# gmongaras/Stable-Diffusion-3-From-Scratch

Measured on AMD Instinct MI355X. Metric: train images/sec MMDiT-B 256^2 bf16, higher is better.
Workload: dtype bf16

## Files before the change

### include/mmdit_hip.h

```cpp
#ifndef MMDIT_HIP_H
#define MMDIT_HIP_H

#include <stdint.h>

#ifdef __cplusplus
extern "C" {
#endif

#define MMDIT_F32 0
#define MMDIT_BF16 1
#define MMDIT_FP8 2

#define MMDIT_ERR_ARG (-1)
#define MMDIT_ERR_DTYPE (-2)
#define MMDIT_ERR_SHAPE (-3)

#define MMDIT_ACT_NONE 0
#define MMDIT_ACT_SILU 1
#define MMDIT_ACT_SWIGLU 2

#define MMDIT_ACT_SWIGLU_BWD 3

#define MMDIT_PREC_BF16 0
#define MMDIT_PREC_SPLIT 1

typedef void* mmdit_stream_t;

#define MMDIT_ABI_VERSION 9
int mmdit_abi_version(void);
int mmdit_struct_size(int which);
const char* mmdit_build_arch(void);

typedef struct {
  const void* A; int a_dtype; int a_kmajor; int64_t lda;
  const void* B; int b_dtype; int b_kmajor; int64_t ldb;
  void* C; int c_dtype; int64_t ldc;
  int M, N, K;
  const float* bias;
  int act;
  const float* gate; int64_t ld_gate; int rows_per_batch;
  const float* residual; int64_t ld_res;
  void* aux; int aux_dtype; int64_t ld_aux;
  int accumulate;
  int precision;
  int split_k;
  int stream_k;
  int conv_mode, conv_H, conv_W, conv_C;
  const void* scale_a;
  const void* scale_b;
  int scale_mode;
  void* c_scales;
  float* dbias;
  int cu_budget;
} mmdit_gemm_args;
int mmdit_gemm(const mmdit_gemm_args* args, mmdit_stream_t stream);
int mmdit_gemm_grouped(const mmdit_gemm_args* args, int count, mmdit_stream_t stream);
int mmdit_gemm_zero_mask(const mmdit_gemm_args* args, int count, unsigned* mask);
typedef struct mmdit_qk_epilogue {
  const float* wq; const float* wk;
  const float* rope_cos; const float* rope_sin;
  int tokens, tok0;
} mmdit_qk_epilogue;
int mmdit_gemm_qkv_norm_rope(const mmdit_gemm_args* args, const mmdit_qk_epilogue* qk, int count, int heads, int s_total,
                             void* Q, void* K, void* V, mmdit_stream_t stream);
int mmdit_gemm_set_workspace(void* ptr, long long bytes);
int mmdit_gemm_set_claiming(int on);
int mmdit_gemm_get_claiming(void);
int mmdit_debug_occupy(int wgs, long long cycles, mmdit_stream_t stream);
int mmdit_device_cus(void);
int mmdit_gemm_plan(const mmdit_gemm_args* args, int count);

int mmdit_fp8_amax(const void* x, int x_dtype, int64_t n, float* amax, mmdit_stream_t stream);
int mmdit_fp8_quantize(const void* x, int x_dtype, int64_t n, const float* amax, void* q_fp8, float* scale, mmdit_stream_t stream);
int mmdit_fp8_quantize_delayed(const void* x, int x_dtype, int64_t n, float* state, int phase, float margin, void* q_fp8, mmdit_stream_t stream);
int mmdit_mxfp8_quantize(const void* x, int x_dtype, int rows, int K, int64_t ldx, void* q_fp8, void* scales_e8m0, mmdit_stream_t stream);
int mmdit_ln_modulate_fwd_mx(const float* x, const void* acc, int acc_dtype, const float* gate, int64_t ld_gate, float* x_out,
                             const float* scale, const float* shift, int64_t ld_mod, int rows, int d, int rows_per_batch,
                             void* q_fp8, void* scales_e8m0, float* mean, float* rstd, mmdit_stream_t stream);
int mmdit_swiglu_fwd_mx(const void* gu, int dtype, int rows, int hidden, void* q_fp8, void* scales_e8m0, mmdit_stream_t stream);
int mmdit_attn_fwd_mx(const void* Q, const void* K, const void* V, int batch, int heads, int S, int n_img, float scale,
                      void* Ox_fp8, void* Oc_fp8, void* scales_x, void* scales_c, mmdit_stream_t stream);

int mmdit_cast(const void* src, int src_dtype, void* dst, int dst_dtype, int64_t n, mmdit_stream_t stream);

int mmdit_ln_modulate_fwd(const float* x, const float* scale, const float* shift, int64_t ld_mod,
                          int rows, int d, int rows_per_batch,
                          void* out, int out_dtype, float* mean, float* rstd, mmdit_stream_t stream);
int mmdit_ln_modulate_fwd_res(const float* x, const void* acc, int acc_dtype, const float* gate, int64_t ld_gate, float* x_out,
                              const float* scale, const float* shift, int64_t ld_mod,
                              int rows, int d, int rows_per_batch,
                              void* out, int out_dtype, float* mean, float* rstd, mmdit_stream_t stream);
typedef struct mmdit_ln_fwd_problem {
  const float* x; const void* acc; const float* gate; int64_t ld_gate; float* x_out;
  const float* scale; const float* shift; int64_t ld_mod; int rows, rows_per_batch;
  void* out; float* mean; float* rstd;
} mmdit_ln_fwd_problem;
int mmdit_ln_modulate_fwd_pair(const mmdit_ln_fwd_problem* p0, const mmdit_ln_fwd_problem* p1, int d, int acc_dtype, int out_dtype, mmdit_stream_t stream);
typedef struct mmdit_ln_bwd_problem {
  const void* dout; const float* x; const float* mean; const float* rstd; const float* scale; int64_t ld_mod; const float* dres; int rows, rows_per_batch;
  float* dx; float* dscale; float* dshift; int64_t ld_dmod;
  const void* acc; const float* gate; int64_t ld_gate; void* dacc; float* dgate; int64_t ld_dgate; float* dbias; int64_t ld_dbias;
} mmdit_ln_bwd_problem;
int mmdit_ln_modulate_bwd_pair(const mmdit_ln_bwd_problem* p0, const mmdit_ln_bwd_problem* p1, int d, int dout_dtype, mmdit_stream_t stream);
int mmdit_gate_residual_fwd(const float* x, const void* acc, int acc_dtype, const float* gate, int64_t ld_gate,
                            int rows, int d, int rows_per_batch, float* out, mmdit_stream_t stream);
int mmdit_ln_modulate_bwd(const void* dout, int dout_dtype, const float* x, const float* mean, const float* rstd,
                          const float* scale, int64_t ld_mod, const float* dres,
                          int rows, int d, int rows_per_batch,
                          float* dx, float* dscale, float* dshift, int64_t ld_dmod, mmdit_stream_t stream);
int mmdit_ln_modulate_bwd_gated(const void* dout, int dout_dtype, const float* x, const float* mean, const float* rstd,
                                const float* scale, int64_t ld_mod, const float* dres,
                                int rows, int d, int rows_per_batch,
                                float* dx, float* dscale, float* dshift, int64_t ld_dmod,
                                const void* acc, int acc_dtype, const float* gate, int64_t ld_gate,
                                void* dacc, float* dgate, int64_t ld_dgate, float* dbias, int64_t ld_dbias, mmdit_stream_t stream);

int mmdit_text_rmsnorm_fwd(const void* x, int x_dtype, const float* w1, const float* w2, const float* s1, const float* s2,
                           int batch, int tokens, int split, int d, void* out1, void* out2, int out_dtype, mmdit_stream_t stream);
int mmdit_text_rmsnorm_bwd(const void* dout1, const void* dout2, int dout_dtype, const void* x, int x_dtype,
                           const float* w1, const float* w2, const float* s1, const float* s2,
                           int batch, int tokens, int split, int d,
                           float* dw1, float* dw2, float* ds1, float* ds2, mmdit_stream_t stream);

int mmdit_qk_norm_rope_fwd(const void* qkv, int qkv_dtype, const float* wq, const float* wk,
                           const float* rope_cos, const float* rope_sin,
                           int batch, int tokens, int heads, int s_total, int tok0,
                           void* Q, void* K, void* V, mmdit_stream_t stream);
int mmdit_qk_norm_rope_bwd(const void* dQ, const void* dK, const void* dV, int dq_dtype,
                           const void* qkv, int qkv_dtype, const float* wq, const float* wk,
                           const float* rope_cos, const float* rope_sin,
                           int batch, int tokens, int heads, int s_total, int tok0,
                           void* dqkv, int dqkv_dtype, float* dwq, float* dwk, mmdit_stream_t stream);
typedef struct mmdit_qk_problem {
  const void* qkv; const float* wq; const float* wk; const float* rope_cos; const float* rope_sin; int tokens, tok0;
  void* dqkv; float* dwq; float* dwk;
} mmdit_qk_problem;
int mmdit_qk_norm_rope_fwd_pair(const mmdit_qk_problem* p0, const mmdit_qk_problem* p1, int qkv_dtype, int batch, int heads, int s_total,
                                void* Q, void* K, void* V, mmdit_stream_t stream);
int mmdit_qk_norm_rope_bwd_pair(const mmdit_qk_problem* p0, const mmdit_qk_problem* p1, const void* dQ, const void* dK, const void* dV, int dq_dtype,
                                int qkv_dtype, int dqkv_dtype, int batch, int heads, int s_total, mmdit_stream_t stream);

int mmdit_attn_fwd(const void* Q, const void* K, const void* V, int batch, int heads, int S, int n_img,
                   float scale, int mode, void* Ox, void* Oc, float* lse, mmdit_stream_t stream);
int mmdit_attn_bwd_qk(const void* Q, const void* K, const void* V, const void* Ox, const void* Oc, const void* dOx, const void* dOc,
                      const float* lse, float* delta, int batch, int heads, int S, int n_img, float scale,
                      const void* qkv_x, const void* qkv_c, const float* wq_x, const float* wk_x, const float* wq_c, const float* wk_c,
                      const float* rope_cos, const float* rope_sin, void* dqkv_x, void* dqkv_c, float* dw, mmdit_stream_t stream);
int mmdit_attn_bwd(const void* Q, const void* K, const void* V, const void* Ox, const void* Oc,
                   const void* dOx, const void* dOc, const float* lse, float* delta,
                   int batch, int heads, int S, int n_img, float scale,
                   void* dQ, void* dK, void* dV, int dq_dtype, mmdit_stream_t stream);

int mmdit_swiglu_fwd(const void* gu, void* h, int dtype, int rows, int hidden, mmdit_stream_t stream);
int mmdit_swiglu_bwd(const void* dh, const void* gu, void* dgu, int dtype, int rows, int hidden, float* dbias, mmdit_stream_t stream);
int mmdit_gelu_fwd(const void* u, void* h, int dtype, int rows, int hidden, mmdit_stream_t stream);
int mmdit_gelu_bwd(const void* dh, const void* u, void* du, int dtype, int rows, int hidden, float* dbias, mmdit_stream_t stream);
typedef struct mmdit_mlp_bwd_problem { const void* dh; const void* gu; void* dgu; int rows; float* dbias; } mmdit_mlp_bwd_problem;
int mmdit_mlp_act_bwd_pair(const mmdit_mlp_bwd_problem* p0, const mmdit_mlp_bwd_problem* p1, int dtype, int hidden, int gelu, mmdit_stream_t stream);
int mmdit_silu_bwd(const void* dy, int dy_dtype, const float* pre, void* dpre, int dpre_dtype, int rows, int cols, float* dbias, int rows_per_bias,
                   mmdit_stream_t stream);

int mmdit_gate_residual_bwd(const float* dy, const void* acc, int acc_dtype, const float* gate, int64_t ld_gate,
                            int rows, int d, int rows_per_batch, void* dacc, int dacc_dtype,
                            float* dgate, int64_t ld_dgate, float* dbias, int64_t ld_dbias, mmdit_stream_t stream);

int mmdit_flow_loss(const float* v, const void* x0, const void* eps, int in_dtype, int64_t n, float coef, float* dv, float* partials,
                    float* loss, mmdit_stream_t stream);

int mmdit_colsum(const void* x, int dtype, int rows, int cols, int64_t ld, float* out, mmdit_stream_t stream);

int mmdit_patchify(const void* img, int img_dtype, int batch, int ch, int H, int W, void* tokens, int tok_dtype, mmdit_stream_t stream);
int mmdit_unpatchify(const void* tokens, int tok_dtype, int batch, int ch, int H, int W, void* img, int img_dtype, mmdit_stream_t stream);

int mmdit_time_embed_fwd(const float* t, const float* time_scale, const float* denom, int batch, int dim, void* out, int out_dtype, mmdit_stream_t stream);
int mmdit_time_embed_bwd(const void* dout, int dout_dtype, const float* t, const float* time_scale, const float* denom, int batch, int dim, float* dtime_scale, mmdit_stream_t stream);

int mmdit_vae_nchw_to_nhwc(const void* src, int src_dtype, int batch, int C, int H, int W, int C_padded, float scale, float shift,
                           void* dst_bf16, mmdit_stream_t stream);
int mmdit_vae_nhwc_to_nchw(const float* src, int batch, int C, int H, int W, int ld, float lo, float hi, float* dst, mmdit_stream_t stream);
int mmdit_vae_im2col3x3(const void* src_bf16, int batch, int H, int W, int C, int mode, void* dst_bf16, mmdit_stream_t stream);
int mmdit_vae_groupnorm(const void* x, int x_dtype, const float* gamma, const float* beta, int batch, int H, int W, int C, int groups, float eps, int silu,
                        float* sums_zeroed, void* y_bf16, int pad, mmdit_stream_t stream);
int mmdit_vae_pad_cast(const void* x, int x_dtype, int batch, int H, int W, int C, int upsample, void* y_bf16, mmdit_stream_t stream);
int mmdit_vae_softmax_rows(const float* x, int rows, int cols, int ld, float scale, void* y_bf16, mmdit_stream_t stream);

#define MMDIT_ADAMW_CHUNK 65536
typedef struct mmdit_adamw_tensor {
  float* param;
  const float* grad;
  float* exp_avg;
  float* exp_avg_sq;
  int64_t numel;
  void* shadow_bf16;
} mmdit_adamw_tensor;
int mmdit_grad_sumsq(const mmdit_adamw_tensor* tensors, const int* chunk_tensor, const int64_t* chunk_off, int n_chunks, float* partials, mmdit_stream_t stream);
int mmdit_clip_coef(const float* partials, int n_chunks, const float* loss_scale, float max_norm, float* out3, mmdit_stream_t stream);
int mmdit_adamw_step(const mmdit_adamw_tensor* tensors, const int* chunk_tensor, const int64_t* chunk_off, int n_chunks, const float* coef_found,
                     const float* step_count, double lr, double beta1, double beta2, double eps, double weight_decay, mmdit_stream_t stream);
int mmdit_adamw_step_dlr(const mmdit_adamw_tensor* tensors, const int* chunk_tensor, const int64_t* chunk_off, int n_chunks, const float* coef_found,
                         const float* step_count, const double* lr_dev, double beta1, double beta2, double eps, double weight_decay, mmdit_stream_t stream);

typedef struct mmdit_cast_tensor {
  const float* src;
  void* dst;
  int64_t numel;
} mmdit_cast_tensor;
int mmdit_cast_multi(const mmdit_cast_tensor* tensors, const int* chunk_tensor, const int64_t* chunk_off, int n_chunks, mmdit_stream_t stream);

#ifdef __cplusplus
}
#endif
#endif
```

### stable-diffusion-3-from-scratch_amd/_lib.py

```python
import ctypes
import os
import re

_HERE = os.path.dirname(os.path.abspath(__file__))
def experiment(name: str, default: str) -> str:
    return os.environ.get(name, default) if os.environ.get("MMDIT_EXPERIMENTS") == "1" else default


LIB_PATH = os.environ.get("MMDIT_LIB") or os.path.join(_HERE, "libmmdit_hip.so")
HEADER_PATH = os.path.join(_HERE, "..", "include", "mmdit_hip.h")

F32, BF16 = 0, 1
ACT_NONE, ACT_SILU, ACT_SWIGLU, ACT_SWIGLU_BWD = 0, 1, 2, 3
PREC_BF16, PREC_SPLIT = 0, 1
FP8 = 2

_vp, _i, _i64, _f, _d = ctypes.c_void_p, ctypes.c_int, ctypes.c_int64, ctypes.c_float, ctypes.c_double


class GemmArgs(ctypes.Structure):
    _fields_ = [
        ("A", _vp), ("a_dtype", _i), ("a_kmajor", _i), ("lda", _i64),
        ("B", _vp), ("b_dtype", _i), ("b_kmajor", _i), ("ldb", _i64),
        ("C", _vp), ("c_dtype", _i), ("ldc", _i64),
        ("M", _i), ("N", _i), ("K", _i),
        ("bias", _vp),
        ("act", _i),
        ("gate", _vp), ("ld_gate", _i64), ("rows_per_batch", _i),
        ("residual", _vp), ("ld_res", _i64),
        ("aux", _vp), ("aux_dtype", _i), ("ld_aux", _i64),
        ("accumulate", _i),
        ("precision", _i),
        ("split_k", _i),
        ("stream_k", _i),
        ("conv_mode", _i), ("conv_H", _i), ("conv_W", _i), ("conv_C", _i),
        ("scale_a", _vp), ("scale_b", _vp), ("scale_mode", _i), ("c_scales", _vp),
        ("dbias", _vp),
        ("cu_budget", _i),
    ]


class LnFwdProblem(ctypes.Structure):
    _fields_ = [("x", ctypes.c_void_p), ("acc", ctypes.c_void_p), ("gate", ctypes.c_void_p), ("ld_gate", ctypes.c_int64), ("x_out", ctypes.c_void_p),
                ("scale", ctypes.c_void_p), ("shift", ctypes.c_void_p), ("ld_mod", ctypes.c_int64), ("rows", ctypes.c_int), ("rows_per_batch", ctypes.c_int),
                ("out", ctypes.c_void_p), ("mean", ctypes.c_void_p), ("rstd", ctypes.c_void_p)]


class LnBwdProblem(ctypes.Structure):
    _fields_ = [("dout", ctypes.c_void_p), ("x", ctypes.c_void_p), ("mean", ctypes.c_void_p), ("rstd", ctypes.c_void_p), ("scale", ctypes.c_void_p),
                ("ld_mod", ctypes.c_int64), ("dres", ctypes.c_void_p), ("rows", ctypes.c_int), ("rows_per_batch", ctypes.c_int),
                ("dx", ctypes.c_void_p), ("dscale", ctypes.c_void_p), ("dshift", ctypes.c_void_p), ("ld_dmod", ctypes.c_int64),
                ("acc", ctypes.c_void_p), ("gate", ctypes.c_void_p), ("ld_gate", ctypes.c_int64), ("dacc", ctypes.c_void_p), ("dgate", ctypes.c_void_p),
                ("ld_dgate", ctypes.c_int64), ("dbias", ctypes.c_void_p), ("ld_dbias", ctypes.c_int64)]


class QkProblem(ctypes.Structure):
    _fields_ = [("qkv", ctypes.c_void_p), ("wq", ctypes.c_void_p), ("wk", ctypes.c_void_p), ("rope_cos", ctypes.c_void_p), ("rope_sin", ctypes.c_void_p),
                ("tokens", ctypes.c_int), ("tok0", ctypes.c_int), ("dqkv", ctypes.c_void_p), ("dwq", ctypes.c_void_p), ("dwk", ctypes.c_void_p)]


class MlpBwdProblem(ctypes.Structure):
    _fields_ = [("dh", ctypes.c_void_p), ("gu", ctypes.c_void_p), ("dgu", ctypes.c_void_p), ("rows", ctypes.c_int), ("dbias", ctypes.c_void_p)]


class QkEpilogue(ctypes.Structure):
    _fields_ = [("wq", _vp), ("wk", _vp), ("rope_cos", _vp), ("rope_sin", _vp), ("tokens", _i), ("tok0", _i)]


_SIGNATURES = {
    "mmdit_abi_version": ([], _i),
    "mmdit_struct_size": ([_i], _i),
    "mmdit_build_arch": ([], ctypes.c_char_p),
    "mmdit_gemm": ([ctypes.POINTER(GemmArgs), _vp], _i),
    "mmdit_gemm_grouped": ([ctypes.POINTER(GemmArgs), _i, _vp], _i),
    "mmdit_gemm_plan": ([ctypes.POINTER(GemmArgs), _i], _i),
    "mmdit_gemm_set_workspace": ([_vp, ctypes.c_longlong], _i),
    "mmdit_debug_occupy": ([_i, ctypes.c_longlong, _vp], _i),
    "mmdit_gemm_set_claiming": ([_i], _i),
    "mmdit_gemm_get_claiming": ([], _i),
    "mmdit_device_cus": ([], _i),
    "mmdit_gemm_qkv_norm_rope": ([ctypes.POINTER(GemmArgs), ctypes.POINTER(QkEpilogue), _i, _i, _i, _vp, _vp, _vp, _vp], _i),
    "mmdit_gemm_zero_mask": ([ctypes.POINTER(GemmArgs), _i, ctypes.POINTER(ctypes.c_uint)], _i),
    "mmdit_fp8_amax": ([_vp, _i, _i64, _vp, _vp], _i),
    "mmdit_fp8_quantize": ([_vp, _i, _i64, _vp, _vp, _vp, _vp], _i),
    "mmdit_fp8_quantize_delayed": ([_vp, _i, _i64, _vp, _i, ctypes.c_float, _vp, _vp], _i),
    "mmdit_mxfp8_quantize": ([_vp, _i, _i, _i, _i64, _vp, _vp, _vp], _i),
    "mmdit_ln_modulate_fwd_mx": ([_vp, _vp, _i, _vp, _i64, _vp, _vp, _vp, _i64, _i, _i, _i, _vp, _vp, _vp, _vp, _vp], _i),
    "mmdit_swiglu_fwd_mx": ([_vp, _i, _i, _i, _vp, _vp, _vp], _i),
    "mmdit_attn_fwd_mx": ([_vp, _vp, _vp, _i, _i, _i, _i, ctypes.c_float, _vp, _vp, _vp, _vp, _vp], _i),
    "mmdit_cast": ([_vp, _i, _vp, _i, _i64, _vp], _i),
    "mmdit_ln_modulate_fwd": ([_vp, _vp, _vp, _i64, _i, _i, _i, _vp, _i, _vp, _vp, _vp], _i),
    "mmdit_ln_modulate_fwd_res": ([_vp, _vp, _i, _vp, _i64, _vp, _vp, _vp, _i64, _i, _i, _i, _vp, _i, _vp, _vp, _vp], _i),
    "mmdit_ln_modulate_fwd_pair": ([ctypes.POINTER(LnFwdProblem), ctypes.POINTER(LnFwdProblem), _i, _i, _i, _vp], _i),
    "mmdit_ln_modulate_bwd_pair": ([ctypes.POINTER(LnBwdProblem), ctypes.POINTER(LnBwdProblem), _i, _i, _vp], _i),
    "mmdit_qk_norm_rope_fwd_pair": ([ctypes.POINTER(QkProblem), ctypes.POINTER(QkProblem), _i, _i, _i, _i, _vp, _vp, _vp, _vp], _i),
    "mmdit_qk_norm_rope_bwd_pair": ([ctypes.POINTER(QkProblem), ctypes.POINTER(QkProblem), _vp, _vp, _vp, _i, _i, _i, _i, _i, _i, _vp], _i),
    "mmdit_mlp_act_bwd_pair": ([ctypes.POINTER(MlpBwdProblem), ctypes.POINTER(MlpBwdProblem), _i, _i, _i, _vp], _i),
    "mmdit_gate_residual_fwd": ([_vp, _vp, _i, _vp, _i64, _i, _i, _i, _vp, _vp], _i),
    "mmdit_ln_modulate_bwd": ([_vp, _i, _vp, _vp, _vp, _vp, _i64, _vp, _i, _i, _i, _vp, _vp, _vp, _i64, _vp], _i),
    "mmdit_ln_modulate_bwd_gated": ([_vp, _i, _vp, _vp, _vp, _vp, _i64, _vp, _i, _i, _i, _vp, _vp, _vp, _i64, _vp, _i, _vp, _i64, _vp, _vp, _i64, _vp, _i64, _vp], _i),
    "mmdit_text_rmsnorm_fwd": ([_vp, _i, _vp, _vp, _vp, _vp, _i, _i, _i, _i, _vp, _vp, _i, _vp], _i),
    "mmdit_text_rmsnorm_bwd": ([_vp, _vp, _i, _vp, _i, _vp, _vp, _vp, _vp, _i, _i, _i, _i, _vp, _vp, _vp, _vp, _vp], _i),
    "mmdit_qk_norm_rope_fwd": ([_vp, _i, _vp, _vp, _vp, _vp, _i, _i, _i, _i, _i, _vp, _vp, _vp, _vp], _i),
    "mmdit_qk_norm_rope_bwd": ([_vp, _vp, _vp, _i, _vp, _i, _vp, _vp, _vp, _vp, _i, _i, _i, _i, _i, _vp, _i, _vp, _vp, _vp], _i),
    "mmdit_attn_fwd": ([_vp, _vp, _vp, _i, _i, _i, _i, _f, _i, _vp, _vp, _vp, _vp], _i),
    "mmdit_attn_bwd_qk": ([_vp] * 9 + [_i, _i, _i, _i, _f] + [_vp] * 11 + [_vp], _i),
    "mmdit_attn_bwd": ([_vp, _vp, _vp, _vp, _vp, _vp, _vp, _vp, _vp, _i, _i, _i, _i, _f, _vp, _vp, _vp, _i, _vp], _i),
    "mmdit_swiglu_fwd": ([_vp, _vp, _i, _i, _i, _vp], _i),
    "mmdit_swiglu_bwd": ([_vp, _vp, _vp, _i, _i, _i, _vp, _vp], _i),
    "mmdit_gelu_fwd": ([_vp, _vp, _i, _i, _i, _vp], _i),
    "mmdit_gelu_bwd": ([_vp, _vp, _vp, _i, _i, _i, _vp, _vp], _i),
    "mmdit_silu_bwd": ([_vp, _i, _vp, _vp, _i, _i, _i, _vp, _i, _vp], _i),
    "mmdit_gate_residual_bwd": ([_vp, _vp, _i, _vp, _i64, _i, _i, _i, _vp, _i, _vp, _i64, _vp, _i64, _vp], _i),
    "mmdit_flow_loss": ([_vp, _vp, _vp, _i, _i64, _f, _vp, _vp, _vp, _vp], _i),
    "mmdit_colsum": ([_vp, _i, _i, _i, _i64, _vp, _vp], _i),
    "mmdit_vae_nchw_to_nhwc": ([_vp, _i, _i, _i, _i, _i, _i, ctypes.c_float, ctypes.c_float, _vp, _vp], _i),
    "mmdit_vae_nhwc_to_nchw": ([_vp, _i, _i, _i, _i, _i, ctypes.c_float, ctypes.c_float, _vp, _vp], _i),
    "mmdit_vae_im2col3x3": ([_vp, _i, _i, _i, _i, _i, _vp, _vp], _i),
    "mmdit_vae_groupnorm": ([_vp, _i, _vp, _vp, _i, _i, _i, _i, _i, ctypes.c_float, _i, _vp, _vp, _i, _vp], _i),
    "mmdit_vae_pad_cast": ([_vp, _i, _i, _i, _i, _i, _i, _vp, _vp], _i),
    "mmdit_vae_softmax_rows": ([_vp, _i, _i, _i, ctypes.c_float, _vp, _vp], _i),
    "mmdit_patchify": ([_vp, _i, _i, _i, _i, _i, _vp, _i, _vp], _i),
    "mmdit_unpatchify": ([_vp, _i, _i, _i, _i, _i, _vp, _i, _vp], _i),
    "mmdit_time_embed_fwd": ([_vp, _vp, _vp, _i, _i, _vp, _i, _vp], _i),
    "mmdit_time_embed_bwd": ([_vp, _i, _vp, _vp, _vp, _i, _i, _vp, _vp], _i),
    "mmdit_grad_sumsq": ([_vp, _vp, _vp, _i, _vp, _vp], _i),
    "mmdit_clip_coef": ([_vp, _i, _vp, _f, _vp, _vp], _i),
    "mmdit_adamw_step": ([_vp, _vp, _vp, _i, _vp, _vp, _d, _d, _d, _d, _d, _vp], _i),
    "mmdit_adamw_step_dlr": ([_vp, _vp, _vp, _i, _vp, _vp, _vp, _d, _d, _d, _d, _vp], _i),
    "mmdit_cast_multi": ([_vp, _vp, _vp, _i, _vp], _i),
}
ADAMW_CHUNK = 65536
ABI_VERSION = 9
_STRUCTS = [("mmdit_gemm_args", GemmArgs), ("mmdit_ln_fwd_problem", LnFwdProblem), ("mmdit_ln_bwd_problem", LnBwdProblem),
            ("mmdit_qk_problem", QkProblem), ("mmdit_mlp_bwd_problem", MlpBwdProblem), ("mmdit_adamw_tensor", None), ("mmdit_cast_tensor", None), ("mmdit_qk_epilogue", QkEpilogue)]

_lib = None


def declared_symbols():
    with open(HEADER_PATH) as f:
        txt = f.read()
    return sorted(set(re.findall(r"\b(mmdit_[a-z0-9_]+)\s*\(", txt)) - {"mmdit_stream_t"})


def lib():
    global _lib
    if _lib is None:
        if not os.path.exists(LIB_PATH):
            raise RuntimeError(
                f"{LIB_PATH} is missing: build it with `python __graft_entry__.py build` "
                "(hipcc --offload-arch=gfx950).  There is no PyTorch/CPU fallback for the MMDiT hot path.")
        try:
            import torch
            if torch.cuda.is_available():
                torch.cuda.init()
        except ImportError:
            pass
        L = ctypes.CDLL(LIB_PATH)
        for name, (argtypes, restype) in _SIGNATURES.items():
            fn = getattr(L, name)
            fn.argtypes = argtypes
            fn.restype = restype
        if L.mmdit_abi_version() != ABI_VERSION:
            raise RuntimeError(f"{LIB_PATH}: ABI version {L.mmdit_abi_version()}, this binding is written for {ABI_VERSION}: rebuild (python __graft_entry__.py build)")
        for which, (name, struct) in enumerate(_STRUCTS):
            if struct is not None and L.mmdit_struct_size(which) != ctypes.sizeof(struct):
                raise RuntimeError(f"{LIB_PATH}: sizeof({name}) = {L.mmdit_struct_size(which)}, the binding's ctypes mirror has {ctypes.sizeof(struct)} bytes")
        _lib = L
    return _lib


ERR_ARG, ERR_DTYPE, ERR_SHAPE = -1, -2, -3


def check(status: int, what: str):
    if status != 0:
        kind = {-1: "invalid argument", -2: "dtype combination not built", -3: "unsupported shape"}.get(status, f"hipError {status}")
        raise RuntimeError(f"{what} failed: {kind}")
```

### stable-diffusion-3-from-scratch_amd/csrc/rowops.hip

```cpp
#include "common.h"
#include <float.h>

namespace {

constexpr float LN_EPS = 1e-5f;
constexpr float RMS_EPS = FLT_EPSILON;

__device__ __forceinline__ float bf16_round(float x) { return __builtin_bit_cast(float, pack_bf2(x, 0.f) << 16); }

template <int NITX, typename TO, typename TA, bool RES, bool MX = false>
__device__ __forceinline__ void ln_mod_fwd_body(int block, const float* __restrict__ x, const float* __restrict__ scale, const float* __restrict__ shift,
                                                int64_t ld_mod, int rows, int d, int rpb, TO* __restrict__ out,
                                                float* __restrict__ mean_o, float* __restrict__ rstd_o,
                                                const TA* __restrict__ acc, const float* __restrict__ gate, int64_t ld_gate, float* __restrict__ xo,
                                                unsigned char* __restrict__ mx_scales) {
  constexpr int NIT = NITX < 0 ? -NITX : NITX;
  constexpr bool EXACT = NITX < 0;
  const int lane = threadIdx.x & 63, row = block * 4 + (threadIdx.x >> 6);
  if (row >= rows) return;
  const int nch = d >> 2;
  const int b = row / rpb;
  const float* xr = x + (int64_t)row * d;
  float v[NIT][4];
  float s = 0.f;
#pragma unroll
  for (int it = 0; it < NIT; it++) {
    int ch = lane + 64 * it;
    if (EXACT || ch < nch) {
      ld4(xr + ch * 4, v[it]);
      if constexpr (RES) {
        float av[4], g[4];
        ld4(acc + (int64_t)row * d + ch * 4, av);
        ld4(gate + (int64_t)b * ld_gate + ch * 4, g);
#pragma unroll
        for (int e = 0; e < 4; e++) v[it][e] = v[it][e] + g[e] * av[e];
        __builtin_nontemporal_store(f32x4{v[it][0], v[it][1], v[it][2], v[it][3]}, (f32x4*)(xo + (int64_t)row * d + ch * 4));
      }
      s += v[it][0] + v[it][1] + v[it][2] + v[it][3];
    }
    else { v[it][0] = v[it][1] = v[it][2] = v[it][3] = 0.f; }
  }
  const float mean = wave_sum(s) / d;
  float q = 0.f;
#pragma unroll
  for (int it = 0; it < NIT; it++) {
    int ch = lane + 64 * it;
    if (EXACT || ch < nch) {
#pragma unroll
      for (int e = 0; e < 4; e++) { float c = v[it][e] - mean; q += c * c; }
    }
  }
  const float rstd = rsqrtf(wave_sum(q) / d + LN_EPS);
  if (lane == 0) { mean_o[row] = mean; rstd_o[row] = rstd; }
  const float* sc = scale + (int64_t)b * ld_mod;
  const float* sh = shift + (int64_t)b * ld_mod;
  TO* orow = out + (int64_t)row * d;
#pragma unroll
  for (int it = 0; it < NIT; it++) {
    int ch = lane + 64 * it;
    if (EXACT || ch < nch) {
      float a[4], h[4], o[4];
      ld4(sc + ch * 4, a); ld4(sh + ch * 4, h);
#pragma unroll
      for (int e = 0; e < 4; e++) o[e] = (v[it][e] - mean) * rstd * (1.f + a[e]) + h[e];
      if constexpr (MX) {
#pragma unroll
        for (int e = 0; e < 4; e++) o[e] = bf16_round(o[e]);
        float amax = fmaxf(fmaxf(fabsf(o[0]), fabsf(o[1])), fmaxf(fabsf(o[2]), fabsf(o[3])));
        amax = fmaxf(amax, __shfl_xor(amax, 1, 64));
        amax = fmaxf(amax, __shfl_xor(amax, 2, 64));
        amax = fmaxf(amax, __shfl_xor(amax, 4, 64));
        float inv;
        const int ex = mx_exponent(amax, inv);
        *(unsigned*)((unsigned char*)out + (int64_t)row * d + ch * 4) = mx_pack4(o, inv);
        if ((lane & 7) == 0) mx_scales[mx_scale_index(row, ch >> 3, rows)] = (unsigned char)(ex + 127);
      } else {
        st4(orow + ch * 4, o);
      }
    }
  }
}

template <int NIT, typename TO, typename TA, bool RES, bool MX = false>
__global__ __launch_bounds__(256) void ln_mod_fwd_kernel(const float* __restrict__ x, const float* __restrict__ scale, const float* __restrict__ shift,
                                                         int64_t ld_mod, int rows, int d, int rpb, TO* __restrict__ out,
                                                         float* __restrict__ mean_o, float* __restrict__ rstd_o,
                                                         const TA* __restrict__ acc, const float* __restrict__ gate, int64_t ld_gate, float* __restrict__ xo,
                                                         unsigned char* __restrict__ mx_scales = nullptr) {
  ln_mod_fwd_body<NIT, TO, TA, RES, MX>((int)blockIdx.x, x, scale, shift, ld_mod, rows, d, rpb, out, mean_o, rstd_o, acc, gate, ld_gate, xo, mx_scales);
}

struct LnFwdProb {
  const float* x; const float* scale; const float* shift; int64_t ld_mod; int rows, rpb; void* out; float* mean; float* rstd;
  const void* acc; const float* gate; int64_t ld_gate; float* xo;
};
template <int NIT, typename TO, typename TA, bool RES>
__global__ __launch_bounds__(256) void ln_mod_fwd_pair_kernel(LnFwdProb p0, LnFwdProb p1, int nblk0, int d) {
  const bool first = (int)blockIdx.x < nblk0;
  const LnFwdProb& p = first ? p0 : p1;
  ln_mod_fwd_body<NIT, TO, TA, RES, false>(first ? (int)blockIdx.x : (int)blockIdx.x - nblk0, p.x, p.scale, p.shift, p.ld_mod, p.rows, d, p.rpb, (TO*)p.out, p.mean, p.rstd,
                                           (const TA*)p.acc, p.gate, p.ld_gate, p.xo, nullptr);
}

template <typename TA>
__global__ __launch_bounds__(256) void gate_residual_fwd_kernel(const float* __restrict__ x, const TA* __restrict__ acc, const float* __restrict__ gate, int64_t ld_gate,
                                                                int rows, int d, int rpb, float* __restrict__ out) {
  const int nch = d >> 2;
  for (int64_t i = (int64_t)blockIdx.x * 256 + threadIdx.x; i < (int64_t)rows * nch; i += (int64_t)gridDim.x * 256) {
    const int row = (int)(i / nch), ch = (int)(i - (int64_t)row * nch);
    float xv[4], av[4], g[4];
    ld4(x + (int64_t)row * d + ch * 4, xv);
    ld4(acc + (int64_t)row * d + ch * 4, av);
    ld4(gate + (int64_t)(row / rpb) * ld_gate + ch * 4, g);
#pragma unroll
    for (int e = 0; e < 4; e++) xv[e] = xv[e] + g[e] * av[e];
    st4(out + (int64_t)row * d + ch * 4, xv);
  }
}

#ifndef MMDIT_LN_BWD_RCH
#define MMDIT_LN_BWD_RCH 16
#endif
constexpr int LN_BWD_RCH = MMDIT_LN_BWD_RCH;
template <int NITX, typename TG, typename TA, bool GATED>
__device__ __forceinline__ void ln_mod_bwd_body(int block, const TG* __restrict__ dout, const float* __restrict__ x, const float* __restrict__ mean_i,
                                                const float* __restrict__ rstd_i, const float* __restrict__ scale, int64_t ld_mod,
                                                const float* __restrict__ dres, int d, int rpb, int nchunk,
                                                float* __restrict__ dx, float* __restrict__ dscale, float* __restrict__ dshift, int64_t ld_dmod,
                                                const TA* __restrict__ acc, const float* __restrict__ gate, int64_t ld_gate, TA* __restrict__ dacc,
                                                float* __restrict__ dgate, int64_t ld_dgate, float* __restrict__ dbias, int64_t ld_dbias, int rch = LN_BWD_RCH) {
  constexpr int NIT = NITX < 0 ? -NITX : NITX;
  constexpr bool EXACT = NITX < 0;
  const int lane = threadIdx.x & 63, wave = threadIdx.x >> 6;
  const int b = block / nchunk, chunk = block % nchunk;
  const int nch = d >> 2;
  const float* sc = scale + (int64_t)b * ld_mod;
  __shared__ float s_a1[NIT * 256], s_gt[GATED ? NIT * 256 : 4];
  for (int c = threadIdx.x; c < NIT * 256; c += 256) {
    s_a1[c] = c < d ? sc[c] + 1.f : 0.f;
    if constexpr (GATED) s_gt[c] = c < d ? gate[(int64_t)b * ld_gate + c] : 0.f;
  }
  __syncthreads();
  float ds[NIT][4], dh[NIT][4];
  float sg[GATED ? NIT : 1][4], sb[GATED ? NIT : 1][4];
#pragma unroll
  for (int it = 0; it < NIT; it++) {
#pragma unroll
    for (int e = 0; e < 4; e++) { ds[it][e] = 0.f; dh[it][e] = 0.f; }
    if constexpr (GATED) {
#pragma unroll
      for (int e = 0; e < 4; e++) { sg[it][e] = 0.f; sb[it][e] = 0.f; }
    }
  }
  const int rend = min(rpb, (chunk + 1) * rch);
  for (int rl = chunk * rch + wave; rl < rend; rl += 4) {
    const int64_t row = (int64_t)b * rpb + rl;
    const float mean = mean_i[row], rstd = rstd_i[row];
    float g[NIT][4], xh[NIT][4];
    float c1 = 0.f, c2 = 0.f;
    asm volatile("" ::: "memory");
#pragma unroll
    for (int it = 0; it < NIT; it++) {
      int ch = lane + 64 * it;
      if (EXACT || ch < nch) {
        float dy[4], xv[4], a1[4];
        ld4_nt(dout + row * d + ch * 4, dy);
        ld4_nt(x + row * d + ch * 4, xv);
        ld4(s_a1 + ch * 4, a1);
#pragma unroll
        for (int e = 0; e < 4; e++) {
          xh[it][e] = (xv[e] - mean) * rstd;
          g[it][e] = dy[e] * a1[e];
          c1 += g[it][e]; c2 += g[it][e] * xh[it][e];
          ds[it][e] += dy[e] * xh[it][e]; dh[it][e] += dy[e];
        }
      }
    }
    c1 = wave_sum(c1) / d; c2 = wave_sum(c2) / d;
#pragma unroll
    for (int it = 0; it < NIT; it++) {
      int ch = lane + 64 * it;
      if (EXACT || ch < nch) {
        float o[4];
        if (dres) ld4(dres + row * d + ch * 4, o); else { o[0] = o[1] = o[2] = o[3] = 0.f; }
#pragma unroll
        for (int e = 0; e < 4; e++) o[e] += rstd * (g[it][e] - c1 - xh[it][e] * c2);
        st4(dx + row * d + ch * 4, o);
        if constexpr (GATED) {
          float av[4], da[4], gt[4];
          ld4_nt(acc + row * d + ch * 4, av);
          ld4(s_gt + ch * 4, gt);
#pragma unroll
          for (int e = 0; e < 4; e++) { da[e] = o[e] * gt[e]; sg[it][e] += o[e] * av[e]; sb[it][e] += da[e]; }
          st4(dacc + row * d + ch * 4, da);
        }
      }
    }
  }
  if constexpr (NIT <= 6) {
    __shared__ float red[4][NIT * 256];
    auto flush = [&](const float (&v)[NIT][4], float* dst) {
#pragma unroll
      for (int it = 0; it < NIT; it++)
#pragma unroll
        for (int e = 0; e < 4; e++) red[wave][(it * 64 + lane) * 4 + e] = v[it][e];
      __syncthreads();
      for (int c = threadIdx.x; c < d; c += 256) atomicAdd(dst + c, red[0][c] + red[1][c] + red[2][c] + red[3][c]);
      __syncthreads();
    };
    flush(ds, dscale + (int64_t)b * ld_dmod);
    flush(dh, dshift + (int64_t)b * ld_dmod);
    if constexpr (GATED) {
      flush(sg, dgate + (int64_t)b * ld_dgate);
      if (dbias) flush(sb, dbias + (int64_t)b * ld_dbias);
    }
  } else {
    auto flush = [&](const float (&v)[NIT][4], float* dst) {
#pragma unroll
      for (int it = 0; it < NIT; it++) {
        int ch = lane + 64 * it;
        if (EXACT || ch < nch) {
#pragma unroll
          for (int e = 0; e < 4; e++) atomicAdd(dst + ch * 4 + e, v[it][e]);
        }
      }
    };
    flush(ds, dscale + (int64_t)b * ld_dmod);
    flush(dh, dshift + (int64_t)b * ld_dmod);
    if constexpr (GATED) {
      flush(sg, dgate + (int64_t)b * ld_dgate);
      if (dbias) flush(sb, dbias + (int64_t)b * ld_dbias);
    }
  }
}

template <int NIT, typename TG, typename TA, bool GATED>
__global__ __launch_bounds__(256) void ln_mod_bwd_kernel(const TG* __restrict__ dout, const float* __restrict__ x, const float* __restrict__ mean_i,
                                                         const float* __restrict__ rstd_i, const float* __restrict__ scale, int64_t ld_mod,
                                                         const float* __restrict__ dres, int d, int rpb, int nchunk,
                                                         float* __restrict__ dx, float* __restrict__ dscale, float* __restrict__ dshift, int64_t ld_dmod,
                                                         const TA* __restrict__ acc, const float* __restrict__ gate, int64_t ld_gate, TA* __restrict__ dacc,
                                                         float* __restrict__ dgate, int64_t ld_dgate, float* __restrict__ dbias, int64_t ld_dbias) {
  ln_mod_bwd_body<NIT, TG, TA, GATED>((int)blockIdx.x, dout, x, mean_i, rstd_i, scale, ld_mod, dres, d, rpb, nchunk, dx, dscale, dshift, ld_dmod, acc, gate, ld_gate, dacc,
                                      dgate, ld_dgate, dbias, ld_dbias);
}

struct LnBwdProb {
  const void* dout; const float* x; const float* mean; const float* rstd; const float* scale; int64_t ld_mod; const float* dres; int rpb, nchunk;
  float* dx; float* dscale; float* dshift; int64_t ld_dmod;
  const void* acc; const float* gate; int64_t ld_gate; void* dacc; float* dgate; int64_t ld_dgate; float* dbias; int64_t ld_dbias;
};
template <int NIT, typename TG, typename TA, bool GATED>
__global__ __launch_bounds__(256) void ln_mod_bwd_pair_kernel(LnBwdProb p0, LnBwdProb p1, int nblk0, int d, int rch) {
  const bool first = (int)blockIdx.x < nblk0;
  const LnBwdProb& p = first ? p0 : p1;
  ln_mod_bwd_body<NIT, TG, TA, GATED>(first ? (int)blockIdx.x : (int)blockIdx.x - nblk0, (const TG*)p.dout, p.x, p.mean, p.rstd, p.scale, p.ld_mod, p.dres, d, p.rpb, p.nchunk,
                                      p.dx, p.dscale, p.dshift, p.ld_dmod, (const TA*)p.acc, p.gate, p.ld_gate, (TA*)p.dacc, p.dgate, p.ld_dgate, p.dbias, p.ld_dbias, rch);
}

template <int NITX, typename TI, typename TO>
__global__ __launch_bounds__(256) void text_rms_fwd_kernel(const TI* __restrict__ x, const float* __restrict__ w, const float* __restrict__ sp,
                                                           int rows, int cnt, int tokens, int off, int d, TO* __restrict__ out) {
  constexpr int NIT = NITX < 0 ? -NITX : NITX;
  constexpr bool EXACT = NITX < 0;
  const int lane = threadIdx.x & 63, m = blockIdx.x * 4 + (threadIdx.x >> 6);
  if (m >= rows) return;
  const int nch = d >> 2;
  const TI* xr = x + ((int64_t)(m / cnt) * tokens + off + m % cnt) * d;
  float v[NIT][4];
  float q = 0.f;
#pragma unroll
  for (int it = 0; it < NIT; it++) {
    int ch = lane + 64 * it;
    if (EXACT || ch < nch) { ld4(xr + ch * 4, v[it]); q += v[it][0] * v[it][0] + v[it][1] * v[it][1] + v[it][2] * v[it][2] + v[it][3] * v[it][3]; }
  }
  const float rinv = rsqrtf(wave_sum(q) / d + RMS_EPS);
  const float s = sp[0];
  TO* orow = out + (int64_t)m * d;
#pragma unroll
  for (int it = 0; it < NIT; it++) {
    int ch = lane + 64 * it;
    if (EXACT || ch < nch) {
      float wv[4], o[4];
      ld4(w + ch * 4, wv);
#pragma unroll
      for (int e = 0; e < 4; e++) o[e] = s * (v[it][e] * rinv * wv[e]);
      st4(orow + ch * 4, o);
    }
  }
}

#ifndef TRB_ROWS
#define TRB_ROWS 64
#endif
struct TextRmsBwdHalf { const void* dout; const float* w; const float* sp; int rows, cnt, off; float* dw; float* dsp; };
template <int NITX, typename TI, typename TG>
__global__ __launch_bounds__(512) void text_rms_bwd_kernel(TextRmsBwdHalf h0, TextRmsBwdHalf h1, const TI* __restrict__ x, int tokens, int d) {
  constexpr int NIT = NITX < 0 ? -NITX : NITX;
  constexpr bool EXACT = NITX < 0;
  const TextRmsBwdHalf& hp = blockIdx.y == 0 ? h0 : h1;
  const TG* __restrict__ dout = (const TG*)hp.dout;
  const float* __restrict__ w = hp.w;
  const float* __restrict__ sp = hp.sp;
  const int rows = hp.rows, cnt = hp.cnt, off = hp.off;
  float* __restrict__ dw = hp.dw;
  float* __restrict__ dsp = hp.dsp;
  __shared__ float red[NIT * 256];
  for (int c = threadIdx.x; c < NIT * 256; c += 512) red[c] = 0.f;
  __syncthreads();
  const int lane = threadIdx.x & 63, wave = threadIdx.x >> 6;
  const int nch = d >> 2;
  const float s = sp[0];
  float accw[NIT][4], wv[NIT][4];
  float accs = 0.f;
#pragma unroll
  for (int it = 0; it < NIT; it++) {
    int ch = lane + 64 * it;
    if (EXACT || ch < nch) ld4(w + ch * 4, wv[it]); else { wv[it][0] = wv[it][1] = wv[it][2] = wv[it][3] = 0.f; }
#pragma unroll
    for (int e = 0; e < 4; e++) accw[it][e] = 0.f;
  }
  for (int m = blockIdx.x * TRB_ROWS + wave; m < min(rows, (int)(blockIdx.x + 1) * TRB_ROWS); m += 8) {
    const TI* xr = x + ((int64_t)(m / cnt) * tokens + off + m % cnt) * d;
    float v[NIT][4];
    float q = 0.f;
#pragma unroll
    for (int it = 0; it < NIT; it++) {
      int ch = lane + 64 * it;
      if (EXACT || ch < nch) { ld4(xr + ch * 4, v[it]); q += v[it][0] * v[it][0] + v[it][1] * v[it][1] + v[it][2] * v[it][2] + v[it][3] * v[it][3]; }
    }
    const float rinv = rsqrtf(wave_sum(q) / d + RMS_EPS);
#pragma unroll
    for (int it = 0; it < NIT; it++) {
      int ch = lane + 64 * it;
      if (EXACT || ch < nch) {
        float dy[4];
        ld4(dout + (int64_t)m * d + ch * 4, dy);
#pragma unroll
        for (int e = 0; e < 4; e++) { float xn = v[it][e] * rinv; accw[it][e] += dy[e] * s * xn; accs += dy[e] * xn * wv[it][e]; }
      }
    }
  }
#pragma unroll
  for (int it = 0; it < NIT; it++) {
    const int ch = lane + 64 * it;
    if (EXACT || ch < nch) {
#pragma unroll
      for (int e = 0; e < 4; e++) atomicAdd(&red[ch * 4 + e], accw[it][e]);
    }
  }
  __syncthreads();
#ifndef TRB_NO_GLOBAL
  for (int c = threadIdx.x; c < d; c += 512) atomicAdd(dw + c, red[c]);
#else
  if (red[threadIdx.x] == 123.456f) dw[0] = 1.f;
#endif
  accs = wave_sum(accs);
#ifndef TRB_NO_DSP
  if (lane == 0) atomicAdd(dsp, accs);
#else
  if (accs == 123.456f) dsp[0] = 1.f;
#endif
}

__device__ __forceinline__ float group8_sum(float v) {
  v += __shfl_xor(v, 1, 64); v += __shfl_xor(v, 2, 64); v += __shfl_xor(v, 4, 64);
  return v;
}

template <typename TI>
__device__ __forceinline__ void qk_norm_rope_fwd_body(int bid, int rstride, const TI* __restrict__ qkv, const float* __restrict__ wq, const float* __restrict__ wk,
                                                      const float* __restrict__ rcos, const float* __restrict__ rsin,
                                                      int rows, int tokens, int heads, int s_total, int tok0,
                                                      bf16_t* __restrict__ Q, bf16_t* __restrict__ K, bf16_t* __restrict__ V) {
  const int hc = threadIdx.x % (8 * heads), part = threadIdx.x / (8 * heads), head = hc >> 3, chunk = hc & 7;
  bf16_t* obase = part == 0 ? Q : part == 1 ? K : V;
  float w[8];
#pragma unroll
  for (int e = 0; e < 8; e++) w[e] = 0.f;
  if (part < 2) ld8((part == 0 ? wq : wk) + chunk * 8, w);
  const bool same_token = rcos && rstride % tokens == 0;
  float cs[2][8], sn[2][8];
  if (same_token && part < 2) {
    const int n = bid % tokens;
    ld8(rcos + (int64_t)n * 64 + chunk * 8, cs[0]);
    ld8(rsin + (int64_t)n * 64 + chunk * 8, sn[0]);
#pragma unroll
    for (int e = 0; e < 8; e++) { cs[1][e] = cs[0][e]; sn[1][e] = sn[0][e]; }
  }
  for (int row0 = bid; row0 < rows; row0 += 2 * rstride) {
    float x[2][8];
#pragma unroll
    for (int k = 0; k < 2; k++) {
      const int row = min(row0 + k * rstride, rows - 1);
      ld8(qkv + (((int64_t)row * 3 + part) * heads + head) * 64 + chunk * 8, x[k]);
    }
    if (part < 2 && rcos && !same_token) {
#pragma unroll
      for (int k = 0; k < 2; k++) {
        const int n = min(row0 + k * rstride, rows - 1) % tokens;
        ld8(rcos + (int64_t)n * 64 + chunk * 8, cs[k]);
        ld8(rsin + (int64_t)n * 64 + chunk * 8, sn[k]);
      }
    }
#pragma unroll
    for (int k = 0; k < 2; k++) {
      const int row = row0 + k * rstride;
      if (row >= rows) break;
      const int n = row % tokens, b = row / tokens;
      if (part < 2) {
// ... 185 lines not shown
        if ((tx & 3) == 0) mx_scales[mx_scale_index(r, c >> 5, rows)] = (unsigned char)(ex + 127);
      } else {
        st8(h + (int64_t)r * hidden + c, o);
      }
    }
  }
}

__device__ __forceinline__ void colsum_flush(float (&acc)[8], float* sbuf , float* dst, int c, int ncols) {
  const int tx = threadIdx.x & 127, ty = threadIdx.x >> 7;
  if (ty == 1) {
#pragma unroll
    for (int e = 0; e < 8; e++) sbuf[tx * 8 + e] = acc[e];
  }
  __syncthreads();
  if (ty == 0 && c < ncols) {
#pragma unroll
    for (int e = 0; e < 8; e++) atomicAdd(dst + c + e, acc[e] + sbuf[tx * 8 + e]);
  }
  __syncthreads();
}

constexpr int MB_RCH = 128;
template <typename T, bool GELU>
__device__ __forceinline__ void mlp_act_bwd_body(int by, const T* __restrict__ dh, const T* __restrict__ gu, T* __restrict__ dgu,
                                                 int rows, int hidden, float* __restrict__ dbias) {
  __shared__ float sbuf[8 * 256];
  const int tx = threadIdx.x & 31, ty = threadIdx.x >> 5;
  const int c = blockIdx.x * 256 + tx * 8;
  const bool act = c < hidden;
  const int64_t ldi = GELU ? hidden : 2 * (int64_t)hidden;
  float sg[8], su[8];
#pragma unroll
  for (int e = 0; e < 8; e++) { sg[e] = 0.f; su[e] = 0.f; }
  const int rend = min(rows, (by + 1) * MB_RCH);
  if (act) {
    for (int r0 = by * MB_RCH + ty; r0 < rend; r0 += 16) {
      float d[2][8], g[2][8], u[2][8];
#pragma unroll
      for (int k = 0; k < 2; k++) {
        const int r = r0 + 8 * k;
        if (r < rend) {
          ld8_nt(dh + (int64_t)r * hidden + c, d[k]);
          ld8_nt(gu + r * ldi + c, g[k]);
          if constexpr (!GELU) ld8_nt(gu + r * ldi + hidden + c, u[k]);
        }
      }
#pragma unroll
      for (int k = 0; k < 2; k++) {
        const int r = r0 + 8 * k;
        if (r >= rend) break;
        float og[8], ou[8];
        if constexpr (GELU) {
#pragma unroll
          for (int e = 0; e < 8; e++) { og[e] = d[k][e] * gelu_grad_f(g[k][e]); sg[e] += og[e]; }
          st8(dgu + r * ldi + c, og);
        } else {
#pragma unroll
          for (int e = 0; e < 8; e++) {
            swiglu_bwd_f(d[k][e], g[k][e], u[k][e], og[e], ou[e]);
            sg[e] += og[e]; su[e] += ou[e];
          }
          st8(dgu + r * ldi + c, og);
          st8(dgu + r * ldi + hidden + c, ou);
        }
      }
    }
  }
  if (dbias) {
    const int col = blockIdx.x * 256 + threadIdx.x;
#pragma unroll
    for (int which = 0; which < (GELU ? 1 : 2); which++) {
#pragma unroll
      for (int e = 0; e < 8; e++) sbuf[ty * 256 + tx * 8 + e] = which == 0 ? sg[e] : su[e];
      __syncthreads();
      if (col < hidden) {
        float s = 0.f;
#pragma unroll
        for (int r = 0; r < 8; r++) s += sbuf[r * 256 + threadIdx.x];
        atomicAdd(dbias + which * hidden + col, s);
      }
      __syncthreads();
    }
  }
}
template <typename T, bool GELU>
__global__ __launch_bounds__(256) void mlp_act_bwd_kernel(const T* __restrict__ dh, const T* __restrict__ gu, T* __restrict__ dgu,
                                                          int rows, int hidden, float* __restrict__ dbias) {
  mlp_act_bwd_body<T, GELU>((int)blockIdx.y, dh, gu, dgu, rows, hidden, dbias);
}
struct MlpBwdProb { const void* dh; const void* gu; void* dgu; int rows; float* dbias; };
template <typename T, bool GELU>
__global__ __launch_bounds__(256) void mlp_act_bwd_pair_kernel(MlpBwdProb p0, MlpBwdProb p1, int nby0, int hidden) {
  const bool first = (int)blockIdx.y < nby0;
  const MlpBwdProb& p = first ? p0 : p1;
  mlp_act_bwd_body<T, GELU>(first ? (int)blockIdx.y : (int)blockIdx.y - nby0, (const T*)p.dh, (const T*)p.gu, (T*)p.dgu, p.rows, hidden, p.dbias);
}

constexpr int GR_RCH = 64;
template <typename TA, typename TO>
__global__ __launch_bounds__(256) void gate_res_bwd_kernel(const float* __restrict__ dy, const TA* __restrict__ acc, const float* __restrict__ gate, int64_t ld_gate,
                                                           int d, int rpb, int nchunk, TO* __restrict__ dacc,
                                                           float* __restrict__ dgate, int64_t ld_dgate, float* __restrict__ dbias, int64_t ld_dbias) {
  __shared__ float sbuf[8 * 256];
  const int tx = threadIdx.x & 31, ty = threadIdx.x >> 5;
  const int c = blockIdx.x * 256 + tx * 8;
  const bool act = c < d;
  const int b = blockIdx.y / nchunk, chunk = blockIdx.y % nchunk;
  float g[8], sgate[8], sb[8];
#pragma unroll
  for (int e = 0; e < 8; e++) { g[e] = 0.f; sgate[e] = 0.f; sb[e] = 0.f; }
  if (act) {
    ld8(gate + (int64_t)b * ld_gate + c, g);
    const int rend = min(rpb, (chunk + 1) * GR_RCH);
    for (int rl = chunk * GR_RCH + ty; rl < rend; rl += 16) {
      const int64_t row0 = (int64_t)b * rpb + rl, row1 = row0 + 8;
      const bool two = rl + 8 < rend;
      float dv0[8], av0[8], dv1[8], av1[8], o[8];
      ld8(dy + row0 * d + c, dv0);
      ld8(acc + row0 * d + c, av0);
      if (two) {
        ld8(dy + row1 * d + c, dv1);
        ld8(acc + row1 * d + c, av1);
      }
#pragma unroll
      for (int e = 0; e < 8; e++) { o[e] = dv0[e] * g[e]; sgate[e] += dv0[e] * av0[e]; sb[e] += o[e]; }
      st8(dacc + row0 * d + c, o);
      if (two) {
#pragma unroll
        for (int e = 0; e < 8; e++) { o[e] = dv1[e] * g[e]; sgate[e] += dv1[e] * av1[e]; sb[e] += o[e]; }
        st8(dacc + row1 * d + c, o);
      }
    }
  }
  const int col = blockIdx.x * 256 + threadIdx.x;
#pragma unroll
  for (int which = 0; which < 2; which++) {
    float* dst = which == 0 ? dgate + (int64_t)b * ld_dgate : (dbias ? dbias + (int64_t)b * ld_dbias : nullptr);
    if (!dst) break;
#pragma unroll
    for (int e = 0; e < 8; e++) sbuf[ty * 256 + tx * 8 + e] = which == 0 ? sgate[e] : sb[e];
    __syncthreads();
    if (col < d) {
      float s = 0.f;
#pragma unroll
      for (int r = 0; r < 8; r++) s += sbuf[r * 256 + threadIdx.x];
      atomicAdd(dst + col, s);
    }
    __syncthreads();
  }
}

template <typename T>
__global__ __launch_bounds__(256) void colsum_kernel(const T* __restrict__ x, int rows, int cols, int64_t ld, float* __restrict__ out, int rch) {
  __shared__ float sbuf[1024];
  const int tx = threadIdx.x & 127, ty = threadIdx.x >> 7;
  const int c = blockIdx.x * 1024 + tx * 8;
  float s[8];
#pragma unroll
  for (int e = 0; e < 8; e++) s[e] = 0.f;
  if (c < cols) {
    const int rend = min(rows, (int)(blockIdx.y + 1) * rch);
#pragma unroll 4
    for (int r = blockIdx.y * rch + ty; r < rend; r += 2) {
      float v[8];
      ld8(x + r * ld + c, v);
#pragma unroll
      for (int e = 0; e < 8; e++) s[e] += v[e];
    }
  }
  colsum_flush(s, sbuf, out, c, cols);
}

template <typename TG, typename TO>
__global__ __launch_bounds__(256) void silu_bwd_kernel(const TG* __restrict__ dy, const float* __restrict__ pre, TO* __restrict__ dpre, int rpg, int cols, float* __restrict__ dbias) {
  __shared__ float sb[4][64];
  const int cl = threadIdx.x & 63, rl = threadIdx.x >> 6;
  const int c = blockIdx.x * 64 + cl;
  const int r0 = blockIdx.y * rpg;
  float s = 0.f;
  if (c < cols) {
#pragma unroll 4
    for (int r = r0 + rl; r < r0 + rpg; r += 4) {
      const int64_t i = (int64_t)r * cols + c;
      const float p = pre[i], sig = sigmoid_f(p);
      const float g = io<TG>::ld(dy + i) * sig * (1.f + p * (1.f - sig));
      io<TO>::st(dpre + i, g);
      s += g;
    }
  }
  sb[rl][cl] = s;
  __syncthreads();
  if (rl == 0 && c < cols && dbias) dbias[(int64_t)blockIdx.y * cols + c] += sb[0][cl] + sb[1][cl] + sb[2][cl] + sb[3][cl];
}

template <typename TI, typename TO>
__global__ void cast_kernel(const TI* __restrict__ src, TO* __restrict__ dst, int64_t n) {
  const int64_t n8 = n >> 3;
  for (int64_t i = (int64_t)blockIdx.x * blockDim.x + threadIdx.x; i < n8; i += (int64_t)gridDim.x * blockDim.x) {
    float v[8];
    ld8(src + i * 8, v);
    st8(dst + i * 8, v);
  }
  if (blockIdx.x == 0 && threadIdx.x < (n & 7)) io<TO>::st(dst + n8 * 8 + threadIdx.x, io<TI>::ld(src + n8 * 8 + threadIdx.x));
}

template <typename TI, typename TO, bool TO_TOKENS>
__global__ void patch_kernel(const TI* __restrict__ src, TO* __restrict__ dst, int batch, int ch, int H, int W) {
  const int W2 = W >> 1, H2 = H >> 1;
  const int64_t total = (int64_t)batch * ch * H * W2;
  for (int64_t g = (int64_t)blockIdx.x * blockDim.x + threadIdx.x; g < total; g += (int64_t)gridDim.x * blockDim.x) {
    const int j = (int)(g % W2); int64_t r = g / W2;
    const int y = (int)(r % H); r /= H;
    const int c = (int)(r % ch); const int64_t b = r / ch;
    const int64_t img_off = ((b * ch + c) * H + y) * W + 2 * j;
    const int64_t tok_off = ((b * H2 + (y >> 1)) * W2 + j) * (int64_t)(ch * 4) + c * 4 + (y & 1) * 2;
    if (TO_TOKENS) { io<TO>::st(dst + tok_off, io<TI>::ld(src + img_off)); io<TO>::st(dst + tok_off + 1, io<TI>::ld(src + img_off + 1)); }
    else { io<TO>::st(dst + img_off, io<TI>::ld(src + tok_off)); io<TO>::st(dst + img_off + 1, io<TI>::ld(src + tok_off + 1)); }
  }
}

template <typename TO>
__global__ void time_embed_fwd_kernel(const float* __restrict__ t, const float* __restrict__ ts, const float* __restrict__ denom, int batch, int dim, TO* __restrict__ out) {
  const int i = blockIdx.x * blockDim.x + threadIdx.x, b = blockIdx.y;
  if (i >= dim) return;
  const float tau = t[b] * ts[0];
  const int half = dim >> 1;
  const float v = i < half ? sinf(tau / denom[2 * i]) : cosf(tau / denom[2 * (i - half) + 1]);
  io<TO>::st(out + (int64_t)b * dim + i, v);
}

template <typename TG>
__global__ __launch_bounds__(256) void time_embed_bwd_kernel(const TG* __restrict__ dout, const float* __restrict__ t, const float* __restrict__ ts,
                                                             const float* __restrict__ denom, int batch, int dim, float* __restrict__ dts) {
  __shared__ float red[4];
  const int b = blockIdx.x;
  const float tau = t[b] * ts[0];
  const int half = dim >> 1;
  float s = 0.f;
  for (int i = threadIdx.x; i < dim; i += 256) {
    const float g = io<TG>::ld(dout + (int64_t)b * dim + i);
    if (i < half) { const float dn = denom[2 * i]; s += g * cosf(tau / dn) / dn; }
    else { const float dn = denom[2 * (i - half) + 1]; s -= g * sinf(tau / dn) / dn; }
  }
  s = wave_sum(s);
  if ((threadIdx.x & 63) == 0) red[threadIdx.x >> 6] = s;
  __syncthreads();
  if (threadIdx.x == 0) atomicAdd(dts, (red[0] + red[1] + red[2] + red[3]) * t[b]);
}

inline int nit_for(int d) { return (d / 4 + 63) / 64; }
inline int grid_cap(int64_t n, int bs) { int64_t g = (n + bs - 1) / bs; return (int)(g < 1 ? 1 : g > 4096 ? 4096 : g); }

}

#define NIT_CASE(n, ...)                                                        \
  { if (d == (n) * 256) { constexpr int NIT = -(n); __VA_ARGS__; } else { constexpr int NIT = (n); __VA_ARGS__; } }
#define NIT_SWITCH(nit, ...)                                    \
  do {                                                          \
    if (nit <= 1) NIT_CASE(1, __VA_ARGS__)                      \
    else if (nit <= 2) NIT_CASE(2, __VA_ARGS__)                 \
    else if (nit <= 3) NIT_CASE(3, __VA_ARGS__)                 \
    else if (nit <= 4) NIT_CASE(4, __VA_ARGS__)                 \
    else if (nit <= 6) NIT_CASE(6, __VA_ARGS__)                 \
    else if (nit <= 9) NIT_CASE(9, __VA_ARGS__)                 \
    else if (nit <= 12) NIT_CASE(12, __VA_ARGS__)               \
    else NIT_CASE(16, __VA_ARGS__)                              \
  } while (0)

#define LN_FWD_NIT (NIT < 0 ? -NIT : NIT)

extern "C" int mmdit_abi_version(void) { return MMDIT_ABI_VERSION; }
extern "C" int mmdit_struct_size(int which) {
  switch (which) {
    case 0: return (int)sizeof(mmdit_gemm_args);
    case 1: return (int)sizeof(mmdit_ln_fwd_problem);
    case 2: return (int)sizeof(mmdit_ln_bwd_problem);
    case 3: return (int)sizeof(mmdit_qk_problem);
    case 4: return (int)sizeof(mmdit_mlp_bwd_problem);
    case 5: return (int)sizeof(mmdit_adamw_tensor);
    case 6: return (int)sizeof(mmdit_cast_tensor);
    case 7: return (int)sizeof(mmdit_qk_epilogue);
    default: return -1;
  }
}
extern "C" const char* mmdit_build_arch(void) { return "gfx950"; }

extern "C" int mmdit_ln_modulate_fwd(const float* x, const float* scale, const float* shift, int64_t ld_mod, int rows, int d, int rpb,
                                     void* out, int out_dtype, float* mean, float* rstd, mmdit_stream_t stream) {
  MMDIT_CHECK_ARG(x && scale && shift && out && mean && rstd && rows > 0 && d > 0 && d % 4 == 0 && d <= 4096 && rpb > 0 && ld_mod % 4 == 0);
  hipStream_t s = (hipStream_t)stream;
  const int nit = nit_for(d);
  dim3 grid((rows + 3) / 4);
  if (out_dtype == MMDIT_BF16) { NIT_SWITCH(nit, hipLaunchKernelGGL((ln_mod_fwd_kernel<LN_FWD_NIT, bf16_t, bf16_t, false>), grid, dim3(256), 0, s, x, scale, shift, ld_mod, rows, d, rpb, (bf16_t*)out, mean, rstd, nullptr, nullptr, 0, nullptr)); }
  else if (out_dtype == MMDIT_F32) { NIT_SWITCH(nit, hipLaunchKernelGGL((ln_mod_fwd_kernel<LN_FWD_NIT, float, float, false>), grid, dim3(256), 0, s, x, scale, shift, ld_mod, rows, d, rpb, (float*)out, mean, rstd, nullptr, nullptr, 0, nullptr)); }
  else return MMDIT_ERR_DTYPE;
  return mmdit_launch_status();
}

extern "C" int mmdit_ln_modulate_fwd_res(const float* x, const void* acc, int acc_dtype, const float* gate, int64_t ld_gate, float* x_out,
                                         const float* scale, const float* shift, int64_t ld_mod, int rows, int d, int rpb,
                                         void* out, int out_dtype, float* mean, float* rstd, mmdit_stream_t stream) {
  MMDIT_CHECK_ARG(x && acc && gate && x_out && scale && shift && out && mean && rstd && rows > 0 && d > 0 && d % 4 == 0 && d <= 4096 && rpb > 0 && ld_mod % 4 == 0 && ld_gate % 4 == 0);
  MMDIT_CHECK_ARG(acc_dtype == out_dtype);
  hipStream_t s = (hipStream_t)stream;
  const int nit = nit_for(d);
  dim3 grid((rows + 3) / 4);
  if (out_dtype == MMDIT_BF16) { NIT_SWITCH(nit, hipLaunchKernelGGL((ln_mod_fwd_kernel<LN_FWD_NIT, bf16_t, bf16_t, true>), grid, dim3(256), 0, s, x, scale, shift, ld_mod, rows, d, rpb, (bf16_t*)out, mean, rstd, (const bf16_t*)acc, gate, ld_gate, x_out)); }
  else if (out_dtype == MMDIT_F32) { NIT_SWITCH(nit, hipLaunchKernelGGL((ln_mod_fwd_kernel<LN_FWD_NIT, float, float, true>), grid, dim3(256), 0, s, x, scale, shift, ld_mod, rows, d, rpb, (float*)out, mean, rstd, (const float*)acc, gate, ld_gate, x_out)); }
  else return MMDIT_ERR_DTYPE;
  return mmdit_launch_status();
}

extern "C" int mmdit_ln_modulate_fwd_mx(const float* x, const void* acc, int acc_dtype, const float* gate, int64_t ld_gate, float* x_out,
                                        const float* scale, const float* shift, int64_t ld_mod, int rows, int d, int rpb,
                                        void* q_fp8, void* scales_e8m0, float* mean, float* rstd, mmdit_stream_t stream) {
  MMDIT_CHECK_ARG(x && scale && shift && q_fp8 && scales_e8m0 && mean && rstd && rows > 0 && d > 0 && d % 64 == 0 && d <= 4096 && rpb > 0 && ld_mod % 4 == 0);
  MMDIT_CHECK_ARG(!acc || (gate && x_out && acc_dtype == MMDIT_BF16 && ld_gate % 4 == 0));
  hipStream_t s = (hipStream_t)stream;
  const int nit = nit_for(d);
  dim3 grid((rows + 3) / 4);
  unsigned char* q = (unsigned char*)q_fp8;
  unsigned char* sc = (unsigned char*)scales_e8m0;
  if (acc) { NIT_SWITCH(nit, hipLaunchKernelGGL((ln_mod_fwd_kernel<LN_FWD_NIT, unsigned char, bf16_t, true, true>), grid, dim3(256), 0, s, x, scale, shift, ld_mod, rows, d, rpb, q, mean, rstd, (const bf16_t*)acc, gate, ld_gate, x_out, sc)); }
  else { NIT_SWITCH(nit, hipLaunchKernelGGL((ln_mod_fwd_kernel<LN_FWD_NIT, unsigned char, bf16_t, false, true>), grid, dim3(256), 0, s, x, scale, shift, ld_mod, rows, d, rpb, q, mean, rstd, nullptr, nullptr, 0, nullptr, sc)); }
  return mmdit_launch_status();
}

extern "C" int mmdit_gate_residual_fwd(const float* x, const void* acc, int acc_dtype, const float* gate, int64_t ld_gate, int rows, int d, int rpb,
                                       float* out, mmdit_stream_t stream) {
  MMDIT_CHECK_ARG(x && acc && gate && out && rows > 0 && d > 0 && d % 4 == 0 && rpb > 0 && ld_gate % 4 == 0);
  hipStream_t s = (hipStream_t)stream;
  dim3 grid(grid_cap((int64_t)rows * (d / 4), 256));
  if (acc_dtype == MMDIT_BF16) hipLaunchKernelGGL((gate_residual_fwd_kernel<bf16_t>), grid, dim3(256), 0, s, x, (const bf16_t*)acc, gate, ld_gate, rows, d, rpb, out);
  else if (acc_dtype == MMDIT_F32) hipLaunchKernelGGL((gate_residual_fwd_kernel<float>), grid, dim3(256), 0, s, x, (const float*)acc, gate, ld_gate, rows, d, rpb, out);
  else return MMDIT_ERR_DTYPE;
  return mmdit_launch_status();
}

template <typename TG, typename TA, bool GATED>
static int ln_mod_bwd_launch(const void* dout, const float* x, const float* mean, const float* rstd, const float* scale, int64_t ld_mod, const float* dres,
                             int rows, int d, int rpb, float* dx, float* dscale, float* dshift, int64_t ld_dmod, const void* acc, const float* gate,
                             int64_t ld_gate, void* dacc, float* dgate, int64_t ld_dgate, float* dbias, int64_t ld_dbias, hipStream_t s) {
  const int nit = nit_for(d), nchunk = (rpb + LN_BWD_RCH - 1) / LN_BWD_RCH;
  dim3 grid((rows / rpb) * nchunk);
  NIT_SWITCH(nit, hipLaunchKernelGGL((ln_mod_bwd_kernel<(NIT < 0 ? -NIT : NIT), TG, TA, GATED>), grid, dim3(256), 0, s, (const TG*)dout, x, mean, rstd, scale, ld_mod, dres, d, rpb, nchunk,
                                     dx, dscale, dshift, ld_dmod, (const TA*)acc, gate, ld_gate, (TA*)dacc, dgate, ld_dgate, dbias, ld_dbias));
  return mmdit_launch_status();
}

extern "C" int mmdit_ln_modulate_bwd(const void* dout, int dout_dtype, const float* x, const float* mean, const float* rstd, const float* scale, int64_t ld_mod,
                                     const float* dres, int rows, int d, int rpb, float* dx, float* dscale, float* dshift, int64_t ld_dmod, mmdit_stream_t stream) {
  MMDIT_CHECK_ARG(dout && x && mean && rstd && scale && dx && dscale && dshift && rows > 0 && d % 4 == 0 && d <= 4096 && rpb > 0 && rows % rpb == 0 && ld_mod % 4 == 0);
  hipStream_t s = (hipStream_t)stream;
  if (dout_dtype == MMDIT_BF16) return ln_mod_bwd_launch<bf16_t, bf16_t, false>(dout, x, mean, rstd, scale, ld_mod, dres, rows, d, rpb, dx, dscale, dshift, ld_dmod, nullptr, nullptr, 0, nullptr, nullptr, 0, nullptr, 0, s);
  if (dout_dtype == MMDIT_F32) return ln_mod_bwd_launch<float, float, false>(dout, x, mean, rstd, scale, ld_mod, dres, rows, d, rpb, dx, dscale, dshift, ld_dmod, nullptr, nullptr, 0, nullptr, nullptr, 0, nullptr, 0, s);
  return MMDIT_ERR_DTYPE;
}

extern "C" int mmdit_ln_modulate_bwd_gated(const void* dout, int dout_dtype, const float* x, const float* mean, const float* rstd, const float* scale, int64_t ld_mod,
                                           const float* dres, int rows, int d, int rpb, float* dx, float* dscale, float* dshift, int64_t ld_dmod,
                                           const void* acc, int acc_dtype, const float* gate, int64_t ld_gate, void* dacc, float* dgate, int64_t ld_dgate,
                                           float* dbias, int64_t ld_dbias, mmdit_stream_t stream) {
  MMDIT_CHECK_ARG(dout && x && mean && rstd && scale && dx && dscale && dshift && rows > 0 && d % 4 == 0 && d <= 4096 && rpb > 0 && rows % rpb == 0 && ld_mod % 4 == 0);
  MMDIT_CHECK_ARG(acc && gate && dacc && dgate && ld_gate % 4 == 0 && acc_dtype == dout_dtype);
  hipStream_t s = (hipStream_t)stream;
  if (dout_dtype == MMDIT_BF16) return ln_mod_bwd_launch<bf16_t, bf16_t, true>(dout, x, mean, rstd, scale, ld_mod, dres, rows, d, rpb, dx, dscale, dshift, ld_dmod, acc, gate, ld_gate, dacc, dgate, ld_dgate, dbias, ld_dbias, s);
  if (dout_dtype == MMDIT_F32) return ln_mod_bwd_launch<float, float, true>(dout, x, mean, rstd, scale, ld_mod, dres, rows, d, rpb, dx, dscale, dshift, ld_dmod, acc, gate, ld_gate, dacc, dgate, ld_dgate, dbias, ld_dbias, s);
  return MMDIT_ERR_DTYPE;
}

extern "C" int mmdit_ln_modulate_fwd_pair(const mmdit_ln_fwd_problem* a, const mmdit_ln_fwd_problem* b, int d, int acc_dtype, int out_dtype, mmdit_stream_t stream) {
  MMDIT_CHECK_ARG(a && b && d > 0 && d % 4 == 0 && d <= 4096);
  const bool res = a->acc != nullptr;
  MMDIT_CHECK_ARG((b->acc != nullptr) == res && (!res || acc_dtype == out_dtype));
  LnFwdProb q[2];
  const mmdit_ln_fwd_problem* src[2] = {a, b};
  for (int i = 0; i < 2; i++) {
    const mmdit_ln_fwd_problem* p = src[i];
    MMDIT_CHECK_ARG(p->x && p->scale && p->shift && p->out && p->mean && p->rstd && p->rows > 0 && p->rows_per_batch > 0 && p->ld_mod % 4 == 0);
    if (res) MMDIT_CHECK_ARG(p->gate && p->x_out && p->ld_gate % 4 == 0);
    q[i] = LnFwdProb{p->x, p->scale, p->shift, p->ld_mod, p->rows, p->rows_per_batch, p->out, p->mean, p->rstd, p->acc, p->gate, p->ld_gate, p->x_out};
  }
  hipStream_t s = (hipStream_t)stream;
  const int nit = nit_for(d), nb0 = (a->rows + 3) / 4, nb1 = (b->rows + 3) / 4;
  dim3 grid(nb0 + nb1);
#define LNP(TO, RES) NIT_SWITCH(nit, hipLaunchKernelGGL((ln_mod_fwd_pair_kernel<LN_FWD_NIT, TO, TO, RES>), grid, dim3(256), 0, s, q[0], q[1], nb0, d))
  if (out_dtype == MMDIT_BF16) { if (res) { LNP(bf16_t, true); } else { LNP(bf16_t, false); } }
  else if (out_dtype == MMDIT_F32) { if (res) { LNP(float, true); } else { LNP(float, false); } }
  else return MMDIT_ERR_DTYPE;
#undef LNP
  return mmdit_launch_status();
}

extern "C" int mmdit_ln_modulate_bwd_pair(const mmdit_ln_bwd_problem* a, const mmdit_ln_bwd_problem* b, int d, int dout_dtype, mmdit_stream_t stream) {
  MMDIT_CHECK_ARG(a && b && d > 0 && d % 4 == 0 && d <= 4096 && a->rows_per_batch > 0 && b->rows_per_batch > 0);
  const bool gated = a->acc != nullptr;
  MMDIT_CHECK_ARG((b->acc != nullptr) == gated);
  LnBwdProb q[2];
  const mmdit_ln_bwd_problem* src[2] = {a, b};
  int nb[2];
  auto wgs = [&](int r) { return (long)(a->rows / a->rows_per_batch) * ((a->rows_per_batch + r - 1) / r) + (long)(b->rows / b->rows_per_batch) * ((b->rows_per_batch + r - 1) / r); };
  const int nit_ = nit_for(d), nit_abs = nit_ < 0 ? -nit_ : nit_;
  int per_cu = nit_abs <= 3 ? 4 : nit_abs == 4 ? 3 : 2, cus = 256;
  {
    static int occ[64][17][2][2], cu_count[64];
    const int dev = mmdit_current_device(), ti = dout_dtype == MMDIT_BF16 ? 0 : 1, gi = gated ? 1 : 0, ni = nit_abs > 16 ? 16 : nit_abs;
    if (!cu_count[dev]) {
      int n = 0;
      cu_count[dev] = (hipDeviceGetAttribute(&n, hipDeviceAttributeMultiprocessorCount, dev) == hipSuccess && n > 0) ? n : 256;
    }
    cus = cu_count[dev];
    if (!occ[dev][ni][ti][gi]) {
      int nbq = 0;
      hipError_t e = hipErrorUnknown;
#define LNQ(T, G) NIT_SWITCH(nit_, e = hipOccupancyMaxActiveBlocksPerMultiprocessor(&nbq, (const void*)ln_mod_bwd_pair_kernel<(NIT < 0 ? -NIT : NIT), T, T, G>, 256, 0))
      if (dout_dtype == MMDIT_BF16) { if (gated) { LNQ(bf16_t, true); } else { LNQ(bf16_t, false); } }
      else if (dout_dtype == MMDIT_F32) { if (gated) { LNQ(float, true); } else { LNQ(float, false); } }
#undef LNQ
      occ[dev][ni][ti][gi] = (e == hipSuccess && nbq > 0) ? nbq : 8;
    }
    per_cu = per_cu < occ[dev][ni][ti][gi] ? per_cu : occ[dev][ni][ti][gi];
  }
  const long slots = (long)cus * per_cu;
  int rch = LN_BWD_RCH;
  if (wgs(LN_BWD_RCH) > slots && wgs(LN_BWD_RCH) <= 2 * slots)
    for (int r = LN_BWD_RCH + 4; r <= 64; r += 4)
      if (wgs(r) <= slots) { rch = r; break; }
  for (int i = 0; i < 2; i++) {
    const mmdit_ln_bwd_problem* p = src[i];
    MMDIT_CHECK_ARG(p->dout && p->x && p->mean && p->rstd && p->scale && p->dx && p->dscale && p->dshift && p->rows > 0 && p->rows_per_batch > 0 &&
                    p->rows % p->rows_per_batch == 0 && p->ld_mod % 4 == 0);
    if (gated) MMDIT_CHECK_ARG(p->gate && p->dacc && p->dgate && p->ld_gate % 4 == 0);
    const int nchunk = (p->rows_per_batch + rch - 1) / rch;
    nb[i] = (p->rows / p->rows_per_batch) * nchunk;
    q[i] = LnBwdProb{p->dout, p->x, p->mean, p->rstd, p->scale, p->ld_mod, p->dres, p->rows_per_batch, nchunk, p->dx, p->dscale, p->dshift, p->ld_dmod,
                     p->acc, p->gate, p->ld_gate, p->dacc, p->dgate, p->ld_dgate, p->dbias, p->ld_dbias};
  }
  hipStream_t s = (hipStream_t)stream;
  const int nit = nit_for(d);
  dim3 grid(nb[0] + nb[1]);
#define LNP(T, G) NIT_SWITCH(nit, hipLaunchKernelGGL((ln_mod_bwd_pair_kernel<(NIT < 0 ? -NIT : NIT), T, T, G>), grid, dim3(256), 0, s, q[0], q[1], nb[0], d, rch))
  if (dout_dtype == MMDIT_BF16) { if (gated) { LNP(bf16_t, true); } else { LNP(bf16_t, false); } }
  else if (dout_dtype == MMDIT_F32) { if (gated) { LNP(float, true); } else { LNP(float, false); } }
  else return MMDIT_ERR_DTYPE;
#undef LNP
  return mmdit_launch_status();
}

extern "C" int mmdit_text_rmsnorm_fwd(const void* x, int x_dtype, const float* w1, const float* w2, const float* s1, const float* s2,
                                      int batch, int tokens, int split, int d, void* out1, void* out2, int out_dtype, mmdit_stream_t stream) {
  MMDIT_CHECK_ARG(x && w1 && w2 && s1 && s2 && out1 && out2 && batch > 0 && split > 0 && split < tokens && d % 4 == 0 && d <= 4096);
  hipStream_t s = (hipStream_t)stream;
  const int nit = nit_for(d);
  for (int half = 0; half < 2; half++) {
    const int cnt = half ? tokens - split : split, off = half ? split : 0, rows = batch * cnt;
    const float* w = half ? w2 : w1; const float* sp = half ? s2 : s1; void* out = half ? out2 : out1;
    dim3 grid((rows + 3) / 4);
#define TRF(TI, TO) NIT_SWITCH(nit, hipLaunchKernelGGL((text_rms_fwd_kernel<LN_FWD_NIT, TI, TO>), grid, dim3(256), 0, s, (const TI*)x, w, sp, rows, cnt, tokens, off, d, (TO*)out))
    if (x_dtype == MMDIT_F32 && out_dtype == MMDIT_F32) { TRF(float, float); }
    else if (x_dtype == MMDIT_F32 && out_dtype == MMDIT_BF16) { TRF(float, bf16_t); }
    else if (x_dtype == MMDIT_BF16 && out_dtype == MMDIT_BF16) { TRF(bf16_t, bf16_t); }
    else if (x_dtype == MMDIT_BF16 && out_dtype == MMDIT_F32) { TRF(bf16_t, float); }
    else return MMDIT_ERR_DTYPE;
#undef TRF
  }
  return mmdit_launch_status();
}

extern "C" int mmdit_text_rmsnorm_bwd(const void* dout1, const void* dout2, int dout_dtype, const void* x, int x_dtype,
                                      const float* w1, const float* w2, const float* s1, const float* s2, int batch, int tokens, int split, int d,
                                      float* dw1, float* dw2, float* ds1, float* ds2, mmdit_stream_t stream) {
  MMDIT_CHECK_ARG(dout1 && dout2 && x && w1 && w2 && s1 && s2 && dw1 && dw2 && ds1 && ds2 && batch > 0 && split > 0 && split < tokens && d % 4 == 0 && d <= 4096);
  hipStream_t s = (hipStream_t)stream;
  const int nit = nit_for(d);
  TextRmsBwdHalf h[2];
  int maxrows = 0;
  for (int half = 0; half < 2; half++) {
    const int cnt = half ? tokens - split : split, rows = batch * cnt;
    h[half] = TextRmsBwdHalf{half ? dout2 : dout1, half ? w2 : w1, half ? s2 : s1, rows, cnt, half ? split : 0, half ? dw2 : dw1, half ? ds2 : ds1};
    maxrows = rows > maxrows ? rows : maxrows;
  }
  dim3 grid((maxrows + TRB_ROWS - 1) / TRB_ROWS, 2);
#define TRB(TI, TG) NIT_SWITCH(nit, hipLaunchKernelGGL((text_rms_bwd_kernel<NIT, TI, TG>), grid, dim3(512), 0, s, h[0], h[1], (const TI*)x, tokens, d))
  if (x_dtype == MMDIT_F32 && dout_dtype == MMDIT_F32) { TRB(float, float); }
  else if (x_dtype == MMDIT_F32 && dout_dtype == MMDIT_BF16) { TRB(float, bf16_t); }
  else if (x_dtype == MMDIT_BF16 && dout_dtype == MMDIT_BF16) { TRB(bf16_t, bf16_t); }
  else if (x_dtype == MMDIT_BF16 && dout_dtype == MMDIT_F32) { TRB(bf16_t, float); }
  else return MMDIT_ERR_DTYPE;
#undef TRB
  return mmdit_launch_status();
}

extern "C" int mmdit_qk_norm_rope_fwd(const void* qkv, int qkv_dtype, const float* wq, const float* wk, const float* rope_cos, const float* rope_sin,
                                      int batch, int tokens, int heads, int s_total, int tok0, void* Q, void* K, void* V, mmdit_stream_t stream) {
  MMDIT_CHECK_ARG(qkv && wq && wk && Q && K && V && batch > 0 && tokens > 0 && heads > 0 && tok0 >= 0 && tok0 + tokens <= s_total);
  MMDIT_CHECK_ARG((rope_cos == nullptr) == (rope_sin == nullptr));
  hipStream_t s = (hipStream_t)stream;
  MMDIT_CHECK_ARG(24 * heads <= 1024);
  const int rows = batch * tokens;
  int g = rows < 1024 ? rows : 1024;
  if (rope_cos && tokens <= 1024 && rows >= tokens) g = (g / tokens > 0 ? g / tokens : 1) * tokens;
  dim3 grid(g);
  if (qkv_dtype == MMDIT_BF16) hipLaunchKernelGGL((qk_norm_rope_fwd_kernel<bf16_t>), grid, dim3(24 * heads), 0, s, (const bf16_t*)qkv, wq, wk, rope_cos, rope_sin, rows, tokens, heads, s_total, tok0, (bf16_t*)Q, (bf16_t*)K, (bf16_t*)V);
  else if (qkv_dtype == MMDIT_F32) hipLaunchKernelGGL((qk_norm_rope_fwd_kernel<float>), grid, dim3(24 * heads), 0, s, (const float*)qkv, wq, wk, rope_cos, rope_sin, rows, tokens, heads, s_total, tok0, (bf16_t*)Q, (bf16_t*)K, (bf16_t*)V);
  else return MMDIT_ERR_DTYPE;
  return mmdit_launch_status();
}

static int qk_bwd_rl(int heads, int min_rows) {
  static const int env = [] { const char* e = mmdit_exp_env("MMDIT_QK_RL"); return e ? atoi(e) : 0; }();
  int rl = 1024 / (24 * heads);
  if (env > 0 && env < rl) rl = env;
  if (rl < 1 || min_rows < 2048) rl = 1;
  return rl;
}
static int qk_bwd_grid(int rows, int tokens, bool rope, int& rl) {
  static const int lanes_max = [] { const char* e = mmdit_exp_env("MMDIT_QK_LANES"); return e ? atoi(e) : 768; }();
  if (rl == 1) {
    int g = rows < 512 ? rows : 512;
    if (rope && tokens <= 1024 && rows >= tokens) g = (g / tokens > 0 ? g / tokens : 1) * tokens;
    return g;
  }
  if (!rope) return lanes_max / rl;
  if (tokens > lanes_max) return tokens <= 2048 && tokens % rl == 0 ? tokens / rl : lanes_max / rl;
  int k = lanes_max / tokens;
  while (k > 1 && (k * tokens) % rl) k--;
  if ((k * tokens) % rl) return lanes_max / rl;
  return k * tokens / rl;
}

extern "C" int mmdit_qk_norm_rope_bwd(const void* dQ, const void* dK, const void* dV, int dq_dtype, const void* qkv, int qkv_dtype,
                                      const float* wq, const float* wk, const float* rope_cos, const float* rope_sin,
                                      int batch, int tokens, int heads, int s_total, int tok0, void* dqkv, int dqkv_dtype, float* dwq, float* dwk, mmdit_stream_t stream) {
  MMDIT_CHECK_ARG(dQ && dK && dV && qkv && wq && wk && dqkv && dwq && dwk && batch > 0 && tokens > 0 && heads > 0 && tok0 >= 0 && tok0 + tokens <= s_total);
  MMDIT_CHECK_ARG((rope_cos == nullptr) == (rope_sin == nullptr));
  hipStream_t s = (hipStream_t)stream;
  MMDIT_CHECK_ARG(heads >= 1 && 24 * heads <= 1024);
  const int rows = batch * tokens;
  int rl = qk_bwd_rl(heads, rows);
  dim3 grid(qk_bwd_grid(rows, tokens, rope_cos != nullptr, rl));
  const bool fast = !rope_cos || ((int)grid.x * rl) % tokens == 0;
#define QKB(TG, TI, TO) do { if (fast) hipLaunchKernelGGL((qk_norm_rope_bwd_kernel<true, TG, TI, TO>), grid, dim3(24 * heads * rl), 0, s, (const TG*)dQ, (const TG*)dK, (const TG*)dV, (const TI*)qkv, wq, wk, rope_cos, rope_sin, rows, tokens, heads, s_total, tok0, (TO*)dqkv, dwq, dwk); \
  else hipLaunchKernelGGL((qk_norm_rope_bwd_kernel<false, TG, TI, TO>), grid, dim3(24 * heads * rl), 0, s, (const TG*)dQ, (const TG*)dK, (const TG*)dV, (const TI*)qkv, wq, wk, rope_cos, rope_sin, rows, tokens, heads, s_total, tok0, (TO*)dqkv, dwq, dwk); } while (0)
  if (dq_dtype == MMDIT_BF16 && qkv_dtype == MMDIT_BF16 && dqkv_dtype == MMDIT_BF16) QKB(bf16_t, bf16_t, bf16_t);
  else if (dq_dtype == MMDIT_F32 && qkv_dtype == MMDIT_F32 && dqkv_dtype == MMDIT_F32) QKB(float, float, float);
  else if (dq_dtype == MMDIT_BF16 && qkv_dtype == MMDIT_F32 && dqkv_dtype == MMDIT_F32) QKB(bf16_t, float, float);
  else return MMDIT_ERR_DTYPE;
#undef QKB
  return mmdit_launch_status();
}

extern "C" int mmdit_qk_norm_rope_fwd_pair(const mmdit_qk_problem* a, const mmdit_qk_problem* b, int qkv_dtype, int batch, int heads, int s_total,
                                           void* Q, void* K, void* V, mmdit_stream_t stream) {
  MMDIT_CHECK_ARG(a && b && Q && K && V && batch > 0 && heads > 0 && 24 * heads <= 1024);
  const mmdit_qk_problem* src[2] = {a, b};
  QkProb q[2];
  int g[2];
  for (int i = 0; i < 2; i++) {
    const mmdit_qk_problem* p = src[i];
    MMDIT_CHECK_ARG(p->qkv && p->wq && p->wk && p->tokens > 0 && p->tok0 >= 0 && p->tok0 + p->tokens <= s_total && (p->rope_cos == nullptr) == (p->rope_sin == nullptr));
    const int rows = batch * p->tokens;
    g[i] = rows < 1024 ? rows : 1024;
    if (p->rope_cos && p->tokens <= 1024) g[i] = (g[i] / p->tokens > 0 ? g[i] / p->tokens : 1) * p->tokens;
    q[i] = QkProb{p->qkv, p->wq, p->wk, p->rope_cos, p->rope_sin, rows, p->tokens, p->tok0, nullptr, nullptr, nullptr, nullptr, nullptr, nullptr};
  }
  hipStream_t s = (hipStream_t)stream;
  dim3 grid(g[0] + g[1]);
  if (qkv_dtype == MMDIT_BF16) hipLaunchKernelGGL((qk_norm_rope_fwd_pair_kernel<bf16_t>), grid, dim3(24 * heads), 0, s, q[0], q[1], g[0], heads, s_total, (bf16_t*)Q, (bf16_t*)K, (bf16_t*)V);
  else if (qkv_dtype == MMDIT_F32) hipLaunchKernelGGL((qk_norm_rope_fwd_pair_kernel<float>), grid, dim3(24 * heads), 0, s, q[0], q[1], g[0], heads, s_total, (bf16_t*)Q, (bf16_t*)K, (bf16_t*)V);
  else return MMDIT_ERR_DTYPE;
  return mmdit_launch_status();
}

extern "C" int mmdit_qk_norm_rope_bwd_pair(const mmdit_qk_problem* a, const mmdit_qk_problem* b, const void* dQ, const void* dK, const void* dV, int dq_dtype,
                                           int qkv_dtype, int dqkv_dtype, int batch, int heads, int s_total, mmdit_stream_t stream) {
  MMDIT_CHECK_ARG(a && b && dQ && dK && dV && batch > 0 && heads > 0 && 24 * heads <= 1024);
  const mmdit_qk_problem* src[2] = {a, b};
  QkProb q[2];
  int g[2];
  for (int i = 0; i < 2; i++) {
    const mmdit_qk_problem* p = src[i];
    MMDIT_CHECK_ARG(p->qkv && p->wq && p->wk && p->dqkv && p->dwq && p->dwk && p->tokens > 0 && p->tok0 >= 0 && p->tok0 + p->tokens <= s_total &&
                    (p->rope_cos == nullptr) == (p->rope_sin == nullptr));
    q[i] = QkProb{p->qkv, p->wq, p->wk, p->rope_cos, p->rope_sin, batch * p->tokens, p->tokens, p->tok0, dQ, dK, dV, p->dqkv, p->dwq, p->dwk};
  }
  int rl = qk_bwd_rl(heads, q[0].rows < q[1].rows ? q[0].rows : q[1].rows);
  for (int i = 0; i < 2; i++) g[i] = qk_bwd_grid(q[i].rows, q[i].tokens, q[i].rcos != nullptr, rl);
  hipStream_t s = (hipStream_t)stream;
  dim3 grid(g[0] + g[1]);
  bool fast = true;
  for (int i = 0; i < 2; i++) fast = fast && (!q[i].rcos || (g[i] * rl) % q[i].tokens == 0);
#define QKP(TG, TI, TO) do { if (fast) hipLaunchKernelGGL((qk_norm_rope_bwd_pair_kernel<true, TG, TI, TO>), grid, dim3(24 * heads * rl), 0, s, q[0], q[1], g[0], heads, s_total); \
  else hipLaunchKernelGGL((qk_norm_rope_bwd_pair_kernel<false, TG, TI, TO>), grid, dim3(24 * heads * rl), 0, s, q[0], q[1], g[0], heads, s_total); } while (0)
  if (dq_dtype == MMDIT_BF16 && qkv_dtype == MMDIT_BF16 && dqkv_dtype == MMDIT_BF16) QKP(bf16_t, bf16_t, bf16_t);
  else if (dq_dtype == MMDIT_F32 && qkv_dtype == MMDIT_F32 && dqkv_dtype == MMDIT_F32) QKP(float, float, float);
  else if (dq_dtype == MMDIT_BF16 && qkv_dtype == MMDIT_F32 && dqkv_dtype == MMDIT_F32) QKP(bf16_t, float, float);
  else return MMDIT_ERR_DTYPE;
#undef QKP
  return mmdit_launch_status();
}

extern "C" int mmdit_mlp_act_bwd_pair(const mmdit_mlp_bwd_problem* a, const mmdit_mlp_bwd_problem* b, int dtype, int hidden, int gelu, mmdit_stream_t stream) {
  MMDIT_CHECK_ARG(a && b && hidden > 0 && hidden % 8 == 0);
  const mmdit_mlp_bwd_problem* src[2] = {a, b};
  MlpBwdProb q[2];
  int nby[2];
  for (int i = 0; i < 2; i++) {
    MMDIT_CHECK_ARG(src[i]->dh && src[i]->gu && src[i]->dgu && src[i]->rows > 0);
    q[i] = MlpBwdProb{src[i]->dh, src[i]->gu, src[i]->dgu, src[i]->rows, src[i]->dbias};
    nby[i] = (src[i]->rows + MB_RCH - 1) / MB_RCH;
  }
  dim3 grid((hidden + 255) / 256, nby[0] + nby[1]);
  hipStream_t s = (hipStream_t)stream;
#define MBP(T, G) hipLaunchKernelGGL((mlp_act_bwd_pair_kernel<T, G>), grid, dim3(256), 0, s, q[0], q[1], nby[0], hidden)
  if (dtype == MMDIT_BF16) { if (gelu) MBP(bf16_t, true); else MBP(bf16_t, false); }
  else if (dtype == MMDIT_F32) { if (gelu) MBP(float, true); else MBP(float, false); }
  else return MMDIT_ERR_DTYPE;
#undef MBP
  return mmdit_launch_status();
}

template <bool GELU>
static int mlp_act_fwd(const void* gu, void* h, int dtype, int rows, int hidden, mmdit_stream_t stream) {
  MMDIT_CHECK_ARG(gu && h && rows > 0 && hidden > 0 && hidden % 8 == 0);
  dim3 grid((hidden + 255) / 256, (rows + CO_RCH - 1) / CO_RCH);
  hipStream_t s = (hipStream_t)stream;
  if (dtype == MMDIT_BF16) hipLaunchKernelGGL((mlp_act_fwd_kernel<bf16_t, GELU>), grid, dim3(256), 0, s, (const bf16_t*)gu, (bf16_t*)h, rows, hidden);
  else if (dtype == MMDIT_F32) hipLaunchKernelGGL((mlp_act_fwd_kernel<float, GELU>), grid, dim3(256), 0, s, (const float*)gu, (float*)h, rows, hidden);
  else return MMDIT_ERR_DTYPE;
  return mmdit_launch_status();
}
template <bool GELU>
static int mlp_act_bwd(const void* dh, const void* gu, void* dgu, int dtype, int rows, int hidden, float* dbias, mmdit_stream_t stream) {
  MMDIT_CHECK_ARG(dh && gu && dgu && rows > 0 && hidden > 0 && hidden % 8 == 0);
  dim3 grid((hidden + 255) / 256, (rows + MB_RCH - 1) / MB_RCH);
  hipStream_t s = (hipStream_t)stream;
  if (dtype == MMDIT_BF16) hipLaunchKernelGGL((mlp_act_bwd_kernel<bf16_t, GELU>), grid, dim3(256), 0, s, (const bf16_t*)dh, (const bf16_t*)gu, (bf16_t*)dgu, rows, hidden, dbias);
  else if (dtype == MMDIT_F32) hipLaunchKernelGGL((mlp_act_bwd_kernel<float, GELU>), grid, dim3(256), 0, s, (const float*)dh, (const float*)gu, (float*)dgu, rows, hidden, dbias);
  else return MMDIT_ERR_DTYPE;
  return mmdit_launch_status();
}
extern "C" int mmdit_swiglu_fwd_mx(const void* gu, int dtype, int rows, int hidden, void* q_fp8, void* scales_e8m0, mmdit_stream_t stream) {
  MMDIT_CHECK_ARG(gu && q_fp8 && scales_e8m0 && rows > 0 && hidden > 0 && hidden % 64 == 0);
  dim3 grid((hidden + 255) / 256, (rows + CO_RCH - 1) / CO_RCH);
  hipStream_t s = (hipStream_t)stream;
  if (dtype == MMDIT_BF16) hipLaunchKernelGGL((mlp_act_fwd_kernel<bf16_t, false, true>), grid, dim3(256), 0, s, (const bf16_t*)gu, (bf16_t*)q_fp8, rows, hidden, (unsigned char*)scales_e8m0);
  else return MMDIT_ERR_DTYPE;
  return mmdit_launch_status();
}
extern "C" int mmdit_swiglu_fwd(const void* gu, void* h, int dtype, int rows, int hidden, mmdit_stream_t st) { return mlp_act_fwd<false>(gu, h, dtype, rows, hidden, st); }
extern "C" int mmdit_swiglu_bwd(const void* dh, const void* gu, void* dgu, int dtype, int rows, int hidden, float* dbias, mmdit_stream_t st) { return mlp_act_bwd<false>(dh, gu, dgu, dtype, rows, hidden, dbias, st); }
extern "C" int mmdit_gelu_fwd(const void* u, void* h, int dtype, int rows, int hidden, mmdit_stream_t st) { return mlp_act_fwd<true>(u, h, dtype, rows, hidden, st); }
extern "C" int mmdit_gelu_bwd(const void* dh, const void* u, void* du, int dtype, int rows, int hidden, float* dbias, mmdit_stream_t st) { return mlp_act_bwd<true>(dh, u, du, dtype, rows, hidden, dbias, st); }

extern "C" int mmdit_silu_bwd(const void* dy, int dy_dtype, const float* pre, void* dpre, int dpre_dtype, int rows, int cols, float* dbias, int rows_per_bias,
                              mmdit_stream_t stream) {
  MMDIT_CHECK_ARG(dy && pre && dpre && rows > 0 && cols > 0);
  const int rpg = rows_per_bias > 0 ? rows_per_bias : rows;
  MMDIT_CHECK_ARG(rows % rpg == 0);
  hipStream_t s = (hipStream_t)stream;
  dim3 grid((cols + 63) / 64, rows / rpg);
  if (dy_dtype == MMDIT_BF16 && dpre_dtype == MMDIT_BF16) hipLaunchKernelGGL((silu_bwd_kernel<bf16_t, bf16_t>), grid, dim3(256), 0, s, (const bf16_t*)dy, pre, (bf16_t*)dpre, rpg, cols, dbias);
  else if (dy_dtype == MMDIT_F32 && dpre_dtype == MMDIT_F32) hipLaunchKernelGGL((silu_bwd_kernel<float, float>), grid, dim3(256), 0, s, (const float*)dy, pre, (float*)dpre, rpg, cols, dbias);
  else if (dy_dtype == MMDIT_F32 && dpre_dtype == MMDIT_BF16) hipLaunchKernelGGL((silu_bwd_kernel<float, bf16_t>), grid, dim3(256), 0, s, (const float*)dy, pre, (bf16_t*)dpre, rpg, cols, dbias);
  else return MMDIT_ERR_DTYPE;
  return mmdit_launch_status();
}

extern "C" int mmdit_gate_residual_bwd(const float* dy, const void* acc, int acc_dtype, const float* gate, int64_t ld_gate, int rows, int d, int rpb,
                                       void* dacc, int dacc_dtype, float* dgate, int64_t ld_dgate, float* dbias, int64_t ld_dbias, mmdit_stream_t stream) {
  MMDIT_CHECK_ARG(dy && acc && gate && dacc && dgate && rows > 0 && d % 8 == 0 && rpb > 0 && rows % rpb == 0 && ld_gate % 4 == 0);
  hipStream_t s = (hipStream_t)stream;
  const int nchunk = (rpb + GR_RCH - 1) / GR_RCH;
  dim3 grid((d + 255) / 256, (rows / rpb) * nchunk);
  if (acc_dtype == MMDIT_BF16 && dacc_dtype == MMDIT_BF16) hipLaunchKernelGGL((gate_res_bwd_kernel<bf16_t, bf16_t>), grid, dim3(256), 0, s, dy, (const bf16_t*)acc, gate, ld_gate, d, rpb, nchunk, (bf16_t*)dacc, dgate, ld_dgate, dbias, ld_dbias);
  else if (acc_dtype == MMDIT_F32 && dacc_dtype == MMDIT_F32) hipLaunchKernelGGL((gate_res_bwd_kernel<float, float>), grid, dim3(256), 0, s, dy, (const float*)acc, gate, ld_gate, d, rpb, nchunk, (float*)dacc, dgate, ld_dgate, dbias, ld_dbias);
  else return MMDIT_ERR_DTYPE;
  return mmdit_launch_status();
}

namespace {
template <typename T>
__global__ __launch_bounds__(256) void flow_loss_partial_kernel(const float* __restrict__ v, const T* __restrict__ x0, const T* __restrict__ eps, int64_t n8, float coef2,
                                                                float* __restrict__ dv, float* __restrict__ partials) {
  float s = 0.f;
  for (int64_t i = (int64_t)blockIdx.x * 256 + threadIdx.x; i < n8; i += (int64_t)gridDim.x * 256) {
    float a[8], b[8], c[8], g[8];
    ld8(v + i * 8, a);
    ld8(x0 + i * 8, b);
    ld8(eps + i * 8, c);
#pragma unroll
    for (int e = 0; e < 8; e++) {
      float lab = c[e] - b[e];
      if (sizeof(T) == 2) lab = bf2f(f2bf(lab));
      const float d = a[e] - lab;
      s += d * d;
      g[e] = coef2 * d;
    }
    if (dv) st8(dv + i * 8, g);
  }
  __shared__ float sm[4];
  s = wave_sum(s);
  if ((threadIdx.x & 63) == 0) sm[threadIdx.x >> 6] = s;
  __syncthreads();
  if (threadIdx.x == 0) partials[blockIdx.x] = ((sm[0] + sm[1]) + sm[2]) + sm[3];
}
__global__ __launch_bounds__(64) void flow_loss_final_kernel(const float* __restrict__ partials, int count, float coef, float* __restrict__ loss) {
  float s = 0.f;
  for (int i = threadIdx.x; i < count; i += 64) s += partials[i];
  s = wave_sum(s);
  if (threadIdx.x == 0) loss[0] = s * coef;
}
}

extern "C" int mmdit_flow_loss(const float* v, const void* x0, const void* eps, int in_dtype, int64_t n, float coef, float* dv, float* partials,
                               float* loss, mmdit_stream_t stream) {
  MMDIT_CHECK_ARG(v && x0 && eps && partials && loss && n > 0 && n % 8 == 0);
  const int64_t n8 = n / 8;
  const int grid = (int)((n8 + 255) / 256 < 256 ? (n8 + 255) / 256 : 256);
  hipStream_t s = (hipStream_t)stream;
  if (in_dtype == MMDIT_BF16)
    hipLaunchKernelGGL((flow_loss_partial_kernel<bf16_t>), dim3(grid), dim3(256), 0, s, v, (const bf16_t*)x0, (const bf16_t*)eps, n8, 2.f * coef, dv, partials);
  else if (in_dtype == MMDIT_F32)
    hipLaunchKernelGGL((flow_loss_partial_kernel<float>), dim3(grid), dim3(256), 0, s, v, (const float*)x0, (const float*)eps, n8, 2.f * coef, dv, partials);
  else
    return MMDIT_ERR_DTYPE;
  hipLaunchKernelGGL(flow_loss_final_kernel, dim3(1), dim3(64), 0, s, (const float*)partials, grid, coef, loss);
  return mmdit_launch_status();
}

extern "C" int mmdit_colsum(const void* x, int dtype, int rows, int cols, int64_t ld, float* out, mmdit_stream_t stream) {
  MMDIT_CHECK_ARG(x && out && rows > 0 && cols > 0 && cols % 8 == 0 && ld % 8 == 0);
  hipStream_t s = (hipStream_t)stream;
  const int rch = rows <= 256 ? 8 : CO_RCH;
  dim3 grid((cols + 1023) / 1024, (rows + rch - 1) / rch);
  if (dtype == MMDIT_BF16) hipLaunchKernelGGL((colsum_kernel<bf16_t>), grid, dim3(256), 0, s, (const bf16_t*)x, rows, cols, ld, out, rch);
  else if (dtype == MMDIT_F32) hipLaunchKernelGGL((colsum_kernel<float>), grid, dim3(256), 0, s, (const float*)x, rows, cols, ld, out, rch);
  else return MMDIT_ERR_DTYPE;
  return mmdit_launch_status();
}

namespace {
template <typename TI>
__global__ __launch_bounds__(256) void fp8_amax_kernel(const TI* __restrict__ x, int64_t n8, float* __restrict__ amax) {
  float m = 0.f;
  for (int64_t i = (int64_t)blockIdx.x * 256 + threadIdx.x; i < n8; i += (int64_t)gridDim.x * 256) {
    float v[8];
    ld8(x + i * 8, v);
#pragma unroll
    for (int e = 0; e < 8; e++) m = fmaxf(m, fabsf(v[e]));
  }
  __shared__ float sm[4];
  m = wave_max(m);
  if ((threadIdx.x & 63) == 0) sm[threadIdx.x >> 6] = m;
  __syncthreads();
  if (threadIdx.x == 0) atomicMax((unsigned int*)amax, __float_as_uint(fmaxf(fmaxf(sm[0], sm[1]), fmaxf(sm[2], sm[3]))));
}
template <typename TI>
__global__ __launch_bounds__(256) void fp8_quant_kernel(const TI* __restrict__ x, int64_t n8, const float* __restrict__ amax, uint2* __restrict__ q, float* __restrict__ scale) {
  const float a = fmaxf(amax[0], 1e-12f), s = 448.f / a;
  if (blockIdx.x == 0 && threadIdx.x == 0) scale[0] = a / 448.f;
  for (int64_t i = (int64_t)blockIdx.x * 256 + threadIdx.x; i < n8; i += (int64_t)gridDim.x * 256) {
    float v[8];
    ld8(x + i * 8, v);
#pragma unroll
    for (int e = 0; e < 8; e++) v[e] = fminf(fmaxf(v[e] * s, -448.f), 448.f);
    int lo = 0, hi = 0;
    lo = __builtin_amdgcn_cvt_pk_fp8_f32(v[0], v[1], lo, false);
    lo = __builtin_amdgcn_cvt_pk_fp8_f32(v[2], v[3], lo, true);
    hi = __builtin_amdgcn_cvt_pk_fp8_f32(v[4], v[5], hi, false);
    hi = __builtin_amdgcn_cvt_pk_fp8_f32(v[6], v[7], hi, true);
    q[i] = make_uint2((unsigned)lo, (unsigned)hi);
  }
}
template <typename TI>
__global__ __launch_bounds__(256) void fp8_quant_delayed_kernel(const TI* __restrict__ x, int64_t n8, float* __restrict__ state, int phase, float margin,
                                                                uint2* __restrict__ q) {
  __shared__ float sm[4];
  const float a = fmaxf(state[phase % 3] * margin, 1e-12f), s = 448.f / a;
  if (blockIdx.x == 0 && threadIdx.x == 0) { state[3] = a / 448.f; state[(phase + 2) % 3] = 0.f; }
  float m = 0.f;
  for (int64_t i = (int64_t)blockIdx.x * 256 + threadIdx.x; i < n8; i += (int64_t)gridDim.x * 256) {
    float v[8];
    ld8(x + i * 8, v);
#pragma unroll
    for (int e = 0; e < 8; e++) { m = fmaxf(m, fabsf(v[e])); v[e] = fminf(fmaxf(v[e] * s, -448.f), 448.f); }
    int lo = 0, hi = 0;
    lo = __builtin_amdgcn_cvt_pk_fp8_f32(v[0], v[1], lo, false);
    lo = __builtin_amdgcn_cvt_pk_fp8_f32(v[2], v[3], lo, true);
    hi = __builtin_amdgcn_cvt_pk_fp8_f32(v[4], v[5], hi, false);
    hi = __builtin_amdgcn_cvt_pk_fp8_f32(v[6], v[7], hi, true);
    q[i] = make_uint2((unsigned)lo, (unsigned)hi);
  }
  m = wave_max(m);
  if ((threadIdx.x & 63) == 0) sm[threadIdx.x >> 6] = m;
  __syncthreads();
  if (threadIdx.x == 0) atomicMax((unsigned int*)(state + (phase + 1) % 3), __float_as_uint(fmaxf(fmaxf(sm[0], sm[1]), fmaxf(sm[2], sm[3]))));
}
}

namespace {
template <typename TI>
__global__ __launch_bounds__(256) void mxfp8_quant_kernel(const TI* __restrict__ x, int rows, int K, int64_t ldx, uint4* __restrict__ q, unsigned char* __restrict__ sc) {
  const int bpr = K >> 5;
  const int64_t t = (int64_t)blockIdx.x * 256 + threadIdx.x;
  if (t >= (int64_t)rows * bpr) return;
  const int row = (int)(t / bpr), blk = (int)(t - (int64_t)row * bpr);
  const TI* src = x + (int64_t)row * ldx + blk * 32;
  float v[32];
#pragma unroll
  for (int c = 0; c < 4; c++) ld8(src + c * 8, *(float(*)[8])(v + c * 8));
  float amax = 0.f;
#pragma unroll
  for (int e = 0; e < 32; e++) amax = fmaxf(amax, fabsf(v[e]));
  float inv;
  const int ex = mx_exponent(amax, inv);
  unsigned w[8];
#pragma unroll
  for (int c = 0; c < 8; c++) w[c] = mx_pack4(v + 4 * c, inv);
  uint4* dst = q + ((int64_t)row * K + blk * 32) / 16;
  dst[0] = make_uint4(w[0], w[1], w[2], w[3]);
  dst[1] = make_uint4(w[4], w[5], w[6], w[7]);
  sc[mx_scale_index(row, blk, rows)] = (unsigned char)(ex + 127);
}
}

extern "C" int mmdit_mxfp8_quantize(const void* x, int x_dtype, int rows, int K, int64_t ldx, void* q_fp8, void* scales, mmdit_stream_t stream) {
  MMDIT_CHECK_ARG(x && q_fp8 && scales && rows > 0 && K > 0 && K % 64 == 0 && ldx >= K && ldx % 8 == 0);
  hipStream_t s = (hipStream_t)stream;
  const int64_t nblk = (int64_t)rows * (K / 32);
  const dim3 grid((unsigned)((nblk + 255) / 256));
  if (x_dtype == MMDIT_F32) hipLaunchKernelGGL((mxfp8_quant_kernel<float>), grid, dim3(256), 0, s, (const float*)x, rows, K, ldx, (uint4*)q_fp8, (unsigned char*)scales);
  else if (x_dtype == MMDIT_BF16) hipLaunchKernelGGL((mxfp8_quant_kernel<bf16_t>), grid, dim3(256), 0, s, (const bf16_t*)x, rows, K, ldx, (uint4*)q_fp8, (unsigned char*)scales);
  else return MMDIT_ERR_DTYPE;
  return mmdit_launch_status();
}

extern "C" int mmdit_fp8_quantize_delayed(const void* x, int x_dtype, int64_t n, float* state, int phase, float margin, void* q_fp8, mmdit_stream_t stream) {
  MMDIT_CHECK_ARG(x && state && q_fp8 && n > 0 && n % 8 == 0 && phase >= 0 && margin >= 1.f);
  hipStream_t s = (hipStream_t)stream;
  const int g0 = grid_cap(n / 8, 256);
  dim3 grid(g0 > 1024 ? 1024 : g0);
  if (x_dtype == MMDIT_F32) hipLaunchKernelGGL((fp8_quant_delayed_kernel<float>), grid, dim3(256), 0, s, (const float*)x, n / 8, state, phase, margin, (uint2*)q_fp8);
  else if (x_dtype == MMDIT_BF16) hipLaunchKernelGGL((fp8_quant_delayed_kernel<bf16_t>), grid, dim3(256), 0, s, (const bf16_t*)x, n / 8, state, phase, margin, (uint2*)q_fp8);
  else return MMDIT_ERR_DTYPE;
  return mmdit_launch_status();
}

extern "C" int mmdit_fp8_amax(const void* x, int x_dtype, int64_t n, float* amax, mmdit_stream_t stream) {
  MMDIT_CHECK_ARG(x && amax && n > 0 && n % 8 == 0);
  hipStream_t s = (hipStream_t)stream;
  const int g0 = grid_cap(n / 8, 256);
  dim3 grid(g0 > 1024 ? 1024 : g0);
  if (x_dtype == MMDIT_F32) hipLaunchKernelGGL((fp8_amax_kernel<float>), grid, dim3(256), 0, s, (const float*)x, n / 8, amax);
  else if (x_dtype == MMDIT_BF16) hipLaunchKernelGGL((fp8_amax_kernel<bf16_t>), grid, dim3(256), 0, s, (const bf16_t*)x, n / 8, amax);
  else return MMDIT_ERR_DTYPE;
  return mmdit_launch_status();
}
extern "C" int mmdit_fp8_quantize(const void* x, int x_dtype, int64_t n, const float* amax, void* q_fp8, float* scale, mmdit_stream_t stream) {
  MMDIT_CHECK_ARG(x && amax && q_fp8 && scale && n > 0 && n % 8 == 0);
  hipStream_t s = (hipStream_t)stream;
  dim3 grid(grid_cap(n / 8, 256));
  if (x_dtype == MMDIT_F32) hipLaunchKernelGGL((fp8_quant_kernel<float>), grid, dim3(256), 0, s, (const float*)x, n / 8, amax, (uint2*)q_fp8, scale);
  else if (x_dtype == MMDIT_BF16) hipLaunchKernelGGL((fp8_quant_kernel<bf16_t>), grid, dim3(256), 0, s, (const bf16_t*)x, n / 8, amax, (uint2*)q_fp8, scale);
  else return MMDIT_ERR_DTYPE;
  return mmdit_launch_status();
}

extern "C" int mmdit_cast(const void* src, int src_dtype, void* dst, int dst_dtype, int64_t n, mmdit_stream_t stream) {
  MMDIT_CHECK_ARG(src && dst && n > 0);
  hipStream_t s = (hipStream_t)stream;
  dim3 grid(grid_cap(n / 8 + 1, 256));
  if (src_dtype == MMDIT_F32 && dst_dtype == MMDIT_BF16) hipLaunchKernelGGL((cast_kernel<float, bf16_t>), grid, dim3(256), 0, s, (const float*)src, (bf16_t*)dst, n);
  else if (src_dtype == MMDIT_BF16 && dst_dtype == MMDIT_F32) hipLaunchKernelGGL((cast_kernel<bf16_t, float>), grid, dim3(256), 0, s, (const bf16_t*)src, (float*)dst, n);
  else return MMDIT_ERR_DTYPE;
  return mmdit_launch_status();
}

template <bool TO_TOKENS>
static int patch_dispatch(const void* src, int sdt, void* dst, int ddt, int batch, int ch, int H, int W, mmdit_stream_t stream) {
  MMDIT_CHECK_ARG(src && dst && batch > 0 && ch > 0 && H > 0 && W > 0 && H % 2 == 0 && W % 2 == 0);
  hipStream_t s = (hipStream_t)stream;
  dim3 grid(grid_cap((int64_t)batch * ch * H * (W / 2), 256));
#define PK(TI, TO) hipLaunchKernelGGL((patch_kernel<TI, TO, TO_TOKENS>), grid, dim3(256), 0, s, (const TI*)src, (TO*)dst, batch, ch, H, W)
  if (sdt == MMDIT_F32 && ddt == MMDIT_F32) PK(float, float);
  else if (sdt == MMDIT_F32 && ddt == MMDIT_BF16) PK(float, bf16_t);
  else if (sdt == MMDIT_BF16 && ddt == MMDIT_BF16) PK(bf16_t, bf16_t);
  else if (sdt == MMDIT_BF16 && ddt == MMDIT_F32) PK(bf16_t, float);
  else return MMDIT_ERR_DTYPE;
#undef PK
  return mmdit_launch_status();
}
extern "C" int mmdit_patchify(const void* img, int img_dtype, int batch, int ch, int H, int W, void* tokens, int tok_dtype, mmdit_stream_t st) {
  return patch_dispatch<true>(img, img_dtype, tokens, tok_dtype, batch, ch, H, W, st);
}
extern "C" int mmdit_unpatchify(const void* tokens, int tok_dtype, int batch, int ch, int H, int W, void* img, int img_dtype, mmdit_stream_t st) {
  return patch_dispatch<false>(tokens, tok_dtype, img, img_dtype, batch, ch, H, W, st);
}

extern "C" int mmdit_time_embed_fwd(const float* t, const float* time_scale, const float* denom, int batch, int dim, void* out, int out_dtype, mmdit_stream_t stream) {
  MMDIT_CHECK_ARG(t && time_scale && denom && out && batch > 0 && dim > 0 && dim % 2 == 0);
  hipStream_t s = (hipStream_t)stream;
  dim3 grid((dim + 255) / 256, batch);
  if (out_dtype == MMDIT_BF16) hipLaunchKernelGGL((time_embed_fwd_kernel<bf16_t>), grid, dim3(256), 0, s, t, time_scale, denom, batch, dim, (bf16_t*)out);
  else if (out_dtype == MMDIT_F32) hipLaunchKernelGGL((time_embed_fwd_kernel<float>), grid, dim3(256), 0, s, t, time_scale, denom, batch, dim, (float*)out);
  else return MMDIT_ERR_DTYPE;
  return mmdit_launch_status();
}
extern "C" int mmdit_time_embed_bwd(const void* dout, int dout_dtype, const float* t, const float* time_scale, const float* denom, int batch, int dim, float* dtime_scale, mmdit_stream_t stream) {
  MMDIT_CHECK_ARG(dout && t && time_scale && denom && dtime_scale && batch > 0 && dim > 0 && dim % 2 == 0);
  hipStream_t s = (hipStream_t)stream;
  if (dout_dtype == MMDIT_BF16) hipLaunchKernelGGL((time_embed_bwd_kernel<bf16_t>), dim3(batch), dim3(256), 0, s, (const bf16_t*)dout, t, time_scale, denom, batch, dim, dtime_scale);
  else if (dout_dtype == MMDIT_F32) hipLaunchKernelGGL((time_embed_bwd_kernel<float>), dim3(batch), dim3(256), 0, s, (const float*)dout, t, time_scale, denom, batch, dim, dtime_scale);
  else return MMDIT_ERR_DTYPE;
  return mmdit_launch_status();
}
```

### stable-diffusion-3-from-scratch_amd/engine.py

```python
from types import SimpleNamespace as NS

import torch

from . import _lib, ops
from ._lib import ACT_SILU, PREC_BF16, PREC_SPLIT

F32 = torch.float32
BF16 = torch.bfloat16


class Mode:
    def __init__(self, fast: bool = True, fp8: bool = False, mx: bool = False):
        self.fast = fast
        self.fp8 = fp8
        self.mx = mx
        self.T = BF16 if fast else F32
        self.prec = PREC_BF16 if fast else PREC_SPLIT
        self.attn_mode = 0 if fast else 1
        self._q = {}

    def act(self, t):
        return t if t.dtype == self.T else ops.cast(t, self.T)


# ... 183 lines not shown
    return [(pres[i], yps[i], mods[i]) for i in range(nb)], pre_all


class Pending:
    __slots__ = ("x", "acc", "gate", "rpb")

    def __init__(self, x, acc=None, gate=None, rpb=0):
        self.x, self.acc, self.gate, self.rpb = x, acc, gate, rpb

    def value(self):
        return self.x if self.acc is None else ops.gate_residual_fwd(self.x, self.acc, self.gate, self.rpb)


def _norm(m, P, scale, shift, rpb, mx=False):
    pend = isinstance(P, Pending) and P.acc is not None
    if mx:
        return ops.ln_modulate_fwd_mx(P.x if isinstance(P, Pending) else P, scale, shift, rpb, acc=P.acc if pend else None, gate=P.gate if pend else None)
    if pend:
        return ops.ln_modulate_fwd_res(P.x, P.acc, P.gate, scale, shift, rpb, m.T)
    x = P.x if isinstance(P, Pending) else P
    return (x,) + ops.ln_modulate_fwd(x, scale, shift, rpb, m.T)


def _norm_pair(m, a, b, mx=False):
    pend = [isinstance(P, Pending) and P.acc is not None for P, *_ in (a, b)]
    dev = (a[0].x if isinstance(a[0], Pending) else a[0]).device
    if mx or pend[0] != pend[1] or dev.type != "cuda" or not _LN_PAIR:
        return _norm(m, *a, mx=mx), _norm(m, *b, mx=mx)
    args = []
    for (P, scale, shift, rpb), pe in zip((a, b), pend):
        d = dict(x=P.x if isinstance(P, Pending) else P, scale=scale, shift=shift, rpb=rpb)
        if pe:
            d.update(acc=P.acc, gate=P.gate)
        args.append(d)
    ra, rb = ops.ln_modulate_fwd_pair(args[0], args[1], m.T)
    return ra, rb


def _ln_bwd_pair(a, b):
    ga, gb = a.get("gated") is not None, b.get("gated") is not None
    if ga != gb or not a["x"].is_cuda or not _LN_PAIR:
        return [ops.ln_modulate_bwd(p["dout"], p["x"], p["mean"], p["rstd"], p["scale"], p["dres"], p["rpb"], p["dscale"], p["dshift"], gated=p.get("gated")) for p in (a, b)]
    return ops.ln_modulate_bwd_pair(a, b)


def block_fwd(m, w, X, C, y, dims, rope, cond=None, keep=True, lazy=False):
    B, N, Mt, H, d = dims
    S, dev = N + Mt, (X.x if isinstance(X, Pending) else X).device
    both = not w.last
    sv = NS(y=y)
    if cond is not None:
        sv.pre, sv.yp, sv.mod = cond
    else:
        sv.pre = torch.empty((B, d), dtype=F32, device=dev)
        sv.yp = _gemm(m, y, w.Wy, bias=w.by, act=ACT_SILU, aux=sv.pre, out_dtype=m.T)
        sv.mod = _gemm(m, sv.yp, w.Wmod, out_dtype=F32)
    ms = _mod_views(sv.mod, d, w.last)
    mxf = (m.mx and not keep and dev.type == "cuda" and d % 128 == 0 and not w.mlp_x.gelu
           and w.mlp_x.hidden % 128 == 0 and (w.last or (not w.mlp_c.gelu and w.mlp_c.hidden % 128 == 0)) and _MX_FUSE)

    (sv.X, sv.ln1x, sv.mu1x, sv.rs1x), (sv.C, sv.ln1c, sv.mu1c, sv.rs1c) = _norm_pair(m, (X, ms.scale1x, ms.shift1x, N), (C, ms.scale1c, ms.shift1c, Mt), mx=mxf)
    sv.Q = torch.empty((B, H, S, 64), dtype=BF16, device=dev)
    sv.K, sv.V = torch.empty_like(sv.Q), torch.empty_like(sv.Q)
    fused = None
    if _QKV_FUSE and m.fast and dev.type == "cuda" and m.T == BF16 and (not m.fp8 or mxf) and d == H * 64:
        qp = [dict(A=sv.ln1x, B=w.Wqkv_x, out_dtype=m.T, precision=m.prec), dict(A=sv.ln1c, B=w.Wqkv_c, out_dtype=m.T, precision=m.prec)]
        if mxf:
            qq = [_to_fp8(m, p) for p in qp]
            qp = qq if all(x is not p for x, p in zip(qq, qp)) else None
        if qp is not None:
            fused = ops.gemm_qkv_norm_rope(qp, [(w.wq_x, w.wk_x, rope[0], rope[1], N, 0), (w.wq_c, w.wk_c, None, None, Mt, N)], H, S, sv.Q, sv.K, sv.V, raw=_QKV_RAW or not mxf)
    if fused is not None:
        sv.qkv_x, sv.qkv_c = fused
    else:
        sv.qkv_x, sv.qkv_c = _group(m, [dict(A=sv.ln1x, B=w.Wqkv_x, out_dtype=m.T), dict(A=sv.ln1c, B=w.Wqkv_c, out_dtype=m.T)], fp8=True)
    if fused is not None:
        pass
    elif _LN_PAIR and dev.type == "cuda":
        ops.qk_norm_rope_fwd_pair((sv.qkv_x, w.wq_x, w.wk_x, rope[0], rope[1], N, 0), (sv.qkv_c, w.wq_c, w.wk_c, None, None, Mt, N), B, H, S, sv.Q, sv.K, sv.V)
    else:
        ops.qk_norm_rope_fwd(sv.qkv_x, w.wq_x, w.wk_x, rope[0], rope[1], B, N, H, S, 0, sv.Q, sv.K, sv.V)
        ops.qk_norm_rope_fwd(sv.qkv_c, w.wq_c, w.wk_c, None, None, B, Mt, H, S, N, sv.Q, sv.K, sv.V)
    if mxf:
        sv.Oxa, sv.Oca = ops.attn_fwd_mx(sv.Q, sv.K, sv.V, N, 64 ** -0.5)
    else:
        sv.Ox, sv.Oc, sv.lse = ops.attn_fwd(sv.Q, sv.K, sv.V, N, 64 ** -0.5, m.attn_mode)
        sv.Oxa = m.act(sv.Ox.view(B * N, d))
        if both:
            sv.Oca = m.act(sv.Oc.view(B * Mt, d))

    probs = [dict(A=sv.Oxa, B=w.Wo_x, out_dtype=m.T)]
    if both:
        probs.append(dict(A=sv.Oca, B=w.Wo_c, out_dtype=m.T))
    outs = _group(m, probs, fp8=True)
    sv.acc_ox = outs[0]
    if both:
        sv.acc_oc = outs[1]
        (sv.X1, sv.ln2x, sv.mu2x, sv.rs2x), (sv.C1, sv.ln2c, sv.mu2c, sv.rs2c) = _norm_pair(
            m, (Pending(sv.X, sv.acc_ox, ms.gate1x, N), ms.scale2x, ms.shift2x, N), (Pending(sv.C, sv.acc_oc, ms.gate1c, Mt), ms.scale2c, ms.shift2c, Mt), mx=mxf)
    else:
        sv.C1 = sv.C
        sv.X1, sv.ln2x, sv.mu2x, sv.rs2x = _norm(m, Pending(sv.X, sv.acc_ox, ms.gate1x, N), ms.scale2x, ms.shift2x, N, mx=mxf)
    fuse = _FUSE_SWIGLU and m.fast and dev.type == "cuda" and not w.mlp_x.gelu and w.mlp_x.hidden % 128 == 0 and d % (128 if m.fp8 else 64) == 0

    def up(xn, mw, rows):
        if fuse and mxf:
            q, sc = ops._mx_buffers(rows, mw.hidden, dev)
            return dict(A=xn, B=mw.Wup, bias=mw.bup, act=ops.ACT_SWIGLU, out=q, out_scales=sc)
        if fuse:
            return dict(A=xn, B=mw.Wup, bias=mw.bup, act=ops.ACT_SWIGLU, aux=torch.empty((rows, 2 * mw.hidden), dtype=m.T, device=dev) if keep else None)
        return dict(A=xn, B=mw.Wup, bias=mw.bup, out_dtype=m.T)

    probs = [up(sv.ln2x, w.mlp_x, B * N)]
    if both:
        probs.append(up(sv.ln2c, w.mlp_c, B * Mt))
    outs = _group(m, probs, fp8=True)
    pre = [p.get("aux") for p in probs]
    if fuse and mxf:
        outs = [ops.MxAct(p["out"], p["out_scales"]) for p in probs]
    if fuse:
        sv.gu_x, sv.h_x = pre[0], outs[0]
    else:
        sv.gu_x = outs[0]
        sv.h_x = ops.swiglu_fwd_mx(sv.gu_x, w.mlp_x.hidden) if mxf else ops.mlp_act_fwd(sv.gu_x, w.mlp_x.hidden, w.mlp_x.gelu)
    probs = [dict(A=sv.h_x, B=w.mlp_x.Wdown, bias=w.mlp_x.bdown, out_dtype=m.T)]
    if both:
        if fuse:
            sv.gu_c, sv.h_c = pre[1], outs[1]
        else:
            sv.gu_c = outs[1]
            sv.h_c = ops.swiglu_fwd_mx(sv.gu_c, w.mlp_c.hidden) if mxf else ops.mlp_act_fwd(sv.gu_c, w.mlp_c.hidden, w.mlp_c.gelu)
        probs.append(dict(A=sv.h_c, B=w.mlp_c.Wdown, bias=w.mlp_c.bdown, out_dtype=m.T))
    outs = _group(m, probs, fp8=True)
    sv.acc_mx = outs[0]
    X2 = Pending(sv.X1, sv.acc_mx, ms.gate2x, N)
    if both:
        sv.acc_mc = outs[1]
        C2 = Pending(sv.C1, sv.acc_mc, ms.gate2c, Mt)
    else:
        C2 = Pending(sv.C1)
    if not lazy:
        X2, C2 = X2.value(), C2.value()
    return X2, C2, sv


_LN_PAIR = _lib.experiment("MMDIT_LN_PAIR", "1") != "0"
_MX_FUSE = _lib.experiment("MMDIT_MX_FUSE", "1") != "0"
_BATCH_WMOD = _lib.experiment("MMDIT_BATCH_WMOD", "1") != "0"
_QKV_FUSE = _lib.experiment("MMDIT_QKV_FUSE", "1") != "0"
_QKV_RAW = _lib.experiment("MMDIT_QKV_RAW", "0") == "1"
_QK_FUSE = _lib.experiment("MMDIT_ATTN_QK_FUSE", "1") != "0"
_FUSE_SWIGLU_BWD = _lib.experiment("MMDIT_FUSE_SWIGLU_BWD", "1") != "0"
_FUSE_GATE = _lib.experiment("MMDIT_FUSE_GATE", "1") != "0"


def _qk_bwd_two_pass(m, w, sv, g, dOx, dOc, dims, rope, dev):
    B, N, Mt, H, d = dims
    S = N + Mt
    dQ, dK, dV = ops.attn_bwd(sv.Q, sv.K, sv.V, sv.Ox, sv.Oc, dOx, dOc, sv.lse, N, 64 ** -0.5, m.T)
    if _LN_PAIR and dev.type == "cuda":
        return ops.qk_norm_rope_bwd_pair(dQ, dK, dV, (sv.qkv_x, w.wq_x, w.wk_x, rope[0], rope[1], N, 0, g.wq_x, g.wk_x),
                                         (sv.qkv_c, w.wq_c, w.wk_c, None, None, Mt, N, g.wq_c, g.wk_c), B, H, S, m.T)
    dqkv_x = ops.qk_norm_rope_bwd(dQ, dK, dV, sv.qkv_x, w.wq_x, w.wk_x, rope[0], rope[1], B, N, H, S, 0, g.wq_x, g.wk_x, m.T)
    dqkv_c = ops.qk_norm_rope_bwd(dQ, dK, dV, sv.qkv_c, w.wq_c, w.wk_c, None, None, B, Mt, H, S, N, g.wq_c, g.wk_c, m.T)
    return dqkv_x, dqkv_c


def block_bwd_begin(m, w, sv, dims, dev, defer_cond=False):
    B, N, Mt, H, d = dims
    both = not w.last
    ms = _mod_views(sv.mod, d, w.last)
    g = NS(mlp_x=NS(), mlp_c=NS() if both else None)
    hx = sv.gu_x.shape[1]
    nb = 2 if both else 1
    shapes = [(nb * d,), (hx,), (64,), (64,), (64,), (64,)] + ([(sv.gu_c.shape[1],)] if both else []) + ([] if defer_cond else [(d,)])
    npar = len(shapes)
    shapes += [tuple(sv.mod.shape), (B, nb * d)]
    zs, small_arena = _zeros_views(shapes, dev, prefix=npar)
    st = NS(g=g, ms=ms, zs=zs, npar=npar, small_arena=small_arena, both=both)
    st.bdown, g.mlp_x.bup, g.wq_x, g.wk_x, g.wq_c, g.wk_c = zs[:6]
    if not defer_cond:
        g.by = zs[npar - 1]
    st.dmod, st.bpart = zs[npar], zs[npar + 1]
    g.mlp_x.bdown = st.bdown[:d]
    if both:
        g.mlp_c.bdown, g.mlp_c.bup = st.bdown[d:], zs[6]
    st.dms = _mod_views(st.dmod, d, w.last)
    st.req_x = (sv.acc_mx, ms.gate2x, st.dms.gate2x, st.bpart[:, :d])
    st.req_c = (sv.acc_mc, ms.gate2c, st.dms.gate2c, st.bpart[:, d:]) if both else None
    return st


def block_bwd(m, w, sv, dX2, dC2, dy_acc, dims, rope, defer_cond=False, st=None, dacc=None, nxt=None, defer_wmod=False):
    B, N, Mt, H, d = dims
    S, dev = N + Mt, dX2.device
    both = not w.last
    if st is None:
        st = block_bwd_begin(m, w, sv, dims, dev, defer_cond)
    g, ms, dms, bpart, bdown, dmod = st.g, st.ms, st.dms, st.bpart, st.bdown, st.dmod
    pending = []
    fuse = _FUSE_GATE

    def defer(ns, name, dY, Xa):
        pending.append((lambda o, ns=ns, name=name: setattr(ns, name, o), _wg(dY, Xa)))

    dacc_x = dacc[0] if dacc is not None else ops.gate_residual_bwd(dX2, sv.acc_mx, ms.gate2x, N, dms.gate2x, bpart[:, :d], m.T)
    probs = [dict(A=dacc_x, B=w.mlp_x.Wdown, b_kmajor=True, out_dtype=m.T)]
    if both:
        dacc_c = dacc[1] if dacc is not None else ops.gate_residual_bwd(dC2, sv.acc_mc, ms.gate2c, Mt, dms.gate2c, bpart[:, d:], m.T)
        probs.append(dict(A=dacc_c, B=w.mlp_c.Wdown, b_kmajor=True, out_dtype=m.T))
    ops.colsum(bpart, bdown)
    dgu = None
    if (_FUSE_SWIGLU_BWD and m.fast and dev.type == "cuda" and m.prec == PREC_BF16 and dacc_x.dtype == BF16 and sv.gu_x.dtype == BF16
            and not w.mlp_x.gelu and (not both or not w.mlp_c.gelu)):
        fp = [dict(A=dacc_x, B=w.mlp_x.Wdown, aux=sv.gu_x, dbias=g.mlp_x.bup, precision=m.prec)]
        if both:
            fp.append(dict(A=dacc_c, B=w.mlp_c.Wdown, aux=sv.gu_c, dbias=g.mlp_c.bup, precision=m.prec))
        dgu = ops.gemm_swiglu_bwd(fp)
    if dgu is None:
        dh = _group(m, probs)
    defer(g.mlp_x, "Wdown", dacc_x, sv.h_x)
    pair = both and _LN_PAIR and dev.type == "cuda" and w.mlp_x.hidden == w.mlp_c.hidden and w.mlp_x.gelu == w.mlp_c.gelu
    if dgu is not None:
        dgu_x, dgu_c = dgu[0], (dgu[1] if both else None)
    elif pair:
        dgu_x, dgu_c = ops.mlp_act_bwd_pair((dh[0], sv.gu_x, g.mlp_x.bup), (dh[1], sv.gu_c, g.mlp_c.bup), w.mlp_x.hidden, w.mlp_x.gelu)
    else:
        dgu_x = ops.mlp_act_bwd(dh[0], sv.gu_x, w.mlp_x.hidden, g.mlp_x.bup, w.mlp_x.gelu)
    probs = [dict(A=dgu_x, B=w.mlp_x.Wup, b_kmajor=True, out_dtype=m.T)]
    defer(g.mlp_x, "Wup", dgu_x, sv.ln2x)
    if both:
        defer(g.mlp_c, "Wdown", dacc_c, sv.h_c)
        if not pair and dgu is None:
            dgu_c = ops.mlp_act_bwd(dh[1], sv.gu_c, w.mlp_c.hidden, g.mlp_c.bup, w.mlp_c.gelu)
        probs.append(dict(A=dgu_c, B=w.mlp_c.Wup, b_kmajor=True, out_dtype=m.T))
        defer(g.mlp_c, "Wup", dgu_c, sv.ln2c)
    dln2 = _group(m, probs)

    ax = dict(dout=dln2[0], x=sv.X1, mean=sv.mu2x, rstd=sv.rs2x, scale=ms.scale2x, dres=dX2, rpb=N, dscale=dms.scale2x, dshift=dms.shift2x)
    if fuse:
        ax["gated"] = (sv.acc_ox, ms.gate1x, dms.gate1x, None)
    dC1 = dC2
    if both:
        ac = dict(dout=dln2[1], x=sv.C1, mean=sv.mu2c, rstd=sv.rs2c, scale=ms.scale2c, dres=dC2, rpb=Mt, dscale=dms.scale2c, dshift=dms.shift2c)
        if fuse:
            ac["gated"] = (sv.acc_oc, ms.gate1c, dms.gate1c, None)
        rx, rc = _ln_bwd_pair(ax, ac)
    else:
        rx = ops.ln_modulate_bwd(ax["dout"], ax["x"], ax["mean"], ax["rstd"], ax["scale"], ax["dres"], N, ax["dscale"], ax["dshift"], gated=ax.get("gated"))
    if fuse:
        dX1, dacc_x = rx
    else:
        dX1 = rx
        dacc_x = ops.gate_residual_bwd(dX1, sv.acc_ox, ms.gate1x, N, dms.gate1x, None, m.T)
    probs = [dict(A=dacc_x, B=w.Wo_x, b_kmajor=True, out_dtype=BF16)]
    defer(g, "Wo_x", dacc_x, sv.Oxa)
    if both:
        if fuse:
            dC1, dacc_c = rc
        else:
            dC1 = rc
            dacc_c = ops.gate_residual_bwd(dC1, sv.acc_oc, ms.gate1c, Mt, dms.gate1c, None, m.T)
        probs.append(dict(A=dacc_c, B=w.Wo_c, b_kmajor=True, out_dtype=BF16))
        defer(g, "Wo_c", dacc_c, sv.Oca)
    dO = _group(m, probs)
    dOx, dOc = dO[0], (dO[1] if both else None)

    if _QK_FUSE and m.fast and dev.type == "cuda" and ops.attn_bwd_qk_ok(sv.Q, N, sv.qkv_x) and g.wq_x.data_ptr() + 768 == g.wk_c.data_ptr():
        dqkv_x, dqkv_c = ops.attn_bwd_qk(sv.Q, sv.K, sv.V, sv.Ox, sv.Oc, dOx, dOc, sv.lse, N, 64 ** -0.5, sv.qkv_x, sv.qkv_c, w.wq_x, w.wk_x, w.wq_c, w.wk_c,
                                         rope[0], rope[1], torch.as_strided(g.wq_x, (256,), (1,)))
    else:
        dqkv_x, dqkv_c = _qk_bwd_two_pass(m, w, sv, g, dOx, dOc, dims, rope, dev)
    dln1 = _group(m, [dict(A=dqkv_x, B=w.Wqkv_x, b_kmajor=True, out_dtype=m.T), dict(A=dqkv_c, B=w.Wqkv_c, b_kmajor=True, out_dtype=m.T)])
    defer(g, "Wqkv_x", dqkv_x, sv.ln1x)
    defer(g, "Wqkv_c", dqkv_c, sv.ln1c)
    nacc = None
    ax = dict(dout=dln1[0], x=sv.X, mean=sv.mu1x, rstd=sv.rs1x, scale=ms.scale1x, dres=dX1, rpb=N, dscale=dms.scale1x, dshift=dms.shift1x)
    ac = dict(dout=dln1[1], x=sv.C, mean=sv.mu1c, rstd=sv.rs1c, scale=ms.scale1c, dres=dC1, rpb=Mt, dscale=dms.scale1c, dshift=dms.shift1c)
    if nxt is not None and fuse:
        ax["gated"], ac["gated"] = nxt.req_x, nxt.req_c
        (dX, nax), (dC, nac) = _ln_bwd_pair(ax, ac)
        nacc = (nax, nac)
    else:
        dX, dC = _ln_bwd_pair(ax, ac)

    dmod_a = m.act(dmod)
    if defer_cond:
        if not defer_wmod:
            defer(g, "Wmod", dmod_a, sv.yp)
        dy_acc = dmod_a
    else:
        defer(g, "Wmod", dmod_a, sv.yp)
        dyp = _dgrad(m, dmod_a, w.Wmod, F32, **({"split_k": 16} if m.fast else {}))
        dpre = ops.silu_bwd(dyp, sv.pre, m.T, g.by)
        dy_acc = _dgrad(m, dpre, w.Wy, F32, residual=dy_acc)
        defer(g, "Wy", dpre, sv.y)

    wg_arena = _wgrad_flush(m, pending)
    g.arenas = [wg_arena, st.small_arena] if wg_arena is not None else None
    if nxt is not None:
        return dX, dC, dy_acc, g, nacc
    return dX, dC, dy_acc, g


def text_fwd(m, W, c):
    B, Mt = c.shape[0], c.shape[1]
    d = W.dim
    cn1, cn2 = ops.text_rmsnorm_fwd(c, W.wn1, W.wn2, W.s1, W.s2, W.split, m.T)
    c1, c2 = _group(m, [dict(A=cn1, B=W.Wc1, out_dtype=F32), dict(A=cn2, B=W.Wc2, out_dtype=F32)])
    C = torch.cat([c1.view(B, W.split, d), c2.view(B, Mt - W.split, d)], dim=1).view(B * Mt, d)
    return C, cn1, cn2


def model_fwd(m, W, x_t, t, c, c_pooled, rope, keep=True, C=None):
    B, Cin, Hh, Ww = x_t.shape
    d, H = W.dim, W.heads
    N, Mt = (Hh // 2) * (Ww // 2), c.shape[1]
    dims = (B, N, Mt, H, d)
    sv = NS(dims=dims, img=(B, Cin, Hh, Ww), c=c, t=t)
    sv.pe = ops.time_embed_fwd(t, W.time_scale, W.denom, m.T)
    temb = _gemm(m, sv.pe, W.Wt, out_dtype=F32)
    sv.cp = m.act(c_pooled)
    sv.y = _gemm(m, sv.cp, W.Wcond, residual=temb, out_dtype=m.T)

    if C is None:
        C, sv.cn1, sv.cn2 = text_fwd(m, W, c)

    sv.patches = ops.patchify(x_t, m.T)
    sv.X0 = _gemm(m, sv.patches, W.Wpatch, out_dtype=m.T)
    X = _gemm(m, sv.X0, W.Wpe, bias=W.bpe, out_dtype=F32)

    sv.blocks = []
    conds, sv.pre_all = cond_fwd_all(m, W.blocks, sv.y)
    for wb, cond in zip(W.blocks, conds):
        X, C, bs = block_fwd(m, wb, X, C, sv.y, dims, rope, cond, keep, lazy=True)
        sv.blocks.append(bs)

    sv.modo = _gemm(m, sv.y, W.Wmod_out, out_dtype=F32)
    sv.Xf, sv.lnf, sv.muf, sv.rsf = _norm(m, X, sv.modo[:, d:], sv.modo[:, :d], N)
    Z = _gemm(m, sv.lnf, W.Wout, bias=W.bout, out_dtype=F32)
    v = ops.unpatchify(Z, B, Cin, Hh, Ww, F32)
    return v, sv


def _grad_tensors(g):
    out = []
    for v in vars(g).values():
        if isinstance(v, NS):
            out += _grad_tensors(v)
        elif torch.is_tensor(v):
            out.append(v)
    return out


def _set_grad_tensors(g, new, pos=0):
    for k, v in list(vars(g).items()):
        if isinstance(v, NS):
            pos = _set_grad_tensors(v, new, pos)
        elif torch.is_tensor(v):
            setattr(g, k, new[pos])
            pos += 1
    return pos


def model_bwd(m, W, sv, dv, rope, on_grads=None):
    B, N, Mt, H, d = sv.dims
    _, Cin, Hh, Ww = sv.img
    dev = dv.device
    if dev.type == "cuda":
        ops.zero_pool_begin(dev)
    g = NS()
    pending = []

    def defer(name, dY, Xa):
        pending.append((lambda o, name=name: setattr(g, name, o), _wg(dY, Xa)))

    dZ = ops.patchify(dv.contiguous(), m.T)
    g.bout = ops.zeros(W.Wout.shape[0], dev)
    ops.colsum(dZ, g.bout)
    dlnf = _dgrad(m, dZ, W.Wout, m.T)
    defer("Wout", dZ, sv.lnf)
    dmodo = ops.zeros(sv.modo.shape, dev) if sv.modo.dtype == F32 else torch.zeros_like(sv.modo)
    nblk = len(W.blocks)
    sts = [None] * nblk
    sts[nblk - 1] = block_bwd_begin(m, W.blocks[-1], sv.blocks[-1], sv.dims, dev, defer_cond=True)
    dacc = None
    if _FUSE_GATE:
        dX, dax = ops.ln_modulate_bwd(dlnf, sv.Xf, sv.muf, sv.rsf, sv.modo[:, d:], None, N, dmodo[:, d:], dmodo[:, :d], gated=sts[-1].req_x)
        dacc = (dax, None)
    else:
        dX = ops.ln_modulate_bwd(dlnf, sv.Xf, sv.muf, sv.rsf, sv.modo[:, d:], None, N, dmodo[:, d:], dmodo[:, :d])
    dmodo_a = m.act(dmodo)
    dy_acc = _dgrad(m, dmodo_a, W.Wmod_out, F32, **({"split_k": 4} if m.fast else {}))
    defer("Wmod_out", dmodo_a, sv.y)

    dC = None
    g.blocks = [None] * nblk
    dmods = [None] * nblk
    yps = [None] * nblk
    batch_wmod = on_grads is None and _BATCH_WMOD
    for i in range(nblk - 1, -1, -1):
        if i > 0:
            sts[i - 1] = block_bwd_begin(m, W.blocks[i - 1], sv.blocks[i - 1], sv.dims, dev, defer_cond=True)
            dX, dC, dmods[i], g.blocks[i], dacc = block_bwd(m, W.blocks[i], sv.blocks[i], dX, dC, None, sv.dims, rope, defer_cond=True,
                                                            st=sts[i], dacc=dacc, nxt=sts[i - 1], defer_wmod=batch_wmod)
        else:
            dX, dC, dmods[i], g.blocks[i] = block_bwd(m, W.blocks[i], sv.blocks[i], dX, dC, None, sv.dims, rope, defer_cond=True, st=sts[i], dacc=dacc,
                                                      defer_wmod=batch_wmod)
        sts[i] = None
        yps[i] = sv.blocks[i].yp
        sv.blocks[i] = None
        if on_grads is not None:
            repl = on_grads(_grad_tensors(g.blocks[i]), _wg_streams.get(dev), g.blocks[i].arenas)
            if repl is not None:
                _set_grad_tensors(g.blocks[i], repl)

    dyp_all = ops.zeros((nblk * B, d), dev)
    by_all = ops.zeros((nblk, d), dev)
    for i0 in range(0, nblk, 12):
        _group(m, [dict(A=dmods[i], B=W.blocks[i].Wmod, b_kmajor=True, out=dyp_all[i * B:(i + 1) * B], **({"split_k": 4} if m.fast else {}))
                   for i in range(i0, min(nblk, i0 + 12))])
    dpre_all = ops.silu_bwd(dyp_all, sv.pre_all, m.T, by_all, rows_per_bias=B)
    dyc = torch.empty((nblk + 1, B, d), dtype=F32, device=dev)
    dyc[nblk].copy_(dy_acc)
    for i0 in range(0, nblk, 12):
        _group(m, [dict(A=dpre_all[i * B:(i + 1) * B], B=W.blocks[i].Wy, b_kmajor=True, out=dyc[i]) for i in range(i0, min(nblk, i0 + 12))])
    dy_acc = dyc.sum(0)
    late = []
    for i in range(nblk):
        g.blocks[i].by = by_all[i]
        pending.append((lambda o, i=i: setattr(g.blocks[i], "Wy", o), _wg(dpre_all[i * B:(i + 1) * B], sv.y)))
        late += [(i, "by"), (i, "Wy")]
        if batch_wmod:
            pending.append((lambda o, i=i: setattr(g.blocks[i], "Wmod", o), _wg(dmods[i], yps[i])))

    g.bpe = ops.zeros(d, dev)
    ops.colsum(dX, g.bpe)
    dX_a = m.act(dX)
    dX0 = _dgrad(m, dX_a, W.Wpe, m.T)
    defer("Wpe", dX_a, sv.X0)
    defer("Wpatch", dX0, sv.patches)

    dCv = dC.view(B, Mt, d)
    dc1 = m.act(dCv[:, :W.split].reshape(B * W.split, d))
    dc2 = m.act(dCv[:, W.split:].reshape(B * (Mt - W.split), d))
    dcn1, dcn2 = _group(m, [dict(A=dc1, B=W.Wc1, b_kmajor=True, out_dtype=m.T), dict(A=dc2, B=W.Wc2, b_kmajor=True, out_dtype=m.T)])
    defer("Wc1", dc1, sv.cn1)
    defer("Wc2", dc2, sv.cn2)
    g.wn1, g.wn2, g.s1, g.s2 = ops.text_rmsnorm_bwd(dcn1, dcn2, sv.c, W.wn1, W.wn2, W.s1, W.s2, W.split)

    dy_a = m.act(dy_acc)
    defer("Wcond", dy_a, sv.cp)
    dpe = _dgrad(m, dy_a, W.Wt, m.T)
    defer("Wt", dy_a, sv.pe)
    g.time_scale = ops.time_embed_bwd(dpe, sv.t, W.time_scale, W.denom)
    _wgrad_flush(m, pending)
    if on_grads is not None:
        keys = [k for k, v in vars(g).items() if torch.is_tensor(v)]
        repl = on_grads([getattr(g, k) for k in keys] + [getattr(g.blocks[i], n) for i, n in late], _wg_streams.get(dev))
        if repl is not None:
            for k, t in zip(keys, repl):
                setattr(g, k, t)
            for (i, n), t in zip(late, repl[len(keys):]):
                setattr(g.blocks[i], n, t)
    wgrad_join(dev)
    return g
```

### stable-diffusion-3-from-scratch_amd/ops.py

```python
import ctypes
import os

import torch

from . import _lib
from ._lib import ACT_NONE, ACT_SILU, ACT_SWIGLU, ACT_SWIGLU_BWD, BF16, F32, FP8, PREC_BF16, PREC_SPLIT, GemmArgs, check

_DT = {torch.float32: F32, torch.bfloat16: BF16, torch.float8_e4m3fn: FP8}

PROFILE = None
_ZERO_ALL = _lib.experiment("MMDIT_ZERO_ALL", "0") == "1"


class _ZeroPool:

    def __init__(self):
        self.buf, self.off, self.cap, self.need = None, 0, 0, 0

    def begin(self, device):
        self.cap = max(self.cap, self.need)
        self.need, self.off = 0, 0
        self.buf = torch.zeros(self.cap, dtype=torch.float32, device=device) if self.cap else None

    def take(self, numel, device):
# ... 208 lines not shown
        aux, out = q["aux"], q.get("out")
        if aux.data_ptr() % 16 or aux.stride(0) % 8 or aux.shape[-1] % 16 or (out is not None and (out.data_ptr() % 16 or out.stride(0) % 8)):
            return None
    _ensure_gemm_workspace(problems[0]["A"].device)
    arr = (GemmArgs * n)()
    outs = [_fill_gemm(arr[i], **dict(problems[i], b_kmajor=True, act=ACT_SWIGLU_BWD)) for i in range(n)]
    if PROFILE is not None:
        e0, e1 = torch.cuda.Event(enable_timing=True), torch.cuda.Event(enable_timing=True)
        e0.record()
    rc = _lib.lib().mmdit_gemm_grouped(arr, n, _s())
    if rc == _lib.ERR_SHAPE:
        return None
    check(rc, "mmdit_gemm_grouped(swiglu_bwd)")
    if PROFILE is not None:
        e1.record()
        PROFILE.append((_variant(arr, n, outs), sum(2.0 * arr[i].M * arr[i].N * arr[i].K for i in range(n)), e0, e1))
    return outs


def gemm_qkv_norm_rope(problems, streams, heads, s_total, Q, K, V, raw=True):
    n = len(problems)
    _ensure_gemm_workspace(problems[0]["A"].device)
    arr = (GemmArgs * n)()
    if raw:
        outs = [_fill_gemm(arr[i], **problems[i]) for i in range(n)]
    else:
        for i in range(n):
            N_ = problems[i]["B"].shape[0]
            _fill_gemm(arr[i], **dict(problems[i], out=torch.empty((1, N_), dtype=problems[i].get("out_dtype") or torch.bfloat16, device=problems[i]["A"].device)))
            arr[i].C = None
        outs = [None] * n
    qk = (_lib.QkEpilogue * n)()
    for i, (wq, wk, rc, rs, tokens, tok0) in enumerate(streams):
        qk[i].wq, qk[i].wk, qk[i].rope_cos, qk[i].rope_sin, qk[i].tokens, qk[i].tok0 = _p(wq), _p(wk), _p(rc), _p(rs), int(tokens), int(tok0)
    L = _lib.lib()
    if PROFILE is not None:
        e0, e1 = torch.cuda.Event(enable_timing=True), torch.cuda.Event(enable_timing=True)
        e0.record()
    rc = L.mmdit_gemm_qkv_norm_rope(arr, qk, n, int(heads), int(s_total), _p(Q), _p(K), _p(V), _s())
    if rc == _lib.ERR_SHAPE:
        return None
    check(rc, "mmdit_gemm_qkv_norm_rope")
    if PROFILE is not None:
        e1.record()
        on8 = arr[0].a_dtype == _lib.FP8 or bool(L.mmdit_gemm_get_claiming())
        PROFILE.append((("gemm8_kernel<256,0,0,bf16>+qk" if on8 else "gemm_wide_kernel<2,4,5,2,0>+qk"), sum(2.0 * arr[i].M * arr[i].N * arr[i].K for i in range(n)), e0, e1))
    return outs


def gemm(A, B, **kw):
    return gemm_grouped([dict(A=A, B=B, **kw)])[0]


def quant_fp8(x):
    n = x.numel()
    buf = torch.zeros(2, dtype=torch.float32, device=x.device)
    q = torch.empty(x.shape, dtype=torch.float8_e4m3fn, device=x.device)
    L = _lib.lib()
    check(L.mmdit_fp8_amax(_p(_c(x)), _dt(x), n, _p(buf), _s()), "mmdit_fp8_amax")
    check(L.mmdit_fp8_quantize(_p(x), _dt(x), n, _p(buf), _p(q), _p(buf[1:]), _s()), "mmdit_fp8_quantize")
    return q, buf[1:]


class MxAct:
    __slots__ = ("q", "sc")

    def __init__(self, q, sc):
        self.q, self.sc = q, sc

    @property
    def shape(self):
        return self.q.shape

    def dequant(self):
        rows, K = self.q.shape
        e = mx_scales_to_rows(self.sc, rows, K).to(torch.int32) - 127
        return (self.q.float().view(rows, K // 32, 32) * torch.ldexp(torch.ones((), device=self.q.device), e).unsqueeze(-1)).view(rows, K)


def mx_scale_bytes(rows, K):
    return (K // 64) * ((rows + 127) // 128 * 128) * 2 + 512


def mx_scales_to_rows(sc, rows, K):
    rp = (rows + 127) // 128 * 128
    v = sc[:(K // 64) * rp * 2].view(K // 64, rp // 128, 32, 2, 4)
    return v.permute(1, 4, 2, 0, 3).reshape(rp, K // 32)[:rows]


def _mx_buffers(rows, K, device):
    return (torch.empty((rows, K), dtype=torch.float8_e4m3fn, device=device), torch.empty(mx_scale_bytes(rows, K), dtype=torch.uint8, device=device))


def ln_modulate_fwd_mx(x, scale, shift, rows_per_batch, acc=None, gate=None):
    rows, d = x.shape
    q, sc = _mx_buffers(rows, d, x.device)
    mean = torch.empty((rows,), dtype=torch.float32, device=x.device)
    rstd = torch.empty((rows,), dtype=torch.float32, device=x.device)
    x1 = torch.empty((rows, d), dtype=torch.float32, device=x.device) if acc is not None else x
    check(_lib.lib().mmdit_ln_modulate_fwd_mx(_p(_c(x)), _p(acc), _dt(acc) if acc is not None else BF16, _p(gate), gate.stride(0) if gate is not None else 0,
                                              _p(x1) if acc is not None else None, _p(scale), _p(shift), scale.stride(0), rows, d, rows_per_batch,
                                              _p(q), _p(sc), _p(mean), _p(rstd), _s()), "mmdit_ln_modulate_fwd_mx")
    return x1, MxAct(q, sc), mean, rstd


def swiglu_fwd_mx(gu, hidden):
    rows = gu.shape[0]
    q, sc = _mx_buffers(rows, hidden, gu.device)
    check(_lib.lib().mmdit_swiglu_fwd_mx(_p(_c(gu)), _dt(gu), rows, hidden, _p(q), _p(sc), _s()), "mmdit_swiglu_fwd_mx")
    return MxAct(q, sc)


def attn_fwd_mx(Q, K, V, n_img, scale):
    B, H, S, hd = Q.shape
    n_txt = S - n_img
    qx, sx = _mx_buffers(B * n_img, H * hd, Q.device)
    qc, scc = _mx_buffers(B * n_txt, H * hd, Q.device) if n_txt else (None, None)
    check(_lib.lib().mmdit_attn_fwd_mx(_p(Q), _p(K), _p(V), B, H, S, n_img, float(scale), _p(qx), _p(qc), _p(sx), _p(scc), _s()), "mmdit_attn_fwd_mx")
    return MxAct(qx, sx), (MxAct(qc, scc) if n_txt else None)


def quant_mxfp8(x):
    rows, K = x.shape
    q = torch.empty((rows, K), dtype=torch.float8_e4m3fn, device=x.device)
    sc = torch.empty(mx_scale_bytes(rows, K), dtype=torch.uint8, device=x.device)
    check(_lib.lib().mmdit_mxfp8_quantize(_p(x), _dt(x), rows, K, x.stride(0), _p(q), _p(sc), _s()), "mmdit_mxfp8_quantize")
    return q, sc


class Fp8Site:

    def __init__(self, margin=1.5):
        self.state, self.phase, self.margin = None, 0, margin

    def quantise(self, x):
        L = _lib.lib()
        q = torch.empty(x.shape, dtype=torch.float8_e4m3fn, device=x.device)
        if self.state is None:
            self.state = torch.zeros(4, dtype=torch.float32, device=x.device)
            check(L.mmdit_fp8_amax(_p(_c(x)), _dt(x), x.numel(), _p(self.state), _s()), "mmdit_fp8_amax")
        check(L.mmdit_fp8_quantize_delayed(_p(_c(x)), _dt(x), x.numel(), _p(self.state), self.phase, float(self.margin if self.phase else 1.0),
                                           _p(q), _s()), "mmdit_fp8_quantize_delayed")
        self.phase += 1
        return q, self.state[3:]


def cast(src, dtype, out=None):
    if out is None:
        out = torch.empty(src.shape, dtype=dtype, device=src.device)
    check(_lib.lib().mmdit_cast(_p(_c(src)), _dt(src), _p(_c(out)), _dt(out), src.numel(), _s()), "mmdit_cast")
    return out


_CAST_TABLES = {}


def cast_multi(pairs):
    import numpy as np
    dev = pairs[0][0].device
    key = tuple((s.data_ptr(), d.data_ptr(), s.numel()) for s, d in pairs)
    t = _CAST_TABLES.get(key)
    if t is None:
        for s, d in pairs:
            if s.dtype != torch.float32 or d.dtype != torch.bfloat16 or not s.is_contiguous() or not d.is_contiguous() or s.numel() != d.numel() or d.device != dev:
                raise RuntimeError("cast_multi: contiguous fp32 sources and bf16 destinations of equal size on one device")
        rec = np.array(key, dtype=np.int64).reshape(-1)
        ct = np.concatenate([np.full((n + _lib.ADAMW_CHUNK - 1) // _lib.ADAMW_CHUNK, i, dtype=np.int32) for i, (_, _, n) in enumerate(key)])
        co = np.concatenate([np.arange(0, n, _lib.ADAMW_CHUNK, dtype=np.int64) for _, _, n in key])
        host = [torch.from_numpy(a).pin_memory() for a in (rec, ct, co)]
        if len(_CAST_TABLES) >= 8:
            _CAST_TABLES.pop(next(iter(_CAST_TABLES)))
        t = _CAST_TABLES[key] = dict(host=host, dev=[h.to(dev, non_blocking=True) for h in host], n=len(ct))
    check(_lib.lib().mmdit_cast_multi(_p(t["dev"][0]), _p(t["dev"][1]), _p(t["dev"][2]), t["n"], _s()), "mmdit_cast_multi")


def ln_modulate_fwd(x, scale, shift, rows_per_batch, out_dtype):
    rows, d = x.shape
    out = torch.empty((rows, d), dtype=out_dtype, device=x.device)
    mean = torch.empty((rows,), dtype=torch.float32, device=x.device)
    rstd = torch.empty((rows,), dtype=torch.float32, device=x.device)
    check(_lib.lib().mmdit_ln_modulate_fwd(_p(_c(x)), _p(scale), _p(shift), scale.stride(0), rows, d, rows_per_batch,
                                           _p(out), _dt(out), _p(mean), _p(rstd), _s()), "mmdit_ln_modulate_fwd")
    return out, mean, rstd


def ln_modulate_fwd_res(x, acc, gate, scale, shift, rows_per_batch, out_dtype):
    rows, d = x.shape
    x1 = torch.empty((rows, d), dtype=torch.float32, device=x.device)
    out = torch.empty((rows, d), dtype=out_dtype, device=x.device)
    mean = torch.empty((rows,), dtype=torch.float32, device=x.device)
    rstd = torch.empty((rows,), dtype=torch.float32, device=x.device)
    check(_lib.lib().mmdit_ln_modulate_fwd_res(_p(_c(x)), _p(_c(acc)), _dt(acc), _p(gate), gate.stride(0), _p(x1), _p(scale), _p(shift), scale.stride(0),
                                               rows, d, rows_per_batch, _p(out), _dt(out), _p(mean), _p(rstd), _s()), "mmdit_ln_modulate_fwd_res")
    return x1, out, mean, rstd


def ln_modulate_fwd_pair(pa, pb, out_dtype):
    res = pa.get("acc") is not None
    assert (pb.get("acc") is not None) == res
    d = pa["x"].shape[1]
    probs, outs = (_lib.LnFwdProblem * 2)(), []
    for q, p in zip(probs, (pa, pb)):
        x = _c(p["x"])
        rows = x.shape[0]
        dev = x.device
        x1 = torch.empty((rows, d), dtype=torch.float32, device=dev) if res else x
        out = torch.empty((rows, d), dtype=out_dtype, device=dev)
        mean = torch.empty((rows,), dtype=torch.float32, device=dev)
        rstd = torch.empty((rows,), dtype=torch.float32, device=dev)
        q.x, q.scale, q.shift, q.ld_mod, q.rows, q.rows_per_batch = _p(x), _p(p["scale"]), _p(p["shift"]), p["scale"].stride(0), rows, p["rpb"]
        q.out, q.mean, q.rstd = _p(out), _p(mean), _p(rstd)
        if res:
            acc = _c(p["acc"])
            q.acc, q.gate, q.ld_gate, q.x_out = _p(acc), _p(p["gate"]), p["gate"].stride(0), _p(x1)
            p["_keep"] = (x, acc)
        else:
            p["_keep"] = (x,)
        outs.append((x1, out, mean, rstd))
    acc_dt = _dt(pa["acc"]) if res else _DT[out_dtype]
    check(_lib.lib().mmdit_ln_modulate_fwd_pair(ctypes.byref(probs[0]), ctypes.byref(probs[1]), d, acc_dt, _DT[out_dtype], _s()), "mmdit_ln_modulate_fwd_pair")
    return outs


def ln_modulate_bwd_pair(pa, pb):
    gated = pa.get("gated") is not None
    assert (pb.get("gated") is not None) == gated
    d = pa["x"].shape[1]
    probs, outs, keep = (_lib.LnBwdProblem * 2)(), [], []
    for q, p in zip(probs, (pa, pb)):
        dout, x = _c(p["dout"]), p["x"]
        rows, dev = x.shape[0], x.device
        dx = torch.empty((rows, d), dtype=torch.float32, device=dev)
        q.dout, q.x, q.mean, q.rstd, q.scale, q.ld_mod = _p(dout), _p(x), _p(p["mean"]), _p(p["rstd"]), _p(p["scale"]), p["scale"].stride(0)
        q.dres, q.rows, q.rows_per_batch = _p(p.get("dres")), rows, p["rpb"]
        q.dx, q.dscale, q.dshift, q.ld_dmod = _p(dx), _p(p["dscale"]), _p(p["dshift"]), p["dscale"].stride(0)
        keep.append(dout)
        if gated:
            acc, gate, dgate, dbias = p["gated"]
            acc = _c(acc)
            dacc = torch.empty((rows, d), dtype=acc.dtype, device=dev)
            q.acc, q.gate, q.ld_gate, q.dacc, q.dgate, q.ld_dgate = _p(acc), _p(gate), gate.stride(0), _p(dacc), _p(dgate), dgate.stride(0)
            q.dbias, q.ld_dbias = _p(dbias), (dbias.stride(0) if dbias is not None else 0)
            keep.append(acc)
            outs.append((dx, dacc))
        else:
            outs.append(dx)
    check(_lib.lib().mmdit_ln_modulate_bwd_pair(ctypes.byref(probs[0]), ctypes.byref(probs[1]), d, _dt(pa["dout"]), _s()), "mmdit_ln_modulate_bwd_pair")
    return outs


def gate_residual_fwd(x, acc, gate, rows_per_batch):
    rows, d = x.shape
    out = torch.empty((rows, d), dtype=torch.float32, device=x.device)
    check(_lib.lib().mmdit_gate_residual_fwd(_p(_c(x)), _p(_c(acc)), _dt(acc), _p(gate), gate.stride(0), rows, d, rows_per_batch, _p(out), _s()), "mmdit_gate_residual_fwd")
    return out


def ln_modulate_bwd(dout, x, mean, rstd, scale, dres, rows_per_batch, dscale, dshift, gated=None):
    rows, d = x.shape
    dx = torch.empty((rows, d), dtype=torch.float32, device=x.device)
    if gated is None:
        check(_lib.lib().mmdit_ln_modulate_bwd(_p(_c(dout)), _dt(dout), _p(x), _p(mean), _p(rstd), _p(scale), scale.stride(0), _p(dres),
                                               rows, d, rows_per_batch, _p(dx), _p(dscale), _p(dshift), dscale.stride(0), _s()), "mmdit_ln_modulate_bwd")
        return dx
    acc, gate, dgate, dbias = gated
    dacc = torch.empty((rows, d), dtype=acc.dtype, device=x.device)
    check(_lib.lib().mmdit_ln_modulate_bwd_gated(_p(_c(dout)), _dt(dout), _p(x), _p(mean), _p(rstd), _p(scale), scale.stride(0), _p(dres),
                                                 rows, d, rows_per_batch, _p(dx), _p(dscale), _p(dshift), dscale.stride(0),
                                                 _p(_c(acc)), _dt(acc), _p(gate), gate.stride(0), _p(dacc), _p(dgate), dgate.stride(0),
                                                 _p(dbias), dbias.stride(0) if dbias is not None else 0, _s()), "mmdit_ln_modulate_bwd_gated")
    return dx, dacc


def text_rmsnorm_fwd(x, w1, w2, s1, s2, split, out_dtype):
    batch, tokens, d = x.shape
    out1 = torch.empty((batch * split, d), dtype=out_dtype, device=x.device)
    out2 = torch.empty((batch * (tokens - split), d), dtype=out_dtype, device=x.device)
    check(_lib.lib().mmdit_text_rmsnorm_fwd(_p(_c(x)), _dt(x), _p(w1), _p(w2), _p(s1), _p(s2), batch, tokens, split, d,
                                            _p(out1), _p(out2), _dt(out1), _s()), "mmdit_text_rmsnorm_fwd")
    return out1, out2


def text_rmsnorm_bwd(dout1, dout2, x, w1, w2, s1, s2, split):
    batch, tokens, d = x.shape
    dw1, dw2 = zeros(w1.shape, w1.device), zeros(w2.shape, w2.device)
    ds1, ds2 = zeros(s1.shape, s1.device), zeros(s2.shape, s2.device)
    check(_lib.lib().mmdit_text_rmsnorm_bwd(_p(_c(dout1)), _p(_c(dout2)), _dt(dout1), _p(x), _dt(x), _p(w1), _p(w2), _p(s1), _p(s2),
                                            batch, tokens, split, d, _p(dw1), _p(dw2), _p(ds1), _p(ds2), _s()), "mmdit_text_rmsnorm_bwd")
    return dw1, dw2, ds1, ds2


def qk_norm_rope_fwd(qkv, wq, wk, rope_cos, rope_sin, batch, tokens, heads, s_total, tok0, Q, K, V):
    check(_lib.lib().mmdit_qk_norm_rope_fwd(_p(_c(qkv)), _dt(qkv), _p(wq), _p(wk), _p(rope_cos), _p(rope_sin), batch, tokens, heads, s_total, tok0,
                                            _p(Q), _p(K), _p(V), _s()), "mmdit_qk_norm_rope_fwd")


def qk_norm_rope_bwd(dQ, dK, dV, qkv, wq, wk, rope_cos, rope_sin, batch, tokens, heads, s_total, tok0, dwq, dwk, out_dtype):
    dqkv = torch.empty(qkv.shape, dtype=out_dtype, device=qkv.device)
    check(_lib.lib().mmdit_qk_norm_rope_bwd(_p(dQ), _p(dK), _p(dV), _dt(dQ), _p(qkv), _dt(qkv), _p(wq), _p(wk), _p(rope_cos), _p(rope_sin),
                                            batch, tokens, heads, s_total, tok0, _p(dqkv), _dt(dqkv), _p(dwq), _p(dwk), _s()), "mmdit_qk_norm_rope_bwd")
    return dqkv


def qk_norm_rope_fwd_pair(img, txt, batch, heads, s_total, Q, K, V):
    probs, keep = (_lib.QkProblem * 2)(), []
    for q, (qkv, wq, wk, rc, rs, tokens, tok0) in zip(probs, (img, txt)):
        qkv = _c(qkv)
        keep.append(qkv)
        q.qkv, q.wq, q.wk, q.rope_cos, q.rope_sin, q.tokens, q.tok0 = _p(qkv), _p(wq), _p(wk), _p(rc), _p(rs), tokens, tok0
    check(_lib.lib().mmdit_qk_norm_rope_fwd_pair(ctypes.byref(probs[0]), ctypes.byref(probs[1]), _dt(img[0]), batch, heads, s_total, _p(Q), _p(K), _p(V), _s()),
          "mmdit_qk_norm_rope_fwd_pair")


def qk_norm_rope_bwd_pair(dQ, dK, dV, img, txt, batch, heads, s_total, out_dtype):
    probs, outs = (_lib.QkProblem * 2)(), []
    for q, (qkv, wq, wk, rc, rs, tokens, tok0, dwq, dwk) in zip(probs, (img, txt)):
        dqkv = torch.empty(qkv.shape, dtype=out_dtype, device=qkv.device)
        q.qkv, q.wq, q.wk, q.rope_cos, q.rope_sin, q.tokens, q.tok0 = _p(qkv), _p(wq), _p(wk), _p(rc), _p(rs), tokens, tok0
        q.dqkv, q.dwq, q.dwk = _p(dqkv), _p(dwq), _p(dwk)
        outs.append(dqkv)
    check(_lib.lib().mmdit_qk_norm_rope_bwd_pair(ctypes.byref(probs[0]), ctypes.byref(probs[1]), _p(dQ), _p(dK), _p(dV), _dt(dQ), _dt(img[0]), _DT[out_dtype],
                                                 batch, heads, s_total, _s()), "mmdit_qk_norm_rope_bwd_pair")
    return outs


def attn_fwd(Q, K, V, n_img, scale, mode):
    batch, heads, S, hd = Q.shape
    if hd != 64:
        raise RuntimeError("attention kernels are built for head_dim 64 (the reference's dim = 64*num_heads convention)")
    D = heads * hd
    Ox = torch.empty((batch, n_img, D), dtype=torch.bfloat16, device=Q.device)
    Oc = torch.empty((batch, S - n_img, D), dtype=torch.bfloat16, device=Q.device) if S > n_img else None
    lse = torch.empty((batch, heads, S), dtype=torch.float32, device=Q.device)
    check(_lib.lib().mmdit_attn_fwd(_p(Q), _p(K), _p(V), batch, heads, S, n_img, float(scale), mode, _p(Ox), _p(Oc), _p(lse), _s()), "mmdit_attn_fwd")
    return Ox, Oc, lse


def attn_bwd(Q, K, V, Ox, Oc, dOx, dOc, lse, n_img, scale, out_dtype):
    batch, heads, S, hd = Q.shape
    delta = torch.empty((batch, heads, S), dtype=torch.float32, device=Q.device)
    dQ = torch.empty(Q.shape, dtype=out_dtype, device=Q.device)
    dK = torch.empty(Q.shape, dtype=out_dtype, device=Q.device)
    dV = torch.empty(Q.shape, dtype=out_dtype, device=Q.device)
    check(_lib.lib().mmdit_attn_bwd(_p(Q), _p(K), _p(V), _p(Ox), _p(Oc), _p(_c(dOx)), _p(_c(dOc)), _p(lse), _p(delta), batch, heads, S, n_img,
                                    float(scale), _p(dQ), _p(dK), _p(dV), _dt(dQ), _s()), "mmdit_attn_bwd")
    return dQ, dK, dV


def attn_bwd_qk(Q, K, V, Ox, Oc, dOx, dOc, lse, n_img, scale, qkv_x, qkv_c, wq_x, wk_x, wq_c, wk_c, rope_cos, rope_sin, dw4):
    batch, heads, S, hd = Q.shape
    delta = torch.empty((batch, heads, S), dtype=torch.float32, device=Q.device)
    dqkv_x = torch.empty(qkv_x.shape, dtype=torch.bfloat16, device=Q.device)
    dqkv_c = torch.empty(qkv_c.shape, dtype=torch.bfloat16, device=Q.device)
    if dw4.dtype != torch.float32 or dw4.numel() != 256 or not dw4.is_contiguous():
        raise RuntimeError("attn_bwd_qk: dw4 is the contiguous fp32 [wq_x | wk_x | wq_c | wk_c] accumulator (256)")
    check(_lib.lib().mmdit_attn_bwd_qk(_p(Q), _p(K), _p(V), _p(Ox), _p(Oc), _p(_c(dOx)), _p(_c(dOc)), _p(lse), _p(delta), batch, heads, S, n_img, float(scale),
                                       _p(_c(qkv_x)), _p(_c(qkv_c)), _p(wq_x), _p(wk_x), _p(wq_c), _p(wk_c), _p(rope_cos), _p(rope_sin),
                                       _p(dqkv_x), _p(dqkv_c), _p(dw4), _s()), "mmdit_attn_bwd_qk")
    return dqkv_x, dqkv_c


def attn_bwd_qk_ok(Q, n_img, qkv_x):
    return Q.is_cuda and Q.shape[-1] == 64 and n_img % 32 == 0 and n_img < Q.shape[2] and qkv_x.dtype == torch.bfloat16


def mlp_act_fwd(gu, hidden, gelu=False):
    rows = gu.shape[0]
    h = torch.empty((rows, hidden), dtype=gu.dtype, device=gu.device)
    fn = _lib.lib().mmdit_gelu_fwd if gelu else _lib.lib().mmdit_swiglu_fwd
    check(fn(_p(_c(gu)), _p(h), _dt(gu), rows, hidden, _s()), "mmdit_mlp_act_fwd")
    return h


def mlp_act_bwd(dh, gu, hidden, dbias, gelu=False):
    rows = gu.shape[0]
    dgu = torch.empty_like(gu)
    fn = _lib.lib().mmdit_gelu_bwd if gelu else _lib.lib().mmdit_swiglu_bwd
    check(fn(_p(_c(dh)), _p(gu), _p(dgu), _dt(gu), rows, hidden, _p(dbias), _s()), "mmdit_mlp_act_bwd")
    return dgu


def mlp_act_bwd_pair(a, b, hidden, gelu=False):
    probs, outs, keep = (_lib.MlpBwdProblem * 2)(), [], []
    for q, (dh, gu, dbias) in zip(probs, (a, b)):
        dh = _c(dh)
        dgu = torch.empty_like(gu)
        q.dh, q.gu, q.dgu, q.rows, q.dbias = _p(dh), _p(gu), _p(dgu), gu.shape[0], _p(dbias)
        keep.append(dh)
        outs.append(dgu)
    check(_lib.lib().mmdit_mlp_act_bwd_pair(ctypes.byref(probs[0]), ctypes.byref(probs[1]), _dt(a[1]), hidden, int(gelu), _s()), "mmdit_mlp_act_bwd_pair")
    return outs


def silu_bwd(dy, pre, out_dtype, dbias, rows_per_bias=0):
    rows, cols = pre.shape
    dpre = torch.empty((rows, cols), dtype=out_dtype, device=pre.device)
    check(_lib.lib().mmdit_silu_bwd(_p(_c(dy)), _dt(dy), _p(pre), _p(dpre), _dt(dpre), rows, cols, _p(dbias), int(rows_per_bias), _s()), "mmdit_silu_bwd")
    return dpre


def gate_residual_bwd(dy, acc, gate, rows_per_batch, dgate, dbias, out_dtype):
    rows, d = dy.shape
    dacc = torch.empty((rows, d), dtype=out_dtype, device=dy.device)
    ld_dbias = dbias.stride(0) if (dbias is not None and dbias.dim() == 2) else 0
    check(_lib.lib().mmdit_gate_residual_bwd(_p(_c(dy)), _p(acc), _dt(acc), _p(gate), gate.stride(0), rows, d, rows_per_batch,
                                             _p(dacc), _dt(dacc), _p(dgate), dgate.stride(0), _p(dbias), ld_dbias, _s()), "mmdit_gate_residual_bwd")
    return dacc


def flow_loss(v, x0, eps, accumulation_steps=1, need_grad=True):
    n = v.numel()
    if v.dtype != torch.float32 or x0.dtype != eps.dtype or x0.numel() != n or eps.numel() != n or n % 8:
        raise RuntimeError("flow_loss: v fp32, x0 and eps of one dtype and v's size, numel % 8 == 0")
    loss = torch.empty((), dtype=torch.float32, device=v.device)
    part = torch.empty(256, dtype=torch.float32, device=v.device)
    dv = torch.empty(v.shape, dtype=torch.float32, device=v.device) if need_grad else None
    check(_lib.lib().mmdit_flow_loss(_p(_c(v)), _p(_c(x0)), _p(_c(eps)), _dt(x0), n, 1.0 / (n * accumulation_steps), _p(dv), _p(part), _p(loss), _s()), "mmdit_flow_loss")
    return loss, dv


def colsum(x, out):
    rows, cols = x.shape
    check(_lib.lib().mmdit_colsum(_p(x), _dt(x), rows, cols, x.stride(0), _p(out), _s()), "mmdit_colsum")
    return out


def patchify(img, out_dtype):
    batch, ch, H, W = img.shape
    tokens = torch.empty((batch * (H // 2) * (W // 2), ch * 4), dtype=out_dtype, device=img.device)
    check(_lib.lib().mmdit_patchify(_p(_c(img)), _dt(img), batch, ch, H, W, _p(tokens), _dt(tokens), _s()), "mmdit_patchify")
    return tokens


def unpatchify(tokens, batch, ch, H, W, out_dtype):
    img = torch.empty((batch, ch, H, W), dtype=out_dtype, device=tokens.device)
    check(_lib.lib().mmdit_unpatchify(_p(_c(tokens)), _dt(tokens), batch, ch, H, W, _p(img), _dt(img), _s()), "mmdit_unpatchify")
    return img


def time_embed_fwd(t, time_scale, denom, out_dtype):
    batch, dim = t.shape[0], denom.shape[0]
    out = torch.empty((batch, dim), dtype=out_dtype, device=t.device)
    check(_lib.lib().mmdit_time_embed_fwd(_p(t), _p(time_scale), _p(denom), batch, dim, _p(out), _dt(out), _s()), "mmdit_time_embed_fwd")
    return out


def time_embed_bwd(dout, t, time_scale, denom):
    batch, dim = t.shape[0], denom.shape[0]
    dts = zeros(time_scale.shape, time_scale.device)
    check(_lib.lib().mmdit_time_embed_bwd(_p(_c(dout)), _dt(dout), _p(t), _p(time_scale), _p(denom), batch, dim, _p(dts), _s()), "mmdit_time_embed_bwd")
    return dts


def vae_nchw_to_nhwc(x, c_padded, scale=1.0, shift=0.0):
    B, C, H, W = x.shape
    out = torch.empty((B, H, W, c_padded), dtype=torch.bfloat16, device=x.device)
    check(_lib.lib().mmdit_vae_nchw_to_nhwc(_p(_c(x)), _dt(x), B, C, H, W, c_padded, float(scale), float(shift), _p(out), _s()), "mmdit_vae_nchw_to_nhwc")
    return out


def vae_nhwc_to_nchw(x2d, B, C, H, W, lo=-float("inf"), hi=float("inf")):
    out = torch.empty((B, C, H, W), dtype=torch.float32, device=x2d.device)
    check(_lib.lib().mmdit_vae_nhwc_to_nchw(_p(_c(x2d)), B, C, H, W, x2d.shape[1], float(lo), float(hi), _p(out), _s()), "mmdit_vae_nhwc_to_nchw")
    return out


def vae_im2col3x3(x, mode=0):
    B, H, W, C = x.shape
    Ho, Wo = (H // 2, W // 2) if mode == 1 else (2 * H, 2 * W) if mode == 2 else (H, W)
    out = torch.empty((B * Ho * Wo, 9 * C), dtype=torch.bfloat16, device=x.device)
    check(_lib.lib().mmdit_vae_im2col3x3(_p(_c(x)), B, H, W, C, mode, _p(out), _s()), "mmdit_vae_im2col3x3")
    return out, Ho, Wo


def vae_groupnorm(x, gamma, beta, B, H, W, groups, eps, silu, padded_out=None):
    C = x.shape[1]
    sums = torch.zeros(B * groups * 2, dtype=torch.float32, device=x.device)
    out = padded_out if padded_out is not None else torch.empty((B * H * W, C), dtype=torch.bfloat16, device=x.device)
    check(_lib.lib().mmdit_vae_groupnorm(_p(_c(x)), _dt(x), _p(gamma), _p(beta), B, H, W, C, groups, float(eps), int(silu), _p(sums), _p(out),
                                         int(padded_out is not None), _s()), "mmdit_vae_groupnorm")
    return out


def vae_pad_cast(x, B, H, W, padded_out, upsample=False):
    check(_lib.lib().mmdit_vae_pad_cast(_p(_c(x)), _dt(x), B, H, W, x.shape[1], int(upsample), _p(padded_out), _s()), "mmdit_vae_pad_cast")
    return padded_out


def vae_softmax_rows(x, scale, cols=None):
    rows, ld = x.shape
    cols = ld if cols is None else cols
    out = torch.empty((rows, ld), dtype=torch.bfloat16, device=x.device)
    check(_lib.lib().mmdit_vae_softmax_rows(_p(_c(x)), rows, cols, ld, float(scale), _p(out), _s()), "mmdit_vae_softmax_rows")
    return out
```

Baseline: 2351.

## Fold backward tail ops into LN-bwd and patchify kernels, batch colsums

Adds a tail variant of the paired adaLN backward kernel. For the first block it writes dX directly as bf16, split into image and text outputs, and accumulates per-batch column sums for the patch-embed bias gradient. This skips the separate fp32 dX store, the colsum and the cast. It also fuses the output patchify with its bias colsum and adds list-based colsum and cast kernels that batch several small launches into one. The cost is extra template instantiations, extra registers in the tail kernel, and atomics in the patchify colsum.

```diff
diff --git a/include/mmdit_hip.h b/include/mmdit_hip.h
--- a/include/mmdit_hip.h
+++ b/include/mmdit_hip.h
@@ -102,6 +102,9 @@
   const void* acc; const float* gate; int64_t ld_gate; void* dacc; float* dgate; int64_t ld_dgate; float* dbias; int64_t ld_dbias;
 } mmdit_ln_bwd_problem;
 int mmdit_ln_modulate_bwd_pair(const mmdit_ln_bwd_problem* p0, const mmdit_ln_bwd_problem* p1, int d, int dout_dtype, mmdit_stream_t stream);
+typedef struct mmdit_ln_bwd_tail { void* out0; void* out1; int split; float* colsum; int64_t ld_colsum; } mmdit_ln_bwd_tail;
+int mmdit_ln_modulate_bwd_pair_tail(const mmdit_ln_bwd_problem* p0, const mmdit_ln_bwd_problem* p1, const mmdit_ln_bwd_tail* t0, const mmdit_ln_bwd_tail* t1,
+                                    int d, int dout_dtype, mmdit_stream_t stream);
 int mmdit_gate_residual_fwd(const float* x, const void* acc, int acc_dtype, const float* gate, int64_t ld_gate,
                             int rows, int d, int rows_per_batch, float* out, mmdit_stream_t stream);
 int mmdit_ln_modulate_bwd(const void* dout, int dout_dtype, const float* x, const float* mean, const float* rstd,
@@ -169,8 +172,13 @@
 
 int mmdit_colsum(const void* x, int dtype, int rows, int cols, int64_t ld, float* out, mmdit_stream_t stream);
 
+#define MMDIT_LIST_MAX 32
+typedef struct mmdit_colsum_task { const float* x; float* out; int rows, cols; int64_t ld; } mmdit_colsum_task;
+int mmdit_colsum_list(const mmdit_colsum_task* tasks, int n, mmdit_stream_t stream);
+
 int mmdit_patchify(const void* img, int img_dtype, int batch, int ch, int H, int W, void* tokens, int tok_dtype, mmdit_stream_t stream);
 int mmdit_unpatchify(const void* tokens, int tok_dtype, int batch, int ch, int H, int W, void* img, int img_dtype, mmdit_stream_t stream);
+int mmdit_patchify_colsum(const void* img, int img_dtype, int batch, int ch, int H, int W, void* tokens, int tok_dtype, float* colsum, mmdit_stream_t stream);
 
 int mmdit_time_embed_fwd(const float* t, const float* time_scale, const float* denom, int batch, int dim, void* out, int out_dtype, mmdit_stream_t stream);
 int mmdit_time_embed_bwd(const void* dout, int dout_dtype, const float* t, const float* time_scale, const float* denom, int batch, int dim, float* dtime_scale, mmdit_stream_t stream);
@@ -206,6 +214,7 @@
   int64_t numel;
 } mmdit_cast_tensor;
 int mmdit_cast_multi(const mmdit_cast_tensor* tensors, const int* chunk_tensor, const int64_t* chunk_off, int n_chunks, mmdit_stream_t stream);
+int mmdit_cast_list(const mmdit_cast_tensor* tensors, int n, mmdit_stream_t stream);
 
 #ifdef __cplusplus
 }
diff --git a/stable-diffusion-3-from-scratch_amd/_lib.py b/stable-diffusion-3-from-scratch_amd/_lib.py
--- a/stable-diffusion-3-from-scratch_amd/_lib.py
+++ b/stable-diffusion-3-from-scratch_amd/_lib.py
@@ -52,6 +52,18 @@
                 ("dx", ctypes.c_void_p), ("dscale", ctypes.c_void_p), ("dshift", ctypes.c_void_p), ("ld_dmod", ctypes.c_int64),
                 ("acc", ctypes.c_void_p), ("gate", ctypes.c_void_p), ("ld_gate", ctypes.c_int64), ("dacc", ctypes.c_void_p), ("dgate", ctypes.c_void_p),
                 ("ld_dgate", ctypes.c_int64), ("dbias", ctypes.c_void_p), ("ld_dbias", ctypes.c_int64)]
+
+
+class LnBwdTail(ctypes.Structure):
+    _fields_ = [("out0", ctypes.c_void_p), ("out1", ctypes.c_void_p), ("split", ctypes.c_int), ("colsum", ctypes.c_void_p), ("ld_colsum", ctypes.c_int64)]
+
+
+class ColsumTask(ctypes.Structure):
+    _fields_ = [("x", ctypes.c_void_p), ("out", ctypes.c_void_p), ("rows", ctypes.c_int), ("cols", ctypes.c_int), ("ld", ctypes.c_int64)]
+
+
+class CastTensor(ctypes.Structure):
+    _fields_ = [("src", ctypes.c_void_p), ("dst", ctypes.c_void_p), ("numel", ctypes.c_int64)]
 
 
 class QkProblem(ctypes.Structure):
@@ -129,6 +141,10 @@
     "mmdit_adamw_step": ([_vp, _vp, _vp, _i, _vp, _vp, _d, _d, _d, _d, _d, _vp], _i),
     "mmdit_adamw_step_dlr": ([_vp, _vp, _vp, _i, _vp, _vp, _vp, _d, _d, _d, _d, _vp], _i),
     "mmdit_cast_multi": ([_vp, _vp, _vp, _i, _vp], _i),
+    "mmdit_cast_list": ([ctypes.POINTER(CastTensor), _i, _vp], _i),
+    "mmdit_colsum_list": ([ctypes.POINTER(ColsumTask), _i, _vp], _i),
+    "mmdit_patchify_colsum": ([_vp, _i, _i, _i, _i, _i, _vp, _i, _vp, _vp], _i),
+    "mmdit_ln_modulate_bwd_pair_tail": ([ctypes.POINTER(LnBwdProblem), ctypes.POINTER(LnBwdProblem), ctypes.POINTER(LnBwdTail), ctypes.POINTER(LnBwdTail), _i, _i, _vp], _i),
 }
 ADAMW_CHUNK = 65536
 ABI_VERSION = 9
diff --git a/stable-diffusion-3-from-scratch_amd/csrc/rowops.hip b/stable-diffusion-3-from-scratch_amd/csrc/rowops.hip
--- a/stable-diffusion-3-from-scratch_amd/csrc/rowops.hip
+++ b/stable-diffusion-3-from-scratch_amd/csrc/rowops.hip
@@ -122,13 +122,16 @@
 #define MMDIT_LN_BWD_RCH 16
 #endif
 constexpr int LN_BWD_RCH = MMDIT_LN_BWD_RCH;
-template <int NITX, typename TG, typename TA, bool GATED>
+template <int NITX, typename TG, typename TA, bool GATED, bool TAIL = false>
 __device__ __forceinline__ void ln_mod_bwd_body(int block, const TG* __restrict__ dout, const float* __restrict__ x, const float* __restrict__ mean_i,
                                                 const float* __restrict__ rstd_i, const float* __restrict__ scale, int64_t ld_mod,
                                                 const float* __restrict__ dres, int d, int rpb, int nchunk,
                                                 float* __restrict__ dx, float* __restrict__ dscale, float* __restrict__ dshift, int64_t ld_dmod,
                                                 const TA* __restrict__ acc, const float* __restrict__ gate, int64_t ld_gate, TA* __restrict__ dacc,
-                                                float* __restrict__ dgate, int64_t ld_dgate, float* __restrict__ dbias, int64_t ld_dbias, int rch = LN_BWD_RCH) {
+                                                float* __restrict__ dgate, int64_t ld_dgate, float* __restrict__ dbias, int64_t ld_dbias, int rch = LN_BWD_RCH,
+                                                bf16_t* __restrict__ tb0 = nullptr, bf16_t* __restrict__ tb1 = nullptr, int tsplit = 0,
+                                                float* __restrict__ tsum = nullptr, int64_t ld_tsum = 0) {
+  static_assert(!(GATED && TAIL), "the tail variant is the plain (not gated) adaLN backward");
   constexpr int NIT = NITX < 0 ? -NITX : NITX;
   constexpr bool EXACT = NITX < 0;
   const int lane = threadIdx.x & 63, wave = threadIdx.x >> 6;
@@ -143,10 +146,15 @@
   __syncthreads();
   float ds[NIT][4], dh[NIT][4];
   float sg[GATED ? NIT : 1][4], sb[GATED ? NIT : 1][4];
+  float sx[TAIL ? NIT : 1][4];
 #pragma unroll
   for (int it = 0; it < NIT; it++) {
 #pragma unroll
     for (int e = 0; e < 4; e++) { ds[it][e] = 0.f; dh[it][e] = 0.f; }
+    if constexpr (TAIL) {
+#pragma unroll
+      for (int e = 0; e < 4; e++) sx[it][e] = 0.f;
+    }
     if constexpr (GATED) {
 #pragma unroll
       for (int e = 0; e < 4; e++) { sg[it][e] = 0.f; sb[it][e] = 0.f; }
@@ -177,6 +185,8 @@
       }
     }
     c1 = wave_sum(c1) / d; c2 = wave_sum(c2) / d;
+    bf16_t* trow = nullptr;
+    if constexpr (TAIL) trow = rl < tsplit ? tb0 + ((int64_t)b * tsplit + rl) * d : tb1 + ((int64_t)b * (rpb - tsplit) + (rl - tsplit)) * d;
 #pragma unroll
     for (int it = 0; it < NIT; it++) {
       int ch = lane + 64 * it;
@@ -185,7 +195,12 @@
         if (dres) ld4(dres + row * d + ch * 4, o); else { o[0] = o[1] = o[2] = o[3] = 0.f; }
 #pragma unroll
         for (int e = 0; e < 4; e++) o[e] += rstd * (g[it][e] - c1 - xh[it][e] * c2);
-        st4(dx + row * d + ch * 4, o);
+        if (!TAIL || dx) st4(dx + row * d + ch * 4, o);
+        if constexpr (TAIL) {
+          if (tb0) st4(trow + ch * 4, o);
+#pragma unroll
+          for (int e = 0; e < 4; e++) sx[it][e] += o[e];
+        }
         if constexpr (GATED) {
           float av[4], da[4], gt[4];
           ld4_nt(acc + row * d + ch * 4, av);
@@ -214,6 +229,9 @@
       flush(sg, dgate + (int64_t)b * ld_dgate);
       if (dbias) flush(sb, dbias + (int64_t)b * ld_dbias);
     }
+    if constexpr (TAIL) {
+      if (tsum) flush(sx, tsum + (int64_t)b * ld_tsum);
+    }
   } else {
     auto flush = [&](const float (&v)[NIT][4], float* dst) {
 #pragma unroll
@@ -231,6 +249,9 @@
       flush(sg, dgate + (int64_t)b * ld_dgate);
       if (dbias) flush(sb, dbias + (int64_t)b * ld_dbias);
     }
+    if constexpr (TAIL) {
+      if (tsum) flush(sx, tsum + (int64_t)b * ld_tsum);
+    }
   }
 }
 
@@ -249,13 +270,15 @@
   const void* dout; const float* x; const float* mean; const float* rstd; const float* scale; int64_t ld_mod; const float* dres; int rpb, nchunk;
   float* dx; float* dscale; float* dshift; int64_t ld_dmod;
   const void* acc; const float* gate; int64_t ld_gate; void* dacc; float* dgate; int64_t ld_dgate; float* dbias; int64_t ld_dbias;
+  bf16_t* tb0; bf16_t* tb1; int tsplit; float* tsum; int64_t ld_tsum;
 };
-template <int NIT, typename TG, typename TA, bool GATED>
+template <int NIT, typename TG, typename TA, bool GATED, bool TAIL = false>
 __global__ __launch_bounds__(256) void ln_mod_bwd_pair_kernel(LnBwdProb p0, LnBwdProb p1, int nblk0, int d, int rch) {
   const bool first = (int)blockIdx.x < nblk0;
   const LnBwdProb& p = first ? p0 : p1;
-  ln_mod_bwd_body<NIT, TG, TA, GATED>(first ? (int)blockIdx.x : (int)blockIdx.x - nblk0, (const TG*)p.dout, p.x, p.mean, p.rstd, p.scale, p.ld_mod, p.dres, d, p.rpb, p.nchunk,
-                                      p.dx, p.dscale, p.dshift, p.ld_dmod, (const TA*)p.acc, p.gate, p.ld_gate, (TA*)p.dacc, p.dgate, p.ld_dgate, p.dbias, p.ld_dbias, rch);
+  ln_mod_bwd_body<NIT, TG, TA, GATED, TAIL>(first ? (int)blockIdx.x : (int)blockIdx.x - nblk0, (const TG*)p.dout, p.x, p.mean, p.rstd, p.scale, p.ld_mod, p.dres, d, p.rpb, p.nchunk,
+                                            p.dx, p.dscale, p.dshift, p.ld_dmod, (const TA*)p.acc, p.gate, p.ld_gate, (TA*)p.dacc, p.dgate, p.ld_dgate, p.dbias, p.ld_dbias, rch,
+                                            p.tb0, p.tb1, p.tsplit, p.tsum, p.ld_tsum);
 }
 
 template <int NITX, typename TI, typename TO>
@@ -747,7 +770,7 @@
 }
 
 template <typename T>
-__global__ __launch_bounds__(256) void colsum_kernel(const T* __restrict__ x, int rows, int cols, int64_t ld, float* __restrict__ out, int rch) {
+__device__ __forceinline__ void colsum_body(const T* __restrict__ x, int rows, int cols, int64_t ld, float* __restrict__ out, int rch) {
   __shared__ float sbuf[1024];
   const int tx = threadIdx.x & 127, ty = threadIdx.x >> 7;
   const int c = blockIdx.x * 1024 + tx * 8;
@@ -765,6 +788,18 @@
     }
   }
   colsum_flush(s, sbuf, out, c, cols);
+}
+template <typename T>
+__global__ __launch_bounds__(256) void colsum_kernel(const T* __restrict__ x, int rows, int cols, int64_t ld, float* __restrict__ out, int rch) {
+  colsum_body<T>(x, rows, cols, ld, out, rch);
+}
+inline int colsum_rch(int rows) { return rows <= 256 ? 8 : CO_RCH; }
+struct ColsumTasks { mmdit_colsum_task t[MMDIT_LIST_MAX]; };
+__global__ __launch_bounds__(256) void colsum_list_kernel(ColsumTasks ts) {
+  const mmdit_colsum_task& t = ts.t[blockIdx.z];
+  const int rch = t.rows <= 256 ? 8 : CO_RCH;
+  if ((int)blockIdx.x * 1024 >= t.cols || (int)blockIdx.y * rch >= t.rows) return;
+  colsum_body<float>(t.x, t.rows, t.cols, t.ld, t.out, rch);
 }
 
 template <typename TG, typename TO>
@@ -815,6 +850,54 @@
   }
 }
 
+constexpr int PT_RCH = CO_RCH;
+template <typename TI, typename TO>
+__global__ __launch_bounds__(256) void patch_tokens_colsum_kernel(const TI* __restrict__ src, TO* __restrict__ dst, int rows, int ch, int H, int W, float* __restrict__ colsum) {
+  __shared__ float sbuf[512];
+  const int P = ch * 2, RL = 256 / P;
+  const int p = threadIdx.x % P, rl = threadIdx.x / P;
+  const int W2 = W >> 1, H2 = H >> 1;
+  const int c = p >> 1, yo = p & 1;
+  float s0 = 0.f, s1 = 0.f;
+  if (rl < RL) {
+    const int rend = min(rows, ((int)blockIdx.x + 1) * PT_RCH);
+    for (int r = blockIdx.x * PT_RCH + rl; r < rend; r += RL) {
+      const int j = r % W2, q = r / W2;
+      const int y2 = q % H2;
+      const int64_t b = q / H2;
+      const int64_t img_off = ((b * ch + c) * H + 2 * y2 + yo) * W + 2 * j;
+      const float v0 = io<TI>::ld(src + img_off), v1 = io<TI>::ld(src + img_off + 1);
+      TO* o = dst + (int64_t)r * (ch * 4) + p * 2;
+      io<TO>::st(o, v0);
+      io<TO>::st(o + 1, v1);
+      s0 += sizeof(TO) == 2 ? bf2f(f2bf(v0)) : v0;
+      s1 += sizeof(TO) == 2 ? bf2f(f2bf(v1)) : v1;
+    }
+    sbuf[rl * 2 * P + 2 * p] = s0;
+    sbuf[rl * 2 * P + 2 * p + 1] = s1;
+  }
+  __syncthreads();
+  for (int col = threadIdx.x; col < 2 * P; col += 256) {
+    float s = 0.f;
+    for (int l = 0; l < RL; l++) s += sbuf[l * 2 * P + col];
+    atomicAdd(colsum + col, s);
+  }
+}
+
+struct CastTasks { mmdit_cast_tensor t[MMDIT_LIST_MAX]; };
+__global__ void cast_list_kernel(CastTasks ts) {
+  const mmdit_cast_tensor& t = ts.t[blockIdx.y];
+  const float* __restrict__ src = t.src;
+  bf16_t* __restrict__ dst = (bf16_t*)t.dst;
+  const int64_t n8 = t.numel >> 3;
+  for (int64_t i = (int64_t)blockIdx.x * blockDim.x + threadIdx.x; i < n8; i += (int64_t)gridDim.x * blockDim.x) {
+    float v[8];
+    ld8(src + i * 8, v);
+    st8(dst + i * 8, v);
+  }
+  if (blockIdx.x == 0 && threadIdx.x < (t.numel & 7)) io<bf16_t>::st(dst + n8 * 8 + threadIdx.x, src[n8 * 8 + threadIdx.x]);
+}
+
 template <typename TO>
 __global__ void time_embed_fwd_kernel(const float* __restrict__ t, const float* __restrict__ ts, const float* __restrict__ denom, int batch, int dim, TO* __restrict__ out) {
   const int i = blockIdx.x * blockDim.x + threadIdx.x, b = blockIdx.y;
@@ -988,10 +1071,13 @@
   return mmdit_launch_status();
 }
 
-extern "C" int mmdit_ln_modulate_bwd_pair(const mmdit_ln_bwd_problem* a, const mmdit_ln_bwd_problem* b, int d, int dout_dtype, mmdit_stream_t stream) {
+static int ln_mod_bwd_pair_launch(const mmdit_ln_bwd_problem* a, const mmdit_ln_bwd_problem* b, const mmdit_ln_bwd_tail* ta, const mmdit_ln_bwd_tail* tb,
+                                  int d, int dout_dtype, mmdit_stream_t stream) {
   MMDIT_CHECK_ARG(a && b && d > 0 && d % 4 == 0 && d <= 4096 && a->rows_per_batch > 0 && b->rows_per_batch > 0);
-  const bool gated = a->acc != nullptr;
+  const bool gated = a->acc != nullptr, tail = ta != nullptr;
   MMDIT_CHECK_ARG((b->acc != nullptr) == gated);
+  MMDIT_CHECK_ARG(!tail || (!gated && dout_dtype == MMDIT_BF16));
+  const mmdit_ln_bwd_tail* tls[2] = {ta, tb};
   LnBwdProb q[2];
   const mmdit_ln_bwd_problem* src[2] = {a, b};
   int nb[2];
@@ -999,8 +1085,8 @@
   const int nit_ = nit_for(d), nit_abs = nit_ < 0 ? -nit_ : nit_;
   int per_cu = nit_abs <= 3 ? 4 : nit_abs == 4 ? 3 : 2, cus = 256;
   {
-    static int occ[64][17][2][2], cu_count[64];
-    const int dev = mmdit_current_device(), ti = dout_dtype == MMDIT_BF16 ? 0 : 1, gi = gated ? 1 : 0, ni = nit_abs > 16 ? 16 : nit_abs;
+    static int occ[64][17][2][3], cu_count[64];
+    const int dev = mmdit_current_device(), ti = dout_dtype == MMDIT_BF16 ? 0 : 1, gi = tail ? 2 : gated ? 1 : 0, ni = nit_abs > 16 ? 16 : nit_abs;
     if (!cu_count[dev]) {
       int n = 0;
       cu_count[dev] = (hipDeviceGetAttribute(&n, hipDeviceAttributeMultiprocessorCount, dev) == hipSuccess && n > 0) ? n : 256;
@@ -1010,7 +1096,8 @@
       int nbq = 0;
       hipError_t e = hipErrorUnknown;
 #define LNQ(T, G) NIT_SWITCH(nit_, e = hipOccupancyMaxActiveBlocksPerMultiprocessor(&nbq, (const void*)ln_mod_bwd_pair_kernel<(NIT < 0 ? -NIT : NIT), T, T, G>, 256, 0))
-      if (dout_dtype == MMDIT_BF16) { if (gated) { LNQ(bf16_t, true); } else { LNQ(bf16_t, false); } }
+      if (tail) NIT_SWITCH(nit_, e = hipOccupancyMaxActiveBlocksPerMultiprocessor(&nbq, (const void*)ln_mod_bwd_pair_kernel<(NIT < 0 ? -NIT : NIT), bf16_t, bf16_t, false, true>, 256, 0));
+      else if (dout_dtype == MMDIT_BF16) { if (gated) { LNQ(bf16_t, true); } else { LNQ(bf16_t, false); } }
       else if (dout_dtype == MMDIT_F32) { if (gated) { LNQ(float, true); } else { LNQ(float, false); } }
 #undef LNQ
       occ[dev][ni][ti][gi] = (e == hipSuccess && nbq > 0) ? nbq : 8;
@@ -1024,23 +1111,38 @@
       if (wgs(r) <= slots) { rch = r; break; }
   for (int i = 0; i < 2; i++) {
     const mmdit_ln_bwd_problem* p = src[i];
-    MMDIT_CHECK_ARG(p->dout && p->x && p->mean && p->rstd && p->scale && p->dx && p->dscale && p->dshift && p->rows > 0 && p->rows_per_batch > 0 &&
+    MMDIT_CHECK_ARG(p->dout && p->x && p->mean && p->rstd && p->scale && (p->dx || (tail && tls[i])) && p->dscale && p->dshift && p->rows > 0 && p->rows_per_batch > 0 &&
                     p->rows % p->rows_per_batch == 0 && p->ld_mod % 4 == 0);
     if (gated) MMDIT_CHECK_ARG(p->gate && p->dacc && p->dgate && p->ld_gate % 4 == 0);
     const int nchunk = (p->rows_per_batch + rch - 1) / rch;
     nb[i] = (p->rows / p->rows_per_batch) * nchunk;
     q[i] = LnBwdProb{p->dout, p->x, p->mean, p->rstd, p->scale, p->ld_mod, p->dres, p->rows_per_batch, nchunk, p->dx, p->dscale, p->dshift, p->ld_dmod,
-                     p->acc, p->gate, p->ld_gate, p->dacc, p->dgate, p->ld_dgate, p->dbias, p->ld_dbias};
+                     p->acc, p->gate, p->ld_gate, p->dacc, p->dgate, p->ld_dgate, p->dbias, p->ld_dbias, nullptr, nullptr, 0, nullptr, 0};
+    if (tail && tls[i]) {
+      const mmdit_ln_bwd_tail* t = tls[i];
+      MMDIT_CHECK_ARG(t->out0 && t->split > 0 && t->split <= p->rows_per_batch && (t->split == p->rows_per_batch || t->out1) && t->ld_colsum % 4 == 0);
+      q[i].tb0 = (bf16_t*)t->out0; q[i].tb1 = (bf16_t*)t->out1; q[i].tsplit = t->split; q[i].tsum = t->colsum; q[i].ld_tsum = t->ld_colsum;
+    }
   }
   hipStream_t s = (hipStream_t)stream;
   const int nit = nit_for(d);
   dim3 grid(nb[0] + nb[1]);
 #define LNP(T, G) NIT_SWITCH(nit, hipLaunchKernelGGL((ln_mod_bwd_pair_kernel<(NIT < 0 ? -NIT : NIT), T, T, G>), grid, dim3(256), 0, s, q[0], q[1], nb[0], d, rch))
-  if (dout_dtype == MMDIT_BF16) { if (gated) { LNP(bf16_t, true); } else { LNP(bf16_t, false); } }
+  if (tail) NIT_SWITCH(nit, hipLaunchKernelGGL((ln_mod_bwd_pair_kernel<(NIT < 0 ? -NIT : NIT), bf16_t, bf16_t, false, true>), grid, dim3(256), 0, s, q[0], q[1], nb[0], d, rch));
+  else if (dout_dtype == MMDIT_BF16) { if (gated) { LNP(bf16_t, true); } else { LNP(bf16_t, false); } }
   else if (dout_dtype == MMDIT_F32) { if (gated) { LNP(float, true); } else { LNP(float, false); } }
   else return MMDIT_ERR_DTYPE;
 #undef LNP
   return mmdit_launch_status();
+}
+
+extern "C" int mmdit_ln_modulate_bwd_pair(const mmdit_ln_bwd_problem* a, const mmdit_ln_bwd_problem* b, int d, int dout_dtype, mmdit_stream_t stream) {
+  return ln_mod_bwd_pair_launch(a, b, nullptr, nullptr, d, dout_dtype, stream);
+}
+extern "C" int mmdit_ln_modulate_bwd_pair_tail(const mmdit_ln_bwd_problem* a, const mmdit_ln_bwd_problem* b, const mmdit_ln_bwd_tail* ta, const mmdit_ln_bwd_tail* tb,
+                                               int d, int dout_dtype, mmdit_stream_t stream) {
+  MMDIT_CHECK_ARG(ta);
+  return ln_mod_bwd_pair_launch(a, b, ta, tb, d, dout_dtype, stream);
 }
 
 extern "C" int mmdit_text_rmsnorm_fwd(const void* x, int x_dtype, const float* w1, const float* w2, const float* s1, const float* s2,
@@ -1328,11 +1430,31 @@
 extern "C" int mmdit_colsum(const void* x, int dtype, int rows, int cols, int64_t ld, float* out, mmdit_stream_t stream) {
   MMDIT_CHECK_ARG(x && out && rows > 0 && cols > 0 && cols % 8 == 0 && ld % 8 == 0);
   hipStream_t s = (hipStream_t)stream;
-  const int rch = rows <= 256 ? 8 : CO_RCH;
+  const int rch = colsum_rch(rows);
   dim3 grid((cols + 1023) / 1024, (rows + rch - 1) / rch);
   if (dtype == MMDIT_BF16) hipLaunchKernelGGL((colsum_kernel<bf16_t>), grid, dim3(256), 0, s, (const bf16_t*)x, rows, cols, ld, out, rch);
   else if (dtype == MMDIT_F32) hipLaunchKernelGGL((colsum_kernel<float>), grid, dim3(256), 0, s, (const float*)x, rows, cols, ld, out, rch);
   else return MMDIT_ERR_DTYPE;
+  return mmdit_launch_status();
+}
+
+extern "C" int mmdit_colsum_list(const mmdit_colsum_task* tasks, int n, mmdit_stream_t stream) {
+  MMDIT_CHECK_ARG(tasks && n > 0);
+  for (int i = 0; i < n; i++)
+    MMDIT_CHECK_ARG(tasks[i].x && tasks[i].out && tasks[i].rows > 0 && tasks[i].cols > 0 && tasks[i].cols % 8 == 0 && tasks[i].ld % 8 == 0);
+  hipStream_t s = (hipStream_t)stream;
+  for (int i0 = 0; i0 < n; i0 += MMDIT_LIST_MAX) {
+    const int m = n - i0 < MMDIT_LIST_MAX ? n - i0 : MMDIT_LIST_MAX;
+    ColsumTasks ts = {};
+    int gx = 1, gy = 1;
+    for (int i = 0; i < m; i++) {
+      const mmdit_colsum_task& t = ts.t[i] = tasks[i0 + i];
+      const int rch = colsum_rch(t.rows);
+      gx = max(gx, (t.cols + 1023) / 1024);
+      gy = max(gy, (t.rows + rch - 1) / rch);
+    }
+    hipLaunchKernelGGL(colsum_list_kernel, dim3(gx, gy, m), dim3(256), 0, s, ts);
+  }
   return mmdit_launch_status();
 }
 
@@ -1473,6 +1595,23 @@
   return mmdit_launch_status();
 }
 
+extern "C" int mmdit_cast_list(const mmdit_cast_tensor* tensors, int n, mmdit_stream_t stream) {
+  MMDIT_CHECK_ARG(tensors && n > 0);
+  for (int i = 0; i < n; i++) MMDIT_CHECK_ARG(tensors[i].src && tensors[i].dst && tensors[i].numel > 0);
+  hipStream_t s = (hipStream_t)stream;
+  for (int i0 = 0; i0 < n; i0 += MMDIT_LIST_MAX) {
+    const int m = n - i0 < MMDIT_LIST_MAX ? n - i0 : MMDIT_LIST_MAX;
+    CastTasks ts = {};
+    int64_t nmax = 0;
+    for (int i = 0; i < m; i++) {
+      ts.t[i] = tensors[i0 + i];
+      nmax = nmax > ts.t[i].numel ? nmax : ts.t[i].numel;
+    }
+    hipLaunchKernelGGL(cast_list_kernel, dim3(grid_cap(nmax / 8 + 1, 256), m), dim3(256), 0, s, ts);
+  }
+  return mmdit_launch_status();
+}
+
 template <bool TO_TOKENS>
 static int patch_dispatch(const void* src, int sdt, void* dst, int ddt, int batch, int ch, int H, int W, mmdit_stream_t stream) {
   MMDIT_CHECK_ARG(src && dst && batch > 0 && ch > 0 && H > 0 && W > 0 && H % 2 == 0 && W % 2 == 0);
@@ -1493,6 +1632,21 @@
 extern "C" int mmdit_unpatchify(const void* tokens, int tok_dtype, int batch, int ch, int H, int W, void* img, int img_dtype, mmdit_stream_t st) {
   return patch_dispatch<false>(tokens, tok_dtype, img, img_dtype, batch, ch, H, W, st);
 }
+extern "C" int mmdit_patchify_colsum(const void* img, int img_dtype, int batch, int ch, int H, int W, void* tokens, int tok_dtype, float* colsum, mmdit_stream_t stream) {
+  MMDIT_CHECK_ARG(img && tokens && colsum && batch > 0 && ch > 0 && ch <= 128 && H > 0 && W > 0 && H % 2 == 0 && W % 2 == 0);
+  const int64_t rows64 = (int64_t)batch * (H / 2) * (W / 2);
+  MMDIT_CHECK_ARG(rows64 < (1ll << 31) - PT_RCH);
+  const int rows = (int)rows64;
+  hipStream_t s = (hipStream_t)stream;
+  dim3 grid((rows + PT_RCH - 1) / PT_RCH);
+#define PK(TI, TO) hipLaunchKernelGGL((patch_tokens_colsum_kernel<TI, TO>), grid, dim3(256), 0, s, (const TI*)img, (TO*)tokens, rows, ch, H, W, colsum)
+  if (img_dtype == MMDIT_F32 && tok_dtype == MMDIT_F32) PK(float, float);
+  else if (img_dtype == MMDIT_F32 && tok_dtype == MMDIT_BF16) PK(float, bf16_t);
+  else if (img_dtype == MMDIT_BF16 && tok_dtype == MMDIT_BF16) PK(bf16_t, bf16_t);
+  else return MMDIT_ERR_DTYPE;
+#undef PK
+  return mmdit_launch_status();
+}
 
 extern "C" int mmdit_time_embed_fwd(const float* t, const float* time_scale, const float* denom, int batch, int dim, void* out, int out_dtype, mmdit_stream_t stream) {
   MMDIT_CHECK_ARG(t && time_scale && denom && out && batch > 0 && dim > 0 && dim % 2 == 0);
diff --git a/stable-diffusion-3-from-scratch_amd/engine.py b/stable-diffusion-3-from-scratch_amd/engine.py
--- a/stable-diffusion-3-from-scratch_amd/engine.py
+++ b/stable-diffusion-3-from-scratch_amd/engine.py
@@ -359,6 +359,7 @@
 _QK_FUSE = _lib.experiment("MMDIT_ATTN_QK_FUSE", "1") != "0"
 _FUSE_SWIGLU_BWD = _lib.experiment("MMDIT_FUSE_SWIGLU_BWD", "1") != "0"
 _FUSE_GATE = _lib.experiment("MMDIT_FUSE_GATE", "1") != "0"
+FOLD_TAIL = True
 
 
 def _qk_bwd_two_pass(m, w, sv, g, dOx, dOc, dims, rope, dev):
@@ -398,7 +399,7 @@
     return st
 
 
-def block_bwd(m, w, sv, dX2, dC2, dy_acc, dims, rope, defer_cond=False, st=None, dacc=None, nxt=None, defer_wmod=False):
+def block_bwd(m, w, sv, dX2, dC2, dy_acc, dims, rope, defer_cond=False, st=None, dacc=None, nxt=None, defer_wmod=False, late_bias=False, tail=None):
     B, N, Mt, H, d = dims
     S, dev = N + Mt, dX2.device
     both = not w.last
@@ -416,7 +417,8 @@
     if both:
         dacc_c = dacc[1] if dacc is not None else ops.gate_residual_bwd(dC2, sv.acc_mc, ms.gate2c, Mt, dms.gate2c, bpart[:, d:], m.T)
         probs.append(dict(A=dacc_c, B=w.mlp_c.Wdown, b_kmajor=True, out_dtype=m.T))
-    ops.colsum(bpart, bdown)
+    if not late_bias:
+        ops.colsum(bpart, bdown)
     dgu = None
     if (_FUSE_SWIGLU_BWD and m.fast and dev.type == "cuda" and m.prec == PREC_BF16 and dacc_x.dtype == BF16 and sv.gu_x.dtype == BF16
             and not w.mlp_x.gelu and (not both or not w.mlp_c.gelu)):
@@ -488,10 +490,13 @@
         ax["gated"], ac["gated"] = nxt.req_x, nxt.req_c
         (dX, nax), (dC, nac) = _ln_bwd_pair(ax, ac)
         nacc = (nax, nac)
+    elif tail is not None:
+        ax["tail"] = dict(split=N, colsum=tail["bpe_part"])
+        (dX, _, _), (_, _, dC) = ops.ln_modulate_bwd_pair(ax, ac)
     else:
         dX, dC = _ln_bwd_pair(ax, ac)
 
-    dmod_a = m.act(dmod)
+    dmod_a = dmod if late_bias else m.act(dmod)
     if defer_cond:
         if not defer_wmod:
             defer(g, "Wmod", dmod_a, sv.yp)
@@ -582,9 +587,13 @@
     def defer(name, dY, Xa):
         pending.append((lambda o, name=name: setattr(g, name, o), _wg(dY, Xa)))
 
-    dZ = ops.patchify(dv.contiguous(), m.T)
+    fold = FOLD_TAIL and on_grads is None and dev.type == "cuda" and m.fast and m.T == BF16
     g.bout = ops.zeros(W.Wout.shape[0], dev)
-    ops.colsum(dZ, g.bout)
+    if fold and Cin <= 128:
+        dZ = ops.patchify_colsum(dv.contiguous(), m.T, g.bout)
+    else:
+        dZ = ops.patchify(dv.contiguous(), m.T)
+        ops.colsum(dZ, g.bout)
     dlnf = _dgrad(m, dZ, W.Wout, m.T)
     defer("Wout", dZ, sv.lnf)
     dmodo = ops.zeros(sv.modo.shape, dev) if sv.modo.dtype == F32 else torch.zeros_like(sv.modo)
@@ -606,14 +615,19 @@
     dmods = [None] * nblk
     yps = [None] * nblk
     batch_wmod = on_grads is None and _BATCH_WMOD
+    late_bias = False
+    tail = dict(bpe_part=ops.zeros((B, d), dev)) if fold and _LN_PAIR else None
+    bias_fin = []
     for i in range(nblk - 1, -1, -1):
         if i > 0:
             sts[i - 1] = block_bwd_begin(m, W.blocks[i - 1], sv.blocks[i - 1], sv.dims, dev, defer_cond=True)
             dX, dC, dmods[i], g.blocks[i], dacc = block_bwd(m, W.blocks[i], sv.blocks[i], dX, dC, None, sv.dims, rope, defer_cond=True,
-                                                            st=sts[i], dacc=dacc, nxt=sts[i - 1], defer_wmod=batch_wmod)
+                                                            st=sts[i], dacc=dacc, nxt=sts[i - 1], defer_wmod=batch_wmod, late_bias=late_bias)
         else:
             dX, dC, dmods[i], g.blocks[i] = block_bwd(m, W.blocks[i], sv.blocks[i], dX, dC, None, sv.dims, rope, defer_cond=True, st=sts[i], dacc=dacc,
-                                                      defer_wmod=batch_wmod)
+                                                      defer_wmod=batch_wmod, late_bias=late_bias, tail=tail)
+        if late_bias:
+            bias_fin.append((sts[i].bpart, sts[i].bdown))
         sts[i] = None
         yps[i] = sv.blocks[i].yp
         sv.blocks[i] = None
@@ -622,6 +636,13 @@
             if repl is not None:
                 _set_grad_tensors(g.blocks[i], repl)
 
+    if tail is not None:
+        g.bpe = ops.zeros(d, dev)
+        bias_fin.append((tail["bpe_part"], g.bpe))
+    if bias_fin:
+        ops.colsum_list(bias_fin)
+    if late_bias:
+        dmods = ops.cast_list(dmods)
     dyp_all = ops.zeros((nblk * B, d), dev)
     by_all = ops.zeros((nblk, d), dev)
     for i0 in range(0, nblk, 12):
@@ -641,9 +662,12 @@
         if batch_wmod:
             pending.append((lambda o, i=i: setattr(g.blocks[i], "Wmod", o), _wg(dmods[i], yps[i])))
 
-    g.bpe = ops.zeros(d, dev)
-    ops.colsum(dX, g.bpe)
-    dX_a = m.act(dX)
+    if tail is not None:
+        dX_a = dX
+    else:
+        g.bpe = ops.zeros(d, dev)
+        ops.colsum(dX, g.bpe)
+        dX_a = m.act(dX)
     dX0 = _dgrad(m, dX_a, W.Wpe, m.T)
     defer("Wpe", dX_a, sv.X0)
     defer("Wpatch", dX0, sv.patches)
diff --git a/stable-diffusion-3-from-scratch_amd/ops.py b/stable-diffusion-3-from-scratch_amd/ops.py
--- a/stable-diffusion-3-from-scratch_amd/ops.py
+++ b/stable-diffusion-3-from-scratch_amd/ops.py
@@ -384,6 +384,17 @@
     return out
 
 
+def cast_list(srcs):
+    outs = [torch.empty(s.shape, dtype=torch.bfloat16, device=s.device) for s in srcs]
+    arr = (_lib.CastTensor * len(srcs))()
+    for q, s, o in zip(arr, srcs, outs):
+        if s.dtype != torch.float32:
+            raise RuntimeError("cast_list: fp32 sources")
+        q.src, q.dst, q.numel = _p(_c(s)), _p(o), s.numel()
+    check(_lib.lib().mmdit_cast_list(arr, len(srcs), _s()), "mmdit_cast_list")
+    return outs
+
+
 _CAST_TABLES = {}
 
 
@@ -457,6 +468,8 @@
 def ln_modulate_bwd_pair(pa, pb):
     gated = pa.get("gated") is not None
     assert (pb.get("gated") is not None) == gated
+    if pa.get("tail") is not None:
+        return _ln_modulate_bwd_pair_tail(pa, pb)
     d = pa["x"].shape[1]
     probs, outs, keep = (_lib.LnBwdProblem * 2)(), [], []
     for q, p in zip(probs, (pa, pb)):
@@ -481,6 +494,32 @@
     return outs
 
 
+def _ln_modulate_bwd_pair_tail(pa, pb):
+    assert pa.get("gated") is None
+    d = pa["x"].shape[1]
+    probs, tails, outs, keep = (_lib.LnBwdProblem * 2)(), (_lib.LnBwdTail * 2)(), [], []
+    for q, t, p in zip(probs, tails, (pa, pb)):
+        dout, x, tl = _c(p["dout"]), p["x"], p.get("tail")
+        rows, dev, rpb = x.shape[0], x.device, p["rpb"]
+        nb = rows // rpb
+        plain = tl is None
+        tl = tl or dict(split=rpb, keep_f32=True)
+        split = tl["split"]
+        dx = torch.empty((rows, d), dtype=torch.float32, device=dev) if tl.get("keep_f32") else None
+        out0 = torch.empty((nb * split, d), dtype=torch.bfloat16, device=dev) if not plain else None
+        out1 = torch.empty((nb * (rpb - split), d), dtype=torch.bfloat16, device=dev) if split < rpb else None
+        cs = tl.get("colsum")
+        q.dout, q.x, q.mean, q.rstd, q.scale, q.ld_mod = _p(dout), _p(x), _p(p["mean"]), _p(p["rstd"]), _p(p["scale"]), p["scale"].stride(0)
+        q.dres, q.rows, q.rows_per_batch = _p(p.get("dres")), rows, rpb
+        q.dx, q.dscale, q.dshift, q.ld_dmod = _p(dx), _p(p["dscale"]), _p(p["dshift"]), p["dscale"].stride(0)
+        t.out0, t.out1, t.split, t.colsum, t.ld_colsum = _p(out0), _p(out1), split, _p(cs), (cs.stride(0) if cs is not None else 0)
+        keep.append(dout)
+        outs.append((out0, out1, dx))
+    check(_lib.lib().mmdit_ln_modulate_bwd_pair_tail(ctypes.byref(probs[0]), ctypes.byref(probs[1]), ctypes.byref(tails[0]), ctypes.byref(tails[1]) if pb.get("tail") is not None else None,
+                                                     d, _dt(pa["dout"]), _s()), "mmdit_ln_modulate_bwd_pair_tail")
+    return outs
+
+
 def gate_residual_fwd(x, acc, gate, rows_per_batch):
     rows, d = x.shape
     out = torch.empty((rows, d), dtype=torch.float32, device=x.device)
@@ -657,6 +696,22 @@
     return out
 
 
+def colsum_list(pairs):
+    arr = (_lib.ColsumTask * len(pairs))()
+    for q, (x, out) in zip(arr, pairs):
+        if x.dtype != torch.float32 or x.dim() != 2 or x.stride(1) != 1:
+            raise RuntimeError("colsum_list: fp32 matrices with unit column stride")
+        q.x, q.out, q.rows, q.cols, q.ld = _p(x), _p(out), x.shape[0], x.shape[1], x.stride(0)
+    check(_lib.lib().mmdit_colsum_list(arr, len(pairs), _s()), "mmdit_colsum_list")
+
+
+def patchify_colsum(img, out_dtype, colsum_out):
+    batch, ch, H, W = img.shape
+    tokens = torch.empty((batch * (H // 2) * (W // 2), ch * 4), dtype=out_dtype, device=img.device)
+    check(_lib.lib().mmdit_patchify_colsum(_p(_c(img)), _dt(img), batch, ch, H, W, _p(tokens), _dt(tokens), _p(colsum_out), _s()), "mmdit_patchify_colsum")
+    return tokens
+
+
 def patchify(img, out_dtype):
     batch, ch, H, W = img.shape
     tokens = torch.empty((batch * (H // 2) * (W // 2), ch * 4), dtype=out_dtype, device=img.device)
```

Result: no change. 2362 (median of 6 runs) (+0.5%).
